# tmtlakmal/acme

Measured on AMD Instinct MI355X. Metric: learner transitions/sec (sample+step) at batch 512, 1/2/4/8 MI355X, higher is better.
Workload: dtype f32 (2xf16 split planes, 3 MFMA terms); 1 GPU; dqn_nature_cnn_prioritized_replay (BASELINE configs[1]); global_batch=512, batch_per_gpu=512, replay_slots=1000000, replay_slots_per_gpu=1000000, obs=uint8[84,84,4], num_actions=18, sampler=prioritized(alpha=0.6), IS beta=0.2, prefetch_size=4, parallelism=dp1

## Files before the change

### acme_amd/_lib.py

```python

from __future__ import annotations

import ctypes
import os
import threading

import torch

_HERE = os.path.dirname(os.path.abspath(__file__))
LIB_PATH = os.environ.get("ACME_LIB_PATH") or os.path.join(_HERE, "libacme_hip.so")

ACME_OK = 0
ACME_ERR_INVALID = -1
ACME_ERR_HIP = -2
ACME_ERR_EMPTY = -3
ACME_ERR_OOM = -4

SEMANTICS_TF = 0
SEMANTICS_JAX = 1

MATMUL_F32 = 0
MATMUL_X6 = 1

MAX_FIELDS = 16
# ... 68 lines not shown
MPO_MAX_ROWS = 131072
MPO_STATS = ("dual_alpha_mean", "dual_alpha_stddev", "dual_temperature", "loss_policy",
             "loss_alpha", "loss_temperature", "kl_q_rel", "penalty_kl_q_rel", "q_min", "q_max",
             "pi_stddev_min", "pi_stddev_max", "pi_stddev_cond")


class MPOConfig(ctypes.Structure):
    _fields_ = [("obs_dim", c_i32), ("act_dim", c_i32), ("max_batch", c_i32),
                ("num_policy_layers", c_i32), ("policy_sizes", c_i32 * D4PG_MAX_LAYERS),
                ("num_critic_layers", c_i32), ("critic_sizes", c_i32 * D4PG_MAX_LAYERS),
                ("action_min", c_f32 * D4PG_MAX_ACT), ("action_max", c_f32 * D4PG_MAX_ACT),
                ("discount", c_f32),
                ("policy_learning_rate", c_f32), ("critic_learning_rate", c_f32),
                ("adam_beta1", c_f32), ("adam_beta2", c_f32), ("adam_epsilon", c_f32),
                ("clipping", c_i32), ("layer_norm_epsilon", c_f32),
                ("num_samples", c_i32), ("target_policy_update_period", c_i32),
                ("target_critic_update_period", c_i32), ("dual_learning_rate", c_f32),
                ("epsilon", c_f32), ("epsilon_mean", c_f32), ("epsilon_stddev", c_f32),
                ("epsilon_penalty", c_f32), ("init_log_temperature", c_f32),
                ("init_log_alpha_mean", c_f32), ("init_log_alpha_stddev", c_f32),
                ("per_dim_constraining", c_i32), ("action_penalization", c_i32),
                ("init_scale", c_f32), ("min_scale", c_f32), ("seed", ctypes.c_uint64)]


class DMPOConfig(ctypes.Structure):
    _anonymous_ = ("mpo",)
    _fields_ = [("mpo", MPOConfig), ("num_atoms", c_i32), ("vmin", c_f32), ("vmax", c_f32)]


class MPOBatch(ctypes.Structure):
    _fields_ = [("o_tm1", c_vp), ("a_tm1", c_vp), ("r_t", c_vp), ("d_t", c_vp), ("o_t", c_vp),
                ("batch", c_i64), ("noise", c_vp)]


class MPOOutputs(ctypes.Structure):
    _fields_ = [("critic_loss", c_vp), ("policy_loss", c_vp), ("stats", c_vp),
                ("kl_mean_rel", c_vp), ("kl_stddev_rel", c_vp)]


IMPALA_TORSO_ATARI = 0
IMPALA_TORSO_FLAT = 1


class IMPALAConfig(ctypes.Structure):
    _fields_ = [("torso", c_i32), ("obs_dim", c_i32), ("num_actions", c_i32),
                ("max_batch", c_i32), ("max_sequence_length", c_i32), ("lstm_size", c_i32),
                ("head_size", c_i32), ("discount", c_f32), ("entropy_cost", c_f32),
                ("baseline_cost", c_f32), ("max_abs_reward", c_f32),
                ("max_gradient_norm", c_f32), ("learning_rate", c_f32), ("adam_beta1", c_f32),
                ("adam_beta2", c_f32), ("adam_epsilon", c_f32), ("semantics", c_i32)]


class R2D2Config(ctypes.Structure):
    _fields_ = [("torso", c_i32), ("obs_dim", c_i32), ("num_actions", c_i32),
                ("max_batch", c_i32), ("max_sequence_length", c_i32), ("burn_in_length", c_i32),
                ("lstm_size", c_i32), ("head_size", c_i32), ("n_step", c_i32),
                ("store_lstm_state", c_i32), ("target_update_period", c_i32),
                ("reserved", c_i32), ("max_replay_size", c_i64),
                ("max_priority_weight", ctypes.c_double),
                ("importance_sampling_exponent", ctypes.c_double), ("discount", c_f32),
                ("learning_rate", c_f32), ("adam_beta1", c_f32), ("adam_beta2", c_f32),
                ("adam_epsilon", c_f32)]


class R2D2Outputs(ctypes.Structure):
    _fields_ = [("loss", c_vp), ("errors", c_vp), ("priorities", c_vp)]


class SequenceBatch(ctypes.Structure):
    _fields_ = [("observation", c_vp), ("prev_action", c_vp), ("prev_reward", c_vp),
                ("action", c_vp), ("reward", c_vp), ("discount", c_vp),
                ("behaviour_logits", c_vp), ("h0", c_vp), ("c0", c_vp),
                ("state_stride", c_i64), ("batch", c_i64), ("sequence_length", c_i64)]


_SIGS = {
    "acme_last_error": (ctypes.c_char_p, []),
    "acme_tune_set": (ctypes.c_int, [ctypes.c_char_p, ctypes.c_int32]),
    "acme_version": (ctypes.c_char_p, []),
    "acme_target_arch": (ctypes.c_char_p, []),
    "acme_set_matmul_engine": (c_i32, [c_i32]),
    "acme_matmul_engine": (c_i32, []),
    "acme_dense_forward": (c_i32, [c_vp, c_i64, c_i64, c_vp, c_vp, c_i64, c_i32, c_vp, c_vp]),
    "acme_dense_forward_staged": (c_i32, [c_vp, c_i64, c_i64, c_vp, c_vp, c_i64, c_i32, c_vp,
                                          c_i32, c_i32, c_i32, c_vp]),
    "acme_replay_create": (c_i32, [ctypes.POINTER(ReplayConfig), ctypes.POINTER(c_vp)]),
    "acme_replay_destroy": (c_i32, [c_vp]),
    "acme_replay_insert": (c_i32, [c_vp, ctypes.POINTER(c_vp), c_i64, c_vp, c_i32, c_vp, c_vp]),
    "acme_replay_stage_capacity": (c_i64, [c_vp]),
    "acme_replay_stage": (c_i32, [c_vp, c_i64, ctypes.POINTER(c_vp)]),
    "acme_replay_commit": (c_i32, [c_vp, c_i64, c_vp, c_vp, c_vp]),
    "acme_replay_sync_inserts": (c_i32, [c_vp]),
    "acme_host_register": (c_i32, [c_vp, c_i64]),
    "acme_event_create": (c_i32, [ctypes.POINTER(c_vp)]),
    "acme_event_destroy": (c_i32, [c_vp]),
    "acme_event_record": (c_i32, [c_vp, c_vp]),
    "acme_stream_wait_event": (c_i32, [c_vp, c_vp]),
    "acme_event_query": (c_i32, [c_vp]),
    "acme_event_synchronize": (c_i32, [c_vp]),
    "acme_host_unregister": (c_i32, [c_vp]),
    "acme_nstep_writer_create": (c_i32, [c_vp, c_i32, c_f32, c_i64, c_i64, c_i64, c_vp]),
    "acme_nstep_writer_destroy": (c_i32, [c_vp]),
    "acme_nstep_writer_start": (c_i32, [c_vp, c_vp]),
    "acme_nstep_writer_add": (c_i32, [c_vp, c_vp, c_f32, c_f32, c_vp, c_i32, c_f64]),
    "acme_nstep_writer_flush": (c_i32, [c_vp]),
    "acme_nstep_writer_reset": (c_i32, [c_vp]),
    "acme_nstep_writer_pending": (c_i64, [c_vp]),
    "acme_replay_fill_synthetic": (c_i32, [c_vp, c_i64, c_i32, c_i32, c_u64, c_vp]),
    "acme_replay_sample": (c_i32, [c_vp, c_i64, c_u64, c_vp, c_vp, c_vp, c_vp, c_vp, c_vp]),
    "acme_replay_gather": (c_i32, [c_vp, c_vp, c_i64, ctypes.POINTER(c_vp), c_vp]),
    "acme_replay_total": (c_i32, [c_vp, c_vp, c_vp]),
    "acme_replay_sample_share": (c_i32, [c_vp, c_i64, c_u64, c_f64, c_vp, c_vp, c_vp, c_vp, c_vp,
                                         ctypes.POINTER(c_vp), c_vp]),
    "acme_replay_sample_share_frames": (c_i32, [c_vp, c_i64, c_u64, c_f64, c_vp, c_vp, c_vp, c_vp,
                                                c_vp, ctypes.POINTER(c_vp), c_vp, c_vp]),
    "acme_replay_sample_gather": (c_i32, [c_vp, c_i64, c_u64, c_vp, c_vp, c_vp, c_vp, c_vp,
                                          ctypes.POINTER(c_vp), c_vp]),
    "acme_replay_sample_gather_frames": (c_i32, [c_vp, c_i64, c_u64, c_vp, c_vp, c_vp, c_vp,
                                                 c_vp, ctypes.POINTER(c_vp), c_vp, c_vp]),
    "acme_replay_pipe_open": (c_i32, [c_vp, ctypes.POINTER(c_i32)]),
    "acme_replay_pipe_close": (c_i32, [c_vp, c_i32]),
    "acme_replay_pipe_flush": (c_i32, [c_vp, c_i32]),
    "acme_replay_sample_gather_pipe": (c_i32, [c_vp, c_i32, c_i64, c_u64, c_vp, c_vp, c_vp, c_vp,
                                               c_vp, ctypes.POINTER(c_vp), c_vp]),
    "acme_r2d2_priorities": (c_i32, [c_vp, c_i32, c_i32, ctypes.c_double, c_vp, c_vp]),
    "acme_r2d2_importance_weights": (c_i32, [c_vp, c_i32, c_i64, ctypes.c_double, c_vp, c_vp]),
    "acme_frames_expand": (c_i32, [c_vp, c_i64, c_i64, c_i32, c_vp, c_i64, c_vp, c_vp]),
    "acme_replay_update_priorities": (c_i32, [c_vp, c_vp, c_vp, c_i64, c_vp]),
    "acme_replay_update_priorities_gated": (c_i32, [c_vp, c_vp, c_vp, c_i64, c_vp, c_vp]),
    "acme_replay_size": (c_i64, [c_vp]),
    "acme_replay_capacity": (c_i64, [c_vp]),
    "acme_replay_debug_leaves": (c_i32, [c_vp, ctypes.POINTER(c_vp), ctypes.POINTER(c_vp),
                                         ctypes.POINTER(c_vp)]),
    "acme_replay_debug_level": (c_i32, [c_vp, c_i32, ctypes.POINTER(c_vp),
                                        ctypes.POINTER(c_i64), ctypes.POINTER(c_i32)]),
    "acme_replay_storage": (c_i32, [c_vp, c_i32, ctypes.POINTER(c_vp)]),
    "acme_replay_inserted": (c_i64, [c_vp]),
    "acme_replay_restore": (c_i32, [c_vp, c_i64, c_vp]),
    "acme_dqn_create": (c_i32, [ctypes.POINTER(DQNConfig), ctypes.POINTER(c_vp)]),
    "acme_dqn_destroy": (c_i32, [c_vp]),
    "acme_dqn_num_params": (c_i64, [c_vp]),
    "acme_dqn_flat_size": (c_i64, [c_vp]),
    "acme_dqn_num_tensors": (c_i32, [c_vp]),
    "acme_dqn_tensor_info": (c_i32, [c_vp, c_i32, ctypes.POINTER(c_i64), ctypes.POINTER(c_i64),
                                     ctypes.POINTER(c_i32), ctypes.POINTER(c_i64),
                                     ctypes.POINTER(ctypes.c_char_p)]),
    "acme_dqn_bind": (c_i32, [c_vp, c_vp, c_vp, c_vp, c_vp, c_vp]),
    "acme_dqn_params_changed": (c_i32, [c_vp]),
    "acme_dqn_plane_overflow": (c_i32, [c_vp, ctypes.POINTER(c_i32), c_i32]),
    "acme_dqn_skipped_steps": (c_i64, [c_vp]),
    "acme_dqn_guard_state": (c_i32, [c_vp, ctypes.POINTER(c_i64)]),
    "acme_dqn_verdict_timeouts": (c_i32, [c_vp, ctypes.POINTER(c_i64)]),
    "acme_dqn_update_rider_launches": (c_i64, [c_vp]),
    "acme_dqn_set_applied_steps": (c_i32, [c_vp, c_i64]),
    "acme_dqn_skip_word": (c_i32, [c_vp, ctypes.POINTER(c_vp)]),
    "acme_dqn_set_reissue": (c_i32, [c_vp, c_i32]),
    "acme_dqn_verdicts_issued": (c_i64, [c_vp]),
    "acme_dqn_step_verdict": (c_i32, [c_vp, c_i64, ctypes.POINTER(c_i32)]),
    "acme_dqn_set_data_parallel_gate": (c_i32, [c_vp, c_i32]),
    "acme_dqn_dense_grads_ready": (c_i32, [c_vp, c_vp]),
    "acme_dqn_dp_init": (c_i32, [c_vp, c_vp, c_i32]),
    "acme_dqn_dp_step": (c_i32, [c_vp, ctypes.POINTER(TransitionBatch), ctypes.POINTER(DQNOutputs),
                                 c_vp]),
    "acme_nccl_get_unique_id": (c_i32, [c_vp]),
    "acme_nccl_comm_init": (c_i32, [c_vp, c_i32, c_i32, ctypes.POINTER(c_vp)]),
    "acme_nccl_comm_destroy": (c_i32, [c_vp]),
    "acme_dqn_scale_state": (c_i32, [c_vp, c_vp, c_i32, ctypes.POINTER(c_i32)]),
    "acme_dqn_set_scale_state": (c_i32, [c_vp, c_vp, c_i32]),
    "acme_dqn_forward_backward": (c_i32, [c_vp, ctypes.POINTER(TransitionBatch),
                                          ctypes.POINTER(DQNOutputs), c_vp]),
    "acme_dqn_apply": (c_i32, [c_vp, c_vp]),
    "acme_dqn_forward_backward_stage": (c_i32, [c_vp, ctypes.POINTER(TransitionBatch),
                                                ctypes.POINTER(DQNOutputs), c_i32, c_vp]),
    "acme_dqn_grad_split": (c_i32, [c_vp, ctypes.POINTER(c_i64)]),
    "acme_dqn_step": (c_i32, [c_vp, ctypes.POINTER(TransitionBatch), ctypes.POINTER(DQNOutputs),
                              c_vp]),
    "acme_dqn_step_update": (c_i32, [c_vp, ctypes.POINTER(TransitionBatch),
                                     ctypes.POINTER(DQNOutputs), c_vp, c_vp, c_vp, c_vp]),
    "acme_dqn_q_values": (c_i32, [c_vp, c_vp, c_i64, c_i32, c_vp, c_vp]),
    "acme_dqn_num_steps": (c_i64, [c_vp]),
    "acme_dqn_debug_buffer": (c_i32, [c_vp, ctypes.c_char_p, ctypes.POINTER(c_vp),
                                      ctypes.POINTER(c_i64)]),
    "acme_dqn_set_num_steps": (c_i32, [c_vp, c_i64]),
    "acme_min_f64": (c_i32, [c_vp, c_i64, c_vp, c_vp]),
    "acme_r2d2_create": (c_i32, [ctypes.POINTER(R2D2Config), ctypes.POINTER(c_vp)]),
    "acme_r2d2_destroy": (c_i32, [c_vp]),
    "acme_r2d2_flat_size": (c_i64, [c_vp]),
    "acme_r2d2_num_tensors": (c_i32, [c_vp]),
    "acme_r2d2_tensor_info": (c_i32, [c_vp, c_i32, ctypes.POINTER(c_i64), ctypes.POINTER(c_i64),
                                      ctypes.POINTER(c_i32), ctypes.POINTER(c_i64),
                                      ctypes.POINTER(ctypes.c_char_p)]),
    "acme_r2d2_bind": (c_i32, [c_vp, c_vp, c_vp, c_vp, c_vp, c_vp]),
    "acme_r2d2_step": (c_i32, [c_vp, ctypes.POINTER(SequenceBatch), c_vp,
                               ctypes.POINTER(R2D2Outputs), c_vp]),
    "acme_r2d2_params_changed": (c_i32, [c_vp]),
    "acme_r2d2_scale_state": (c_i32, [c_vp, c_vp, c_i32, ctypes.POINTER(c_i32)]),
    "acme_r2d2_set_scale_state": (c_i32, [c_vp, c_vp, c_i32]),
    "acme_r2d2_skipped_steps": (c_i64, [c_vp]),
    "acme_r2d2_guard_state": (c_i32, [c_vp, ctypes.POINTER(c_i64)]),
    "acme_r2d2_skip_word": (c_vp, [c_vp]),
    "acme_r2d2_set_applied_steps": (c_i32, [c_vp, c_i64]),
    "acme_r2d2_num_steps": (c_i64, [c_vp]),
    "acme_r2d2_set_num_steps": (c_i32, [c_vp, c_i64]),
    "acme_r2d2_set_lstm_unroll": (c_i32, [c_vp, c_i32]),
    "acme_r2d2_debug_buffer": (c_i32, [c_vp, ctypes.c_char_p, ctypes.POINTER(c_vp),
                                       ctypes.POINTER(c_i64)]),
    "acme_impala_create": (c_i32, [ctypes.POINTER(IMPALAConfig), ctypes.POINTER(c_vp)]),
    "acme_impala_destroy": (c_i32, [c_vp]),
    "acme_impala_flat_size": (c_i64, [c_vp]),
    "acme_impala_num_tensors": (c_i32, [c_vp]),
    "acme_impala_tensor_info": (c_i32, [c_vp, c_i32, ctypes.POINTER(c_i64), ctypes.POINTER(c_i64),
                                        ctypes.POINTER(c_i32), ctypes.POINTER(c_i64),
                                        ctypes.POINTER(ctypes.c_char_p)]),
    "acme_impala_bind": (c_i32, [c_vp, c_vp, c_vp, c_vp, c_vp]),
    "acme_impala_params_changed": (c_i32, [c_vp]),
    "acme_impala_step": (c_i32, [c_vp, ctypes.POINTER(SequenceBatch), c_vp, c_vp]),
    "acme_impala_set_lstm_unroll": (c_i32, [c_vp, c_i32]),
    "acme_impala_plane_overflow": (c_i32, [c_vp, ctypes.POINTER(c_i32), c_i32]),
    "acme_impala_skipped_steps": (c_i64, [c_vp]),
    "acme_impala_guard_state": (c_i32, [c_vp, ctypes.POINTER(c_i64)]),
    "acme_impala_set_applied_steps": (c_i32, [c_vp, c_i64]),
    "acme_impala_scale_state": (c_i32, [c_vp, c_vp, c_i32, ctypes.POINTER(c_i32)]),
    "acme_impala_set_scale_state": (c_i32, [c_vp, c_vp, c_i32]),
    "acme_impala_policy_step": (c_i32, [c_vp, c_vp, c_vp, c_vp, c_vp, c_vp, c_i64, c_vp, c_vp,
                                        c_vp, c_vp, c_vp]),
    "acme_impala_set_policy_planes": (c_i32, [c_vp, c_i32]),
    "acme_impala_num_steps": (c_i64, [c_vp]),
    "acme_impala_set_num_steps": (c_i32, [c_vp, c_i64]),
    "acme_impala_debug_buffer": (c_i32, [c_vp, ctypes.c_char_p, ctypes.POINTER(c_vp),
                                         ctypes.POINTER(c_i64)]),
    "acme_d4pg_create": (c_i32, [ctypes.POINTER(D4PGConfig), ctypes.POINTER(c_vp)]),
    "acme_d4pg_destroy": (c_i32, [c_vp]),
    "acme_d4pg_flat_size": (c_i64, [c_vp]),
    "acme_d4pg_policy_size": (c_i64, [c_vp]),
    "acme_d4pg_num_tensors": (c_i32, [c_vp]),
    "acme_d4pg_tensor_info": (c_i32, [c_vp, c_i32, ctypes.POINTER(c_i64), ctypes.POINTER(c_i64),
                                      ctypes.POINTER(c_i32), ctypes.POINTER(c_i64),
                                      ctypes.POINTER(ctypes.c_char_p)]),
    "acme_d4pg_bind": (c_i32, [c_vp, c_vp, c_vp, c_vp, c_vp, c_vp]),
    "acme_d4pg_step": (c_i32, [c_vp, ctypes.POINTER(D4PGBatch), ctypes.POINTER(D4PGOutputs),
                               c_vp]),
    "acme_d4pg_policy": (c_i32, [c_vp, c_vp, c_i64, c_i32, c_vp, c_vp]),
    "acme_d4pg_num_steps": (c_i64, [c_vp]),
    "acme_d4pg_set_num_steps": (c_i32, [c_vp, c_i64]),
    "acme_d4pg_debug_buffer": (c_i32, [c_vp, ctypes.c_char_p, ctypes.POINTER(c_vp),
                                       ctypes.POINTER(c_i64)]),
    "acme_ddpg_create": (c_i32, [ctypes.POINTER(DDPGConfig), ctypes.POINTER(c_vp)]),
    "acme_ddpg_destroy": (c_i32, [c_vp]),
    "acme_ddpg_flat_size": (c_i64, [c_vp]),
    "acme_ddpg_policy_size": (c_i64, [c_vp]),
    "acme_ddpg_num_tensors": (c_i32, [c_vp]),
    "acme_ddpg_tensor_info": (c_i32, [c_vp, c_i32, ctypes.POINTER(c_i64), ctypes.POINTER(c_i64),
                                      ctypes.POINTER(c_i32), ctypes.POINTER(c_i64),
                                      ctypes.POINTER(ctypes.c_char_p)]),
    "acme_ddpg_bind": (c_i32, [c_vp, c_vp, c_vp, c_vp, c_vp, c_vp]),
    "acme_ddpg_step": (c_i32, [c_vp, ctypes.POINTER(D4PGBatch), ctypes.POINTER(D4PGOutputs),
                               c_vp]),
    "acme_ddpg_policy": (c_i32, [c_vp, c_vp, c_i64, c_i32, c_vp, c_vp]),
    "acme_ddpg_num_steps": (c_i64, [c_vp]),
    "acme_ddpg_set_num_steps": (c_i32, [c_vp, c_i64]),
    "acme_ddpg_debug_buffer": (c_i32, [c_vp, ctypes.c_char_p, ctypes.POINTER(c_vp),
                                       ctypes.POINTER(c_i64)]),
    "acme_mpo_create": (c_i32, [ctypes.POINTER(MPOConfig), ctypes.POINTER(c_vp)]),
    "acme_mpo_destroy": (c_i32, [c_vp]),
    "acme_mpo_flat_size": (c_i64, [c_vp]),
    "acme_mpo_policy_size": (c_i64, [c_vp]),
    "acme_mpo_dual_offset": (c_i64, [c_vp]),
    "acme_mpo_num_tensors": (c_i32, [c_vp]),
    "acme_mpo_tensor_info": (c_i32, [c_vp, c_i32, ctypes.POINTER(c_i64), ctypes.POINTER(c_i64),
                                     ctypes.POINTER(c_i32), ctypes.POINTER(c_i64),
                                     ctypes.POINTER(ctypes.c_char_p)]),
    "acme_mpo_bind": (c_i32, [c_vp, c_vp, c_vp, c_vp, c_vp, c_vp]),
    "acme_mpo_init_duals": (c_i32, [c_vp]),
    "acme_mpo_step": (c_i32, [c_vp, ctypes.POINTER(MPOBatch), ctypes.POINTER(MPOOutputs), c_vp]),
    "acme_mpo_policy": (c_i32, [c_vp, c_vp, c_i64, c_i32, c_vp, c_vp, c_vp]),
    "acme_mpo_num_steps": (c_i64, [c_vp]),
    "acme_mpo_set_num_steps": (c_i32, [c_vp, c_i64]),
    "acme_mpo_debug_buffer": (c_i32, [c_vp, ctypes.c_char_p, ctypes.POINTER(c_vp),
                                      ctypes.POINTER(c_i64)]),
    "acme_dmpo_create": (c_i32, [ctypes.POINTER(DMPOConfig), ctypes.POINTER(c_vp)]),
    "acme_dmpo_destroy": (c_i32, [c_vp]),
    "acme_dmpo_flat_size": (c_i64, [c_vp]),
    "acme_dmpo_policy_size": (c_i64, [c_vp]),
    "acme_dmpo_dual_offset": (c_i64, [c_vp]),
    "acme_dmpo_num_tensors": (c_i32, [c_vp]),
    "acme_dmpo_tensor_info": (c_i32, [c_vp, c_i32, ctypes.POINTER(c_i64), ctypes.POINTER(c_i64),
                                      ctypes.POINTER(c_i32), ctypes.POINTER(c_i64),
                                      ctypes.POINTER(ctypes.c_char_p)]),
    "acme_dmpo_bind": (c_i32, [c_vp, c_vp, c_vp, c_vp, c_vp, c_vp]),
    "acme_dmpo_init_duals": (c_i32, [c_vp]),
    "acme_dmpo_step": (c_i32, [c_vp, ctypes.POINTER(MPOBatch), ctypes.POINTER(MPOOutputs), c_vp]),
    "acme_dmpo_policy": (c_i32, [c_vp, c_vp, c_i64, c_i32, c_vp, c_vp, c_vp]),
    "acme_dmpo_num_steps": (c_i64, [c_vp]),
    "acme_dmpo_set_num_steps": (c_i32, [c_vp, c_i64]),
    "acme_dmpo_debug_buffer": (c_i32, [c_vp, ctypes.c_char_p, ctypes.POINTER(c_vp),
                                       ctypes.POINTER(c_i64)]),
    "acme_profile_enable": (c_i32, [c_i32]),
    "acme_profile_reset": (c_i32, []),
    "acme_profile_num_sections": (c_i32, []),
    "acme_profile_query_peak": (c_i32, [c_i32, ctypes.POINTER(c_f64)]),
    "acme_profile_query": (c_i32, [c_i32, ctypes.POINTER(ctypes.c_char_p), ctypes.POINTER(c_f64),
                                   ctypes.POINTER(c_i64), ctypes.POINTER(c_f64),
                                   ctypes.POINTER(c_f64)]),
    "acme_adam_update": (c_i32, [c_vp, c_vp, c_vp, c_vp, c_i64, c_f32, c_f32, c_f32, c_f32, c_i64,
                                 c_vp]),
}
# ... 106 lines not shown
```

### acme_amd/csrc/dqn.hip

```cpp
#include <hip/hip_runtime.h>

#include <algorithm>
#include <cmath>
#include <cstring>
#include <string>
#include <vector>

#include "common.h"
#include "conv.h"
#include "rescale.h"
#include "conv_p3.h"
#include "gemm.h"
#include "gemm_p3.h"
#include "gemm_x6.h"
#include "kernels.h"
#include "launch.h"
#include "learner_common.h"
#include "plane_guard.h"
#include "prio_update.h"
#include "profiler.h"
#include "rccl_dyn.h"
#include "torso.h"

using namespace acme;
using namespace acme::conv;
using acme::gemm::launch_gemm;

namespace {

using torso::G1;
constexpr int kFlat = torso::kFlat;
constexpr int kHidden = 512;
constexpr int kObsBytes = 84 * 84 * 4;

struct Layer {
  int in = 0, out = 0;
  int w = -1, b = -1;
  bool relu = true;
};

struct StepPlan {
  bool calibrating = false;
  bool fused = false;
  bool join_dense = false;
  acme_replay* replay = nullptr;
  const uint64_t* keys = nullptr;
  hipEvent_t after = nullptr;
};

struct StepState {
  int64_t fwd_batch = 0;
  bool last_p3 = false;
  torso::Frames cur_frames{nullptr};
  LossArgs pending_la{};
  bool loss_pending = false;
  bool head_deferred = false;
  int head_splits = 0;
  int64_t loss_nparts = 0;
  hipEvent_t dense_ev = nullptr;
  bool slabs_pending = false;
  torso::WgradSlab wslabs[3];
  bool rescaled = false;
  const double* upd_prio = nullptr;
  int upd_n = 0;
  bool update_issued = false;
};

}

struct acme_dqn : PlaneGuard {
  acme_dqn_config cfg;
  std::vector<Tensor> tensors;
  int64_t flat = 0, logical = 0;
  float *params = nullptr, *target = nullptr, *grads = nullptr, *m = nullptr, *v = nullptr;
  int64_t num_steps = 0;
  int t_c1w = -1, t_c1b, t_c2w, t_c2b, t_c3w, t_c3b, t_fcw, t_fcb, t_vw, t_vb, t_aw, t_ab;
  std::vector<Layer> layers;
  std::vector<void*> allocs;
  float *x1 = nullptr, *x2 = nullptr, *x3 = nullptr, *hid = nullptr;
  float *t1 = nullptr, *t2 = nullptr, *t3 = nullptr, *thid = nullptr;
  std::vector<float*> mlp_act, mlp_tact, mlp_dz;
  float *q_on = nullptr, *q_tg = nullptr;
  float *dzh = nullptr, *dz3 = nullptr, *dz2 = nullptr, *dz1 = nullptr;
  float* slab = nullptr;
  int64_t slab_floats = 0;
  bool stamps_on = false;
  uint64_t* stamps = nullptr;
  float* g = nullptr;
  int32_t* a_cache = nullptr;
  float* loss_tmp = nullptr;
  float* td_tmp = nullptr;
  double* prio_tmp = nullptr;
  bool p3_capable = false;
  bool planes_stale = true;
  uint16_t *wpl = nullptr, *tpl = nullptr;
  uint16_t* frames = nullptr;
  StepState step;
  hipStream_t side = nullptr;
  hipEvent_t ev[4] = {nullptr, nullptr, nullptr, nullptr};
  float* slab2 = nullptr;
  float* side_slab = nullptr;
  float* tslab = nullptr;
  bool target_dirty = true;
  torso::Plane x1p{}, x2p{}, x3p{}, t1p{}, t2p{}, t3p{}, dzhp{}, dz3p{}, dz2p{}, dz1p{};
  hipEvent_t ev_dense = nullptr;
  void* dp_comm = nullptr;
  int dp_world = 0;
  hipStream_t dp_stream = nullptr;
  hipEvent_t dp_ev[4] = {nullptr, nullptr, nullptr, nullptr};
  double* dp_gmin = nullptr;
  double* loss_part = nullptr;
  bool single_stream = false;
  bool single_role = false;
  bool bk32 = false;
  bool update_rider = true;
  int64_t rider_launches = 0;
  bool frames_u8 = true;
  int64_t seq = 0;
  uint32_t* host_verdicts = nullptr;
  uint32_t verdict_seq = 0;
  bool sticky = false;
  bool dp_gate = false;
  int64_t dp_gate_index = -1;
};

namespace {

enum {
  kScX1, kScX2, kScX3, kScT1, kScT2, kScT3, kScDzh, kScDz3, kScDz2, kScDz1,
  kScTransient,
  kScParams = kScTransient, kScTarget,
  kScCount
};
constexpr int64_t kParamAmaxPeriod = 8;
constexpr int kVerdictRing = 64;

int add_tensor(acme_dqn* l, const std::string& name, std::initializer_list<int64_t> shape) {
  const int t = acme::add_tensor<acme_dqn>(l, name, shape);
  l->logical += l->tensors[t].numel;
  return t;
}

inline torso::Plane WP(const acme_dqn* l, uint16_t* base, int t) {
  return torso::Plane{base + l->tensors[t].offset, l->flat,
                      l->scales + (base == l->tpl ? kScTarget : kScParams)};
}
int convert_frames(acme_dqn* l, const void* obs_a, const void* obs_b, int split, int rows,
                   hipStream_t st) {
  ACME_PROF("frames_f16", st, 0.0, 3.0 * (double)rows * kObsBytes);
  return launch_frames_f16(static_cast<const uint8_t*>(obs_a), static_cast<const uint8_t*>(obs_b),
                           split, rows, kObsBytes, l->frames, st);
}
bool use_p3(const acme_dqn* l) { return l->p3_capable && gemm::use_x6(); }
Gate step_gate(const acme_dqn* l) {
  Gate q;
  q.g = l->guard;
  q.par = (int)(l->seq & 1);
  if (l->dp_gate) q.dp = l->grads + l->dp_gate_index;
  return q;
}
hipStream_t side_stream(const acme_dqn* l) { return prof::enabled() ? nullptr : l->side; }

constexpr int kFcFwdSplits = 8;
constexpr int kHeadFwdSplits = 16;
constexpr int kHeadBwdSplits = 8;

int64_t slab_floats_needed(int B, int A) {
  return std::max<int64_t>({torso::wgrad_slab_floats(), (int64_t)kFcFwdSplits * 2 * B * 2 * kHidden,
                            (int64_t)kHeadFwdSplits * 2 * B * (A + 1),
                            (int64_t)kHeadBwdSplits * (2 * kHidden + 1) * (A + 1)});
}

int slab_reduce(const float* slab, int splits, int64_t count, float* out0, int64_t split_at,
                float* out1, const float* bias, int ncols, int relu, const char* name,
                hipStream_t st) {
  ACME_PROF(name, st, 0.0, 4.0 * (double)(splits + 1) * (double)count);
  return launch_slab_reduce(slab, splits, count, out0, split_at, out1, bias, ncols, relu, st);
}

int adam_range(acme_dqn* l, int64_t off, int64_t n, const Gate& gate, const AdamTail& tail,
               hipStream_t st) {
  const bool jax = l->cfg.semantics == ACME_SEMANTICS_JAX;
  const bool p3 = l->p3_capable;
  return launch_adam(l->params + off, l->grads + off, l->m + off, l->v + off, n,
                     l->cfg.learning_rate, l->cfg.adam_beta1, l->cfg.adam_beta2,
                     l->cfg.adam_epsilon, 0, p3 ? l->wpl + off : nullptr, l->flat, st, jax ? 1 : 0,
                     &l->guard->applied, p3 ? l->scales + kScParams : nullptr, gate, !p3, tail);
}

torso::Weights torso_weights(const acme_dqn* l, const float* prm) {
  return torso::Weights{P(l, prm, l->t_c1w), P(l, prm, l->t_c1b), P(l, prm, l->t_c2w),
                        P(l, prm, l->t_c2b), P(l, prm, l->t_c3w), P(l, prm, l->t_c3b)};
}
torso::Grads torso_grads(const acme_dqn* l) {
  float* gr = l->grads;
  return torso::Grads{Pm(l, gr, l->t_c1w), Pm(l, gr, l->t_c1b), Pm(l, gr, l->t_c2w),
                      Pm(l, gr, l->t_c2b), Pm(l, gr, l->t_c3w), Pm(l, gr, l->t_c3b)};
}
torso::PWeights torso_pweights(const acme_dqn* l, const float* prm, uint16_t* wpl) {
  return torso::PWeights{WP(l, wpl, l->t_c1w), WP(l, wpl, l->t_c2w), WP(l, wpl, l->t_c3w),
                         P(l, prm, l->t_c1b), P(l, prm, l->t_c2b), P(l, prm, l->t_c3b)};
}

int head_forward(acme_dqn* l, const float* prm, int rows, const float* hid, float* q,
                 hipStream_t st) {
  const int A = l->cfg.num_actions;
  DuelHeadFwd p;
  p.M = rows; p.N = A + 1; p.K = 2 * kHidden; p.k_chunk = chunk_for(p.K, kHeadFwdSplits);
  p.H = kHidden; p.A = A; p.h = hid; p.wv = P(l, prm, l->t_vw); p.wa = P(l, prm, l->t_aw);
  p.slab = l->slab;
  ACME_GEMM("head_fwd", 64, 32, 2, 1, 16, 1, p, kHeadFwdSplits);
  ACME_PROF("head_fwd_finish", st, 0.0, 0.0);
  return launch_duel_head_finish(l->slab, kHeadFwdSplits, rows, A, P(l, prm, l->t_vb),
                                 P(l, prm, l->t_ab), q, st);
}

int nature_forward(acme_dqn* l, const float* prm, const void* obs_a, const void* obs_b,
                   int split, int rows, float* x1, float* x2, float* x3, float* hid,
                   float* q, hipStream_t st) {
  const bool u8 = l->cfg.obs_dtype == ACME_OBS_U8_SCALED;
  int rc0 = torso::forward(torso_weights(l, prm), u8, obs_a, obs_b, split, rows,
                           torso::Acts{x1, x2, x3}, st);
  if (rc0 != ACME_OK) return rc0;
  {
    DenseFwd<true> p;
    const int splits = kFcFwdSplits;
    p.M = rows; p.N = 2 * kHidden; p.K = kFlat; p.k_chunk = chunk_for(kFlat, splits);
    p.x = x3; p.x2 = x3; p.split_b = rows; p.ldx = kFlat;
    p.w = P(l, prm, l->t_fcw); p.bias = P(l, prm, l->t_fcb); p.y = hid; p.act = ACT_RELU;
    p.slab = l->slab;
    ACME_GEMM("fc_fwd", 128, 128, 2, 2, 32, 1, p, splits);
    const int64_t cnt = (int64_t)rows * 2 * kHidden;
    int rc = slab_reduce(l->slab, splits, cnt, hid, cnt, nullptr, P(l, prm, l->t_fcb),
                         2 * kHidden, 1, "fc_fwd_reduce", st);
    if (rc != ACME_OK) return rc;
  }
  return head_forward(l, prm, rows, hid, q, st);
}

template <int BM>
int fc_fwd_gemm(const acme_dqn* l, const char* name, P3DenseFwd p, int splits,
                hipStream_t st) {
  if (l->single_role) ACME_P3_GEMM(name, BM, 128, 2, 2, 32, p, splits);
  else ACME_P3WS_GEMM(name, BM, 128, 2, 2, 32, p, splits);
  return ACME_OK;
}

int nature_forward_p3(acme_dqn* l, const float* prm, uint16_t* wpl, const torso::Frames& frames,
                      int rows, const torso::Plane& x1, const torso::Plane& x2,
                      const torso::Plane& x3, float* hid, float* q, hipStream_t st,
                      float* slab = nullptr, int keep_x1 = -1, bool defer_head = false) {
  if (!slab) slab = l->slab;
  int rc = torso::forward_p3(torso_pweights(l, prm, wpl), frames, rows, torso::PActs{x1, x2, x3}, st, keep_x1, l->bk32);
  if (rc != ACME_OK) return rc;
  {
    P3DenseFwd p;
    const bool tall = rows > 512;
    const bool ttall = rows == 512 && !defer_head;
    const int splits = kFcFwdSplits;
    p.M = rows; p.N = 2 * kHidden; p.K = kFlat; p.k_chunk = chunk_for(kFlat, splits);
    p.a_src = SRC(x3, (int64_t)rows * kFlat); p.ldx = kFlat;
    p.b_src = SRC(WP(l, wpl, l->t_fcw), (int64_t)kFlat * 2 * kHidden); p.slab = slab;
    if (tall) p.stamps = l->stamps;
    rc = tall || ttall ? fc_fwd_gemm<256>(l, ttall ? "fc_fwd_target" : "fc_fwd", p, splits, st)
                       : fc_fwd_gemm<128>(l, "fc_fwd", p, splits, st);
    if (rc != ACME_OK) return rc;
    if (defer_head &&
        dqn_head_loss_dz_fusable(kHidden, l->cfg.num_actions, splits, P(l, prm, l->t_vw),
                                 P(l, prm, l->t_aw), P(l, prm, l->t_fcb))) {
      l->step.head_deferred = true;
      l->step.head_splits = splits;
      return ACME_OK;
    }
    ACME_PROF("fc_head_fwd", st, 0.0, 4.0 * (double)rows * 2 * kHidden * (splits + 1));
    return launch_fc_head_forward(slab, splits, rows, kHidden, P(l, prm, l->t_fcb),
                                  P(l, prm, l->t_vw), P(l, prm, l->t_vb), P(l, prm, l->t_aw),
                                  P(l, prm, l->t_ab), l->cfg.num_actions, hid, q, st);
  }
}

template <class In>
int mlp_layer(acme_dqn* l, const float* prm, const Layer& L, const void* a, const void* b,
              int split, int rows, float* y, hipStream_t st) {
  const bool vec = L.in % 4 == 0 && L.out % 4 == 0;
  if (vec) {
    DenseFwd<true, In> p;
    p.M = rows; p.N = L.out; p.K = L.in; p.k_chunk = L.in;
    p.x = static_cast<const typename In::T*>(a); p.x2 = static_cast<const typename In::T*>(b);
    p.split_b = split; p.ldx = L.in; p.w = P(l, prm, L.w); p.bias = P(l, prm, L.b); p.y = y;
    p.act = L.relu ? ACT_RELU : ACT_NONE;
    ACME_GEMM("mlp_fwd", 64, 64, 2, 2, 16, 1, p, 1);
  } else {
    DenseFwd<false, In> p;
    p.M = rows; p.N = L.out; p.K = L.in; p.k_chunk = L.in;
    p.x = static_cast<const typename In::T*>(a); p.x2 = static_cast<const typename In::T*>(b);
    p.split_b = split; p.ldx = L.in; p.w = P(l, prm, L.w); p.bias = P(l, prm, L.b); p.y = y;
    p.act = L.relu ? ACT_RELU : ACT_NONE;
    ACME_GEMM("mlp_fwd", 64, 64, 2, 2, 16, 1, p, 1);
  }
  return ACME_OK;
}

int mlp_forward(acme_dqn* l, const float* prm, const void* obs_a, const void* obs_b, int split,
                int rows, std::vector<float*>& act, float* q, hipStream_t st) {
  const int nl = (int)l->layers.size();
  for (int i = 0; i < nl; ++i) {
    const Layer& L = l->layers[i];
    float* y = i == nl - 1 ? q : act[i];
    int rc;
    if (i == 0) {
      rc = l->cfg.obs_dtype == ACME_OBS_U8_SCALED
               ? mlp_layer<InU8>(l, prm, L, obs_a, obs_b, split, rows, y, st)
               : mlp_layer<InF32>(l, prm, L, obs_a, obs_b, split, rows, y, st);
    } else {
      rc = mlp_layer<InF32>(l, prm, L, act[i - 1], act[i - 1], rows, rows, y, st);
    }
    if (rc != ACME_OK) return rc;
  }
  return ACME_OK;
}

RescaleJob take_step_rescale(acme_dqn* l, bool defer_r) {
  RescaleJob j;
  j.s = l->scales;
  j.nt = j.n = kScTransient;
  j.overflow = l->overflow;
  j.skip_lo = kScT1;
  j.skip_hi = kScT3 + 1;
  j.defer_r = defer_r ? 1 : 0;
  j.rg.g = l->guard;
  j.rg.mode = kRgStep;
  j.rg.gate = step_gate(l);
  j.rg.host_skipped = l->host_skipped;
  j.rg.host_verdicts = l->host_verdicts;
  j.rg.seq = l->verdict_seq++;
  j.rg.sticky = l->sticky ? 1 : 0;
  l->step.rescaled = true;
  return j;
}

int torso_backward_p3(acme_dqn* l, const StepPlan& plan, int B, hipStream_t st) {
  const torso::Grads g = torso_grads(l);
  StepState& s = l->step;
  torso::Side sd;
  sd.bk32 = l->bk32;
  sd.conv1_single = true;
  if (side_stream(l)) {
    sd.side = l->side;
    sd.slab = l->side_slab;
    for (int i = 0; i < 3; ++i) sd.e[i] = l->ev[i];
  }
  if (plan.fused && !plan.calibrating && l->slab2) {
    sd.slab = l->side_slab;
    sd.slab2 = l->slab2;
    sd.defer = s.wslabs;
    s.slabs_pending = true;
  }
  int rc = torso::backward_p3_convs(torso_pweights(l, l->params, l->wpl), g, B,
                                    torso::PActs{l->x1p, l->x2p, l->x3p}, l->dz3p, l->dz2p,
                                    l->dz1p, l->slab, st, sd);
  if (rc != ACME_OK) return rc;
  const bool write_back = plan.replay && s.upd_prio;
  FusedUpdateArgs upd;
  const bool rider = write_back && l->update_rider && plan.fused && !l->dp_gate &&
                     s.upd_n >= 1 && s.upd_n <= kUpdateRiderMax;
  if (rider) {
    if (plan.after) ACME_HIP_TRY(hipStreamWaitEvent(st, plan.after, 0));
    const RescaleJob job = take_step_rescale(l, true);
    if ((rc = replay_update_prepare(plan.replay, plan.keys, s.upd_prio, s.upd_n, step_gate(l), st,
                                    &job, kUpdateRiderBlocks, &upd)) != ACME_OK)
      return rc;
    l->rider_launches += 1;
    s.update_issued = true;
  }
  rc = torso::backward_p3_conv1(g, s.cur_frames, B, l->dz1p, l->slab, st, sd,
                                rider ? &upd : nullptr);
  if (rider) replay_update_release(plan.replay);
  if (rc != ACME_OK) return rc;
  if (write_back && !rider) {
    s.update_issued = true;
    if (plan.after) ACME_HIP_TRY(hipStreamWaitEvent(st, plan.after, 0));
    const RescaleJob job = take_step_rescale(l, true);
    if ((rc = replay_update_priorities_gated(plan.replay, plan.keys, s.upd_prio, s.upd_n,
                                             step_gate(l), st, &job)) != ACME_OK)
      return rc;
  }
  return torso::backward_p3_join(st, sd);
}

int nature_backward(acme_dqn* l, const StepPlan& plan, const void* o_tm1, int B,
                    hipStream_t st_main, bool join_dense) {
  StepState& s = l->step;
  hipStream_t st = st_main;
  const float* prm = l->params;
  float* gr = l->grads;
  const int A = l->cfg.num_actions;
  const bool p3 = use_p3(l);
  int rc;
  bool loss_sum = false;
  const LossArgs la = s.pending_la;
  if (p3 && s.loss_pending && s.head_deferred) {
    s.loss_pending = s.head_deferred = false;
    loss_sum = true;
    s.loss_nparts = B;
    ACME_PROF("head_loss_dz", st, 0.0, 4.0 * (double)2 * B * 2 * kHidden * (s.head_splits + 1));
    rc = launch_dqn_head_loss_dz(la, l->slab, s.head_splits, kHidden, P(l, prm, l->t_fcb),
// ... 29 lines not shown
    s.upd_n = B;
  }
  const bool sum_in_scatter = loss_sum;
  {
    DuelHeadWgrad p;
    p.M = 2 * kHidden; p.N = A + 1; p.K = B; p.k_chunk = chunk_for(B, kHeadBwdSplits);
    p.A = A; p.h = l->hid; p.g = l->g; p.act = l->a_cache; p.slab = hslab;
    ACME_GEMM("head_wgrad", 64, 32, 2, 1, 16, 1, p, kHeadBwdSplits);
    ACME_PROF("head_wgrad_scatter", st, 0.0, 0.0);
    rc = launch_duel_head_grad_scatter(
        hslab, kHeadBwdSplits, kHidden, A, Pm(l, gr, l->t_vw), Pm(l, gr, l->t_vb),
        Pm(l, gr, l->t_aw), Pm(l, gr, l->t_ab), st, sum_in_scatter ? la.loss_part : nullptr,
        s.loss_nparts, la.mean_over, la.loss);
    if (rc != ACME_OK) return rc;
  }
  if (p3) {
    {
      P3DenseWgrad p;
      p.M = kFlat; p.N = 2 * kHidden; p.K = B; p.k_chunk = B;
      p.a_src = SRC(l->x3p, (int64_t)B * kFlat); p.ldx = kFlat;
      p.b_src = SRC(l->dzhp, (int64_t)B * 2 * kHidden); p.out = Pm(l, gr, l->t_fcw);
      p.bias_out = Pm(l, gr, l->t_fcb);
      ACME_P3_GEMM("fc_wgrad", 128, 128, 2, 2, 16, p, 1);
    }
    if (fork) {
      ACME_HIP_TRY(hipEventRecord(l->ev[3], l->side));
      st = st_main;
    }
    {
      P3DenseDgrad p;
      p.M = B; p.N = kFlat; p.K = 2 * kHidden; p.k_chunk = p.K;
      p.a_src = SRC(l->dzhp, (int64_t)B * 2 * kHidden);
      p.b_src = SRC(WP(l, l->wpl, l->t_fcw), (int64_t)kFlat * 2 * kHidden); p.xprev = CP(l->x3p);
      p.ldx = kFlat; p.dx = PP(l->dz3p);
      if (l->single_role) ACME_P3G_GEMM("fc_dgrad", 128, 128, 2, 2, 32, 3, p, 1);
      else ACME_P3WS_GEMM("fc_dgrad", 128, 128, 2, 2, 32, p, 1);
    }
    if (fork && join_dense) ACME_HIP_TRY(hipStreamWaitEvent(st_main, l->ev[3], 0));
    if (fork) s.dense_ev = l->ev[3];
    return ACME_OK;
  }
  {
    DenseWgrad<true> p;
    p.M = kFlat; p.N = 2 * kHidden; p.K = B; p.k_chunk = B;
    p.x = l->x3; p.ldx = kFlat; p.dz = l->dzh; p.out = Pm(l, gr, l->t_fcw);
    p.bias_out = Pm(l, gr, l->t_fcb);
    ACME_GEMM("fc_wgrad", 128, 128, 2, 2, 16, 1, p, 1);
  }
  {
    DenseDgrad<true> p;
    p.M = B; p.N = kFlat; p.K = 2 * kHidden; p.k_chunk = p.K;
    p.dz = l->dzh; p.w = P(l, prm, l->t_fcw); p.xprev = l->x3; p.ldx = kFlat; p.dx = l->dz3;
    ACME_GEMM("fc_dgrad", 64, 128, 2, 2, 16, 1, p, 1);
  }
  return ACME_OK;
}

template <class In>
int mlp_wgrad(acme_dqn* l, const Layer& L, const void* x, const float* dz, int B, float* dw,
              float* db, hipStream_t st) {
  if (L.in % 4 == 0 && L.out % 4 == 0) {
    DenseWgrad<true, In> p;
    p.M = L.in; p.N = L.out; p.K = B; p.k_chunk = B;
    p.x = static_cast<const typename In::T*>(x); p.ldx = L.in; p.dz = dz; p.out = dw;
    p.bias_out = db;
    ACME_GEMM("mlp_wgrad", 64, 64, 2, 2, 16, 1, p, 1);
  } else {
    DenseWgrad<false, In> p;
    p.M = L.in; p.N = L.out; p.K = B; p.k_chunk = B;
    p.x = static_cast<const typename In::T*>(x); p.ldx = L.in; p.dz = dz; p.out = dw;
    p.bias_out = db;
    ACME_GEMM("mlp_wgrad", 64, 64, 2, 2, 16, 1, p, 1);
  }
  return ACME_OK;
}

int mlp_backward(acme_dqn* l, const void* o_tm1, int B, hipStream_t st) {
  const int nl = (int)l->layers.size();
  const float* prm = l->params;
  float* gr = l->grads;
  int rc = launch_onehot_dq(l->g, l->a_cache, B, l->cfg.num_actions, l->mlp_dz[nl - 1], st);
  if (rc != ACME_OK) return rc;
  for (int i = nl - 1; i >= 0; --i) {
    const Layer& L = l->layers[i];
    const float* dz = l->mlp_dz[i];
    if (i == 0) {
      rc = l->cfg.obs_dtype == ACME_OBS_U8_SCALED
               ? mlp_wgrad<InU8>(l, L, o_tm1, dz, B, Pm(l, gr, L.w), Pm(l, gr, L.b), st)
               : mlp_wgrad<InF32>(l, L, o_tm1, dz, B, Pm(l, gr, L.w), Pm(l, gr, L.b), st);
    } else {
      rc = mlp_wgrad<InF32>(l, L, l->mlp_act[i - 1], dz, B, Pm(l, gr, L.w), Pm(l, gr, L.b), st);
    }
    if (rc != ACME_OK) return rc;
    if (i > 0) {
      if (L.in % 4 == 0 && L.out % 4 == 0) {
        DenseDgrad<true> p;
        p.M = B; p.N = L.in; p.K = L.out; p.k_chunk = L.out;
        p.dz = dz; p.w = P(l, prm, L.w); p.xprev = l->mlp_act[i - 1]; p.ldx = L.in;
        p.dx = l->mlp_dz[i - 1];
        ACME_GEMM("mlp_dgrad", 64, 64, 2, 2, 16, 1, p, 1);
      } else {
        DenseDgrad<false> p;
        p.M = B; p.N = L.in; p.K = L.out; p.k_chunk = L.out;
        p.dz = dz; p.w = P(l, prm, L.w); p.xprev = l->mlp_act[i - 1]; p.ldx = L.in;
        p.dx = l->mlp_dz[i - 1];
        ACME_GEMM("mlp_dgrad", 64, 64, 2, 2, 16, 1, p, 1);
      }
    }
  }
  return ACME_OK;
}

int sync_planes(acme_dqn* l, hipStream_t st) {
  if (!l->p3_capable || !l->planes_stale) return ACME_OK;
  int rc = launch_split_planes(l->params, l->flat, l->wpl, l->flat, l->scales + kScParams, st,
                               l->overflow, 1);
  if (rc == ACME_OK)
    rc = launch_split_planes(l->target, l->flat, l->tpl, l->flat, l->scales + kScTarget, st,
                             l->overflow, 1);
  if (rc == ACME_OK) l->planes_stale = false;
  return rc;
}

int reset_scales(acme_dqn* l) {
  return scales_init(l, kScCount, [l](int i) {
    return i >= kScT1 && i <= kScT3 ? &l->guard->tt
           : i >= kScTransient     ? &l->guard->prm
                                   : &l->guard->on;
  });
}

}

extern "C" {

int acme_dqn_create(const acme_dqn_config* cfg, acme_dqn** out) {
  ACME_CHECK_ARG(cfg && out, "null argument");
  ACME_CHECK_ARG(cfg->num_actions >= 1 && cfg->num_actions <= 63, "num_actions must be in [1, 63]");
  ACME_CHECK_ARG(cfg->max_batch >= 1 && cfg->max_batch <= 65536, "max_batch must be in [1, 65536]");
  ACME_CHECK_ARG(cfg->network == ACME_NET_NATURE_DQN || cfg->network == ACME_NET_MLP,
                 "unknown network kind %d", cfg->network);
  ACME_CHECK_ARG(cfg->obs_dtype == ACME_OBS_U8_SCALED || cfg->obs_dtype == ACME_OBS_F32,
                 "unknown observation dtype %d", cfg->obs_dtype);
  ACME_CHECK_ARG(cfg->huber_loss_parameter >= 0.f, "quadratic_linear_boundary must be >= 0.");
  ACME_CHECK_ARG(cfg->target_update_period >= 1, "target_update_period must be >= 1");
  ACME_CHECK_ARG(cfg->semantics == ACME_SEMANTICS_TF || cfg->semantics == ACME_SEMANTICS_JAX,
                 "unknown learner semantics %d", cfg->semantics);
  acme_dqn* l = new acme_dqn();
  l->cfg = *cfg;
  l->single_stream = tune_variant("SIDE") == 1;
  l->single_role = tune_variant("WSN") == 1;
  l->bk32 = tune_variant("BK32") == 1;
  l->update_rider = tune_variant("UPDATE_RIDER", kUpdateRiderDefault) != 0;
  l->stamps_on = tune_variant("STAMPS") == 1;
  const int A = cfg->num_actions;
  const int B = cfg->max_batch;
  int rc = ACME_OK;
  auto fail = [&](int code) {
    acme_dqn_destroy(l);
    return code;
  };
  if ((rc = guard_create(l)) != ACME_OK) return fail(rc);
  if (hipHostMalloc(reinterpret_cast<void**>(&l->host_verdicts), kVerdictRing * sizeof(uint32_t),
                    hipHostMallocCoherent | hipHostMallocMapped) != hipSuccess)
    return fail((set_error("step guard allocation failed"), ACME_ERR_HIP));
  for (int i = 0; i < kVerdictRing; ++i) l->host_verdicts[i] = 0xFFFFFFFFu;
  if (cfg->network == ACME_NET_NATURE_DQN) {
    l->t_c1w = add_tensor(l, "atari_torso/conv2_d/w", {8, 8, 4, 32});
    l->t_c1b = add_tensor(l, "atari_torso/conv2_d/b", {32});
    l->t_c2w = add_tensor(l, "atari_torso/conv2_d_1/w", {4, 4, 32, 64});
    l->t_c2b = add_tensor(l, "atari_torso/conv2_d_1/b", {64});
    l->t_c3w = add_tensor(l, "atari_torso/conv2_d_2/w", {3, 3, 64, 64});
    l->t_c3b = add_tensor(l, "atari_torso/conv2_d_2/b", {64});
    l->t_fcw = add_tensor(l, "duelling_q_network/hidden/w", {kFlat, 2 * kHidden});
    l->t_fcb = add_tensor(l, "duelling_q_network/hidden/b", {2 * kHidden});
    l->t_vw = add_tensor(l, "duelling_q_network/mlp/linear_1/w", {kHidden, 1});
    l->t_vb = add_tensor(l, "duelling_q_network/mlp/linear_1/b", {1});
    l->t_aw = add_tensor(l, "duelling_q_network/mlp_1/linear_1/w", {kHidden, A});
    l->t_ab = add_tensor(l, "duelling_q_network/mlp_1/linear_1/b", {A});
    const int R2 = 2 * B;
    if ((rc = dev_alloc(l, &l->x1, (int64_t)R2 * G1::OPIX * G1::CO)) ||
        (rc = dev_alloc(l, &l->x2, (int64_t)R2 * kFlat)) ||
        (rc = dev_alloc(l, &l->x3, (int64_t)R2 * kFlat)) ||
        (rc = dev_alloc(l, &l->hid, (int64_t)R2 * 2 * kHidden)) ||
        (rc = dev_alloc(l, &l->t1, (int64_t)B * G1::OPIX * G1::CO)) ||
        (rc = dev_alloc(l, &l->t2, (int64_t)B * kFlat)) ||
        (rc = dev_alloc(l, &l->t3, (int64_t)B * kFlat)) ||
        (rc = dev_alloc(l, &l->thid, (int64_t)B * 2 * kHidden)) ||
        (rc = dev_alloc(l, &l->dzh, (int64_t)B * 2 * kHidden)) ||
        (rc = dev_alloc(l, &l->dz3, (int64_t)B * kFlat)) ||
        (rc = dev_alloc(l, &l->dz2, (int64_t)B * kFlat)) ||
        (rc = dev_alloc(l, &l->dz1, (int64_t)B * G1::OPIX * G1::CO)))
      return fail(rc);
    l->slab_floats = slab_floats_needed(B, A);
    if (cfg->obs_dtype == ACME_OBS_U8_SCALED && (int64_t)R2 * kObsBytes * 2 < (int64_t)INT32_MAX) {
      l->p3_capable = true;
      const int64_t fl = l->flat;
      if ((rc = reset_scales(l)) ||
          (rc = dev_alloc(l, &l->wpl, gemm::kPlanes * fl)) ||
          (rc = dev_alloc(l, &l->tpl, gemm::kPlanes * fl)) ||
          (rc = dev_alloc(l, &l->frames, (int64_t)R2 * kObsBytes)) ||
          (rc = plane_alloc(l, &l->x1p, (int64_t)R2 * torso::kX1, kScX1)) ||
          (rc = plane_alloc(l, &l->x2p, (int64_t)R2 * kFlat, kScX2)) ||
          (rc = plane_alloc(l, &l->x3p, (int64_t)R2 * kFlat, kScX3)) ||
          (rc = plane_alloc(l, &l->t1p, (int64_t)B * torso::kX1, kScT1)) ||
          (rc = plane_alloc(l, &l->t2p, (int64_t)B * kFlat, kScT2)) ||
          (rc = plane_alloc(l, &l->t3p, (int64_t)B * kFlat, kScT3)) ||
          (rc = plane_alloc(l, &l->dzhp, (int64_t)B * 2 * kHidden, kScDzh)) ||
          (rc = dev_alloc(l, &l->loss_part,
                          std::max<int64_t>(B, dqn_loss_head_dz_blocks(B, kHidden)))) ||
          (rc = plane_alloc(l, &l->dz3p, (int64_t)B * kFlat, kScDz3)) ||
          (rc = plane_alloc(l, &l->dz2p, (int64_t)B * kFlat, kScDz2)) ||
          (rc = plane_alloc(l, &l->dz1p, (int64_t)B * torso::kX1, kScDz1)))
        return fail(rc);
      l->slab_floats = std::max(l->slab_floats, torso::wgrad_slab_floats_p3());
      if (!l->single_stream) {
        hipError_t e = hipStreamCreateWithFlags(&l->side, hipStreamNonBlocking);
        for (auto& ev : l->ev)
          if (e == hipSuccess) e = make_order_event(&ev);
        if (e != hipSuccess)
          return fail((set_error("side stream: %s", hipGetErrorString(e)), ACME_ERR_HIP));
      }
      if ((rc = dev_alloc(l, &l->side_slab, l->slab_floats)) ||
          (rc = dev_alloc(l, &l->tslab, l->slab_floats)) ||
          (rc = dev_alloc(l, &l->slab2, torso::wgrad_slab_floats_p3())))
        return fail(rc);
    }
  } else {
    ACME_CHECK_ARG(cfg->obs_dim >= 1, "obs_dim must be >= 1");
    ACME_CHECK_ARG(cfg->num_hidden >= 0 && cfg->num_hidden <= ACME_MAX_MLP_LAYERS,
                   "num_hidden must be in [0, %d]", ACME_MAX_MLP_LAYERS);
    int in = cfg->obs_dim;
    char name[64];
    for (int i = 0; i <= cfg->num_hidden; ++i) {
      Layer L;
      L.in = in;
      L.out = i < cfg->num_hidden ? cfg->hidden[i] : A;
      L.relu = i < cfg->num_hidden;
      if (L.out < 1) return fail((set_error("hidden sizes must be >= 1"), ACME_ERR_INVALID));
      snprintf(name, sizeof(name), "mlp/linear_%d/w", i);
      L.w = add_tensor(l, name, {L.in, L.out});
      snprintf(name, sizeof(name), "mlp/linear_%d/b", i);
      L.b = add_tensor(l, name, {L.out});
      l->layers.push_back(L);
      in = L.out;
    }
    for (size_t i = 0; i < l->layers.size(); ++i) {
      float *a = nullptr, *ta = nullptr, *dz = nullptr;
      const int w = l->layers[i].out;
      if ((rc = dev_alloc(l, &a, (int64_t)2 * B * w)) || (rc = dev_alloc(l, &ta, (int64_t)B * w)) ||
          (rc = dev_alloc(l, &dz, (int64_t)B * w)))
        return fail(rc);
      l->mlp_act.push_back(a);
      l->mlp_tact.push_back(ta);
      l->mlp_dz.push_back(dz);
    }
    l->slab_floats = 1;
  }
  if (make_order_event(&l->ev_dense) != hipSuccess)
    return fail((set_error("event creation failed"), ACME_ERR_HIP));
  if ((rc = dev_alloc(l, &l->q_on, (int64_t)2 * B * A)) ||
      (rc = dev_alloc(l, &l->q_tg, (int64_t)B * A)) ||
      (rc = dev_alloc(l, &l->slab, l->slab_floats)) ||
      (rc = dev_alloc(l, &l->g, (int64_t)B)) || (rc = dev_alloc(l, &l->a_cache, (int64_t)B)) ||
      (rc = dev_alloc(l, &l->loss_tmp, 4)) || (rc = dev_alloc(l, &l->td_tmp, (int64_t)B)) ||
      (rc = dev_alloc(l, &l->prio_tmp, (int64_t)B)) ||
      (l->stamps_on && (rc = dev_alloc(l, &l->stamps, (int64_t)5 * 4096 * 8))))
    return fail(rc);
  if (l->stamps_on) {
    for (int i = 0; i < 3; ++i) torso::g_stamps_conv[i] = l->stamps + (int64_t)(i + 1) * 4096 * 8;
    g_update_stamps = l->stamps + (int64_t)4 * 4096 * 8;
  }
  if (hipDeviceSynchronize() != hipSuccess)
    return fail((set_error("learner init failed"), ACME_ERR_HIP));
  *out = l;
  return ACME_OK;
}

int acme_dqn_destroy(acme_dqn* l) {
  if (!l) return ACME_OK;
  (void)hipDeviceSynchronize();
  if (l->stamps_on) {
    for (auto& p : torso::g_stamps_conv) p = nullptr;
    g_update_stamps = nullptr;
  }
  for (void* p : l->allocs) (void)hipFree(p);
  for (auto& e : l->ev)
    if (e) (void)hipEventDestroy(e);
  if (l->side) (void)hipStreamDestroy(l->side);
  if (l->ev_dense) (void)hipEventDestroy(l->ev_dense);
  for (auto& e : l->dp_ev)
    if (e) (void)hipEventDestroy(e);
  if (l->dp_stream) (void)hipStreamDestroy(l->dp_stream);
  guard_destroy(l);
  if (l->host_verdicts) (void)hipHostFree(l->host_verdicts);
  delete l;
  return ACME_OK;
}

int64_t acme_dqn_num_params(const acme_dqn* l) { return l ? l->logical : 0; }
int64_t acme_dqn_flat_size(const acme_dqn* l) { return l ? l->flat : 0; }
int32_t acme_dqn_num_tensors(const acme_dqn* l) { return l ? (int32_t)l->tensors.size() : 0; }

int acme_dqn_tensor_info(const acme_dqn* l, int32_t i, int64_t* offset, int64_t* numel,
                         int32_t* ndim, int64_t* shape4, const char** name) {
  return tensor_info(l, i, offset, numel, ndim, shape4, name);
}

int acme_dqn_bind(acme_dqn* l, float* params, float* target, float* grads, float* adam_m,
                  float* adam_v) {
  ACME_CHECK_ARG(l && params && target && grads && adam_m && adam_v, "null buffer");
  for (const float* p : {params, target, grads, adam_m, adam_v})
    ACME_CHECK_ARG(reinterpret_cast<uintptr_t>(p) % 16 == 0, "buffers must be 16-byte aligned");
  l->params = params;
  l->target = target;
  l->grads = grads;
  l->m = adam_m;
  l->v = adam_v;
  l->planes_stale = true;
  l->scales_ok = false;
  return ACME_OK;
}

int acme_dqn_params_changed(acme_dqn* l) {
  ACME_CHECK_ARG(l, "null learner");
  l->planes_stale = true;
  l->scales_ok = false;
  l->target_dirty = true;
  return ACME_OK;
}

int acme_dqn_scale_state(const acme_dqn* l, float* out, int32_t capacity, int32_t* count) {
  return scale_state(l, out, capacity, count);
}

int acme_dqn_set_scale_state(acme_dqn* l, const float* in, int32_t count) {
  const int rc = set_scale_state(l, in, count);
  if (rc == ACME_OK) l->target_dirty = true;
  return rc;
}

int acme_dqn_plane_overflow(acme_dqn* l, int32_t* overflow, int32_t reset) {
  return plane_overflow(l, overflow, reset);
}

int64_t acme_dqn_skipped_steps(const acme_dqn* l) { return skipped_steps(l); }

int acme_dqn_guard_state(acme_dqn* l, int64_t* out4) {
  ACME_CHECK_ARG(l && out4 && l->guard, "null argument");
  StepGuard g;
  if (int rc = read_guard(l, &g)) return rc;
  out4[0] = g.applied;
  out4[1] = g.skipped;
  out4[2] = g.last;
  out4[3] = g.qv;
  return ACME_OK;
}

int acme_dqn_verdict_timeouts(acme_dqn* l, int64_t* out) {
  ACME_CHECK_ARG(l && out, "null argument");
  *out = 0;
  if (!l->guard) return ACME_OK;
  StepGuard g;
  if (int rc = read_guard(l, &g)) return rc;
  *out = g.vtimeout;
  return ACME_OK;
}

int64_t acme_dqn_update_rider_launches(const acme_dqn* l) { return l ? l->rider_launches : 0; }

int acme_dqn_set_reissue(acme_dqn* l, int32_t enable) {
  ACME_CHECK_ARG(l, "null learner");
  l->sticky = enable != 0 && l->p3_capable;
  return ACME_OK;
}

int64_t acme_dqn_verdicts_issued(const acme_dqn* l) { return l ? (int64_t)l->verdict_seq : 0; }

int acme_dqn_step_verdict(const acme_dqn* l, int64_t seq, int32_t* state) {
  ACME_CHECK_ARG(l && state && seq >= 0, "bad argument");
  *state = -1;
  if (!l->host_verdicts || seq >= (int64_t)l->verdict_seq) return ACME_OK;
  ACME_CHECK_ARG(seq + kVerdictRing >= (int64_t)l->verdict_seq,
                 "verdict %lld is older than the ring's %d", (long long)seq, kVerdictRing);
  const uint32_t v =
      __atomic_load_n(l->host_verdicts + (seq & (kVerdictRing - 1)), __ATOMIC_ACQUIRE);
  if ((v >> 1) == ((uint32_t)seq & 0x7fffffffu)) *state = (int32_t)(v & 1u);
  return ACME_OK;
}

int acme_dqn_set_applied_steps(acme_dqn* l, int64_t n) {
  ACME_CHECK_ARG(l && l->guard && n >= 0, "bad argument");
  return set_applied(l, n);
}

int acme_dqn_skip_word(const acme_dqn* l, const uint32_t** out) {
  ACME_CHECK_ARG(l && out, "null argument");
  *out = l->p3_capable ? &l->guard->last : nullptr;
  return ACME_OK;
}

int acme_dqn_set_data_parallel_gate(acme_dqn* l, int32_t enable) {
  ACME_CHECK_ARG(l, "null learner");
  if (enable && l->cfg.network == ACME_NET_NATURE_DQN && l->p3_capable) {
    const Tensor& t = l->tensors[l->t_c1b];
    ACME_CHECK_ARG(align64(t.offset + t.numel) > t.offset + t.numel, "no padding word for the gate");
    l->dp_gate_index = t.offset + t.numel;
    l->dp_gate = true;
  } else {
    l->dp_gate = false;
  }
  return ACME_OK;
}

int64_t acme_dqn_num_steps(const acme_dqn* l) { return l ? l->num_steps : 0; }
int acme_dqn_set_num_steps(acme_dqn* l, int64_t n) {
  ACME_CHECK_ARG(l && n >= 0, "bad argument");
  l->num_steps = n;
  return ACME_OK;
}

int acme_dqn_debug_buffer(const acme_dqn* l, const char* name, const float** out,
                          int64_t* count) {
  ACME_CHECK_ARG(l && name && out && count, "null argument");
  const int64_t B = l->cfg.max_batch;
  struct {
    const char* n;
    const float* p;
    int64_t c;
  } tab[] = {{"gemm_stamps", reinterpret_cast<const float*>(l->stamps), 2 * 5 * 4096 * 8},
             {"x1", l->x1, 2 * B * 441 * 32}, {"x2", l->x2, 2 * B * kFlat},
             {"x3", l->x3, 2 * B * kFlat},    {"hid", l->hid, 2 * B * 2 * kHidden},
             {"dzh", l->dzh, B * 2 * kHidden}, {"dz3", l->dz3, B * kFlat},
             {"dz2", l->dz2, B * kFlat},       {"dz1", l->dz1, B * 441 * 32},
             {"q_on", l->q_on, 2 * B * l->cfg.num_actions},
             {"q_tg", l->q_tg, B * l->cfg.num_actions}, {"g", l->g, B}};
  for (auto& e : tab)
    if (e.p && std::strcmp(e.n, name) == 0) {
      if (l->step.last_p3) {
        struct {
          const char* n;
          torso::Plane pl;
        } ptab[] = {{"x1", l->x1p},   {"x2", l->x2p},   {"x3", l->x3p},  {"dzh", l->dzhp},
                    {"dz3", l->dz3p}, {"dz2", l->dz2p}, {"dz1", l->dz1p}};
        for (auto& q : ptab)
          if (std::strcmp(q.n, name) == 0) {
            int rc = launch_join_planes(q.pl.p, q.pl.stride, e.c, const_cast<float*>(e.p),
                                        q.pl.sc, 0);
            if (rc != ACME_OK) return rc;
            ACME_HIP_TRY(hipDeviceSynchronize());
          }
      }
      *out = e.p;
      *count = e.c;
      return ACME_OK;
    }
  for (size_t i = 0; i < l->mlp_act.size(); ++i) {
    char nm[16];
    snprintf(nm, sizeof(nm), "act%zu", i);
    if (std::strcmp(nm, name) == 0) {
      *out = l->mlp_act[i];
      *count = 2 * B * l->layers[i].out;
      return ACME_OK;
    }
  }
  set_error("unknown debug buffer '%s'", name);
  return ACME_ERR_INVALID;
}

int acme_dqn_q_values(acme_dqn* l, const void* obs, int64_t batch, int32_t use_target,
                      float* q_out, void* stream) {
  ACME_CHECK_ARG(l && obs && q_out && l->params, "null argument or unbound learner");
  ACME_CHECK_ARG(batch >= 1 && batch <= l->cfg.max_batch, "batch must be in [1, max_batch]");
  hipStream_t st = as_stream(stream);
  const float* prm = use_target ? l->target : l->params;
  const int B = (int)batch;
  if (l->cfg.network == ACME_NET_NATURE_DQN && use_p3(l)) {
    l->target_dirty = true;
    int rc = sync_planes(l, st);
    if (rc == ACME_OK) rc = convert_frames(l, obs, obs, B, B, st);
    for (int pass = l->scales_ok ? 1 : 0; pass < 2 && rc == ACME_OK; ++pass) {
      rc = nature_forward_p3(l, prm, use_target ? l->tpl : l->wpl, torso::Frames{l->frames}, B,
                             l->t1p, l->t2p, l->t3p, l->thid, q_out, st);
      RescaleGuard rg;
      rg.g = l->guard;
      rg.mode = kRgQValues;
      if (rc == ACME_OK)
        rc = launch_plane_rescale(l->scales + kScT1, 3, 3, -1, -1, l->overflow, st, -1, -1, rg);
    }
    return rc;
  }
  if (l->cfg.network == ACME_NET_NATURE_DQN)
    return nature_forward(l, prm, obs, obs, B, B, l->t1, l->t2, l->t3, l->thid, q_out, st);
  return mlp_forward(l, prm, obs, obs, B, B, l->mlp_tact, q_out, st);
}

static int forward_backward_stage(acme_dqn* l, const StepPlan& plan,
                                  const acme_transition_batch* batch,
                                  const acme_dqn_outputs* out, int32_t stage, void* stream);

int acme_dqn_forward_backward_stage(acme_dqn* l, const acme_transition_batch* batch,
                                    const acme_dqn_outputs* out, int32_t stage, void* stream) {
  StepPlan plan;
  plan.join_dense = true;
  return forward_backward_stage(l, plan, batch, out, stage, stream);
}

static int loss_and_dense_backward(acme_dqn* l, const StepPlan& plan,
                                   const acme_transition_batch* batch,
                                   const acme_dqn_outputs* out, hipStream_t st, bool join_dense) {
  const int B = (int)batch->batch, A = l->cfg.num_actions;
  const bool nature = l->cfg.network == ACME_NET_NATURE_DQN;
  int rc;
  float* loss = out && out->loss ? out->loss : l->loss_tmp;
  float* td = out && out->td_error ? out->td_error : l->td_tmp;
  double* prio = out && out->priorities ? out->priorities : l->prio_tmp;
  LossArgs la;
  la.q_on = l->q_on;
  la.q_tg = l->q_tg;
  la.a = batch->a_tm1;
  la.r = batch->r_t;
  la.d = batch->d_t;
  la.probs = batch->probabilities;
  la.global_min_prob = batch->global_min_probability;
  la.B = B;
  la.A = A;
  la.mean_over = batch->mean_over > 0 ? (int)batch->mean_over : B;
  la.discount = l->cfg.discount;
  la.beta = l->cfg.importance_sampling_exponent;
  la.delta = l->cfg.huber_loss_parameter;
  la.max_abs_reward = l->cfg.max_abs_reward;
  la.jax = l->cfg.semantics == ACME_SEMANTICS_JAX;
  la.loss = loss;
  la.td = td;
  la.prio = prio;
  la.g = l->g;
  la.a_cache = l->a_cache;
  if (l->step.last_p3) {
    la.loss_part = l->loss_part;
    l->step.pending_la = la;
    l->step.loss_pending = true;
  } else {
    ACME_PROF("loss", st, 0.0, 0.0);
    if ((rc = launch_dqn_loss(la, st)) != ACME_OK) return rc;
  }
  rc = nature ? nature_backward(l, plan, batch->o_tm1, B, st, join_dense)
              : mlp_backward(l, batch->o_tm1, B, st);
  if (rc != ACME_OK) return rc;
  if (out && out->q_tm1)
    ACME_HIP_TRY(hipMemcpyAsync(out->q_tm1, l->q_on, (size_t)B * A * sizeof(float),
                                hipMemcpyDeviceToDevice, st));
  if (!l->step.dense_ev) {
    ACME_HIP_TRY(hipEventRecord(l->ev_dense, st));
    l->step.dense_ev = l->ev_dense;
  }
  return ACME_OK;
}

constexpr int kCalibrationPasses = 4;
static int calibrate_scales(acme_dqn* l, const acme_transition_batch* batch, hipStream_t st) {
  acme_transition_batch cb = *batch;
  cb.global_min_probability = nullptr;
  StepPlan plan;
  plan.calibrating = true;
  const StepState outer = l->step;
  int rc = ACME_OK;
  for (int pass = 0; pass < kCalibrationPasses && rc == ACME_OK; ++pass) {
    rc = forward_backward_stage(l, plan, &cb, nullptr, 2, st);
    if (rc == ACME_OK) rc = forward_backward_stage(l, plan, &cb, nullptr, 3, st);
    if (rc == ACME_OK) rc = forward_backward_stage(l, plan, &cb, nullptr, 1, st);
    if (rc == ACME_OK)
      rc = launch_plane_rescale(l->scales, kScTransient, kScTransient, -1, -1, l->overflow, st);
  }
  l->step = outer;
  if (rc != ACME_OK) return rc;
  return calibration_done(l, st);
}

static int forward_backward_stage(acme_dqn* l, const StepPlan& plan,
                                  const acme_transition_batch* batch,
                                  const acme_dqn_outputs* out, int32_t stage, void* stream) {
  ACME_CHECK_ARG(l && batch && l->params, "null argument or unbound learner");
  ACME_CHECK_ARG(stage >= 0 && stage <= 4, "stage must be 0, 1, 2, 3 or 4");
  ACME_CHECK_ARG(batch->o_tm1 && batch->a_tm1 && batch->r_t && batch->d_t && batch->o_t &&
                     batch->probabilities,
                 "transition batch has null fields");
  ACME_CHECK_ARG(batch->batch >= 1 && batch->batch <= l->cfg.max_batch,
                 "batch %lld outside [1, max_batch=%d]", (long long)batch->batch, l->cfg.max_batch);
  hipStream_t st = as_stream(stream);
  const int B = (int)batch->batch;
  const bool nature = l->cfg.network == ACME_NET_NATURE_DQN;
  if (stage == 1) {
    if (!nature) return ACME_OK;
    if (use_p3(l)) {
      int rc = torso_backward_p3(l, plan, B, st);
      if (rc == ACME_OK && l->dp_gate && !plan.calibrating) {
        Gate local = step_gate(l);
        local.dp = nullptr;
        rc = launch_gate_publish(local, l->grads + l->dp_gate_index, st, l->scales,
                                 kScTransient, kScT1, kScT3 + 1);
      }
      return rc;
    }
    return torso::backward(torso_weights(l, l->params), torso_grads(l),
                           l->cfg.obs_dtype == ACME_OBS_U8_SCALED, batch->o_tm1, B,
                           torso::Acts{l->x1, l->x2, l->x3}, l->dz3, l->dz2, l->dz1, l->slab, st);
  }
  int rc;
  if (stage == 3 || stage == 4) {
    ACME_CHECK_ARG(l->step.fwd_batch == (int64_t)B,
                   "stage %d needs the stage-2 forward of this batch", stage);
    l->step.fwd_batch = 0;
    return loss_and_dense_backward(l, plan, batch, out, st, plan.join_dense && stage == 3);
  }
  l->step = StepState{};
  l->step.last_p3 = nature && use_p3(l);
  if (l->step.last_p3) {
    const bool u8 = !batch->obs_f16 && l->frames_u8 &&
                    ((reinterpret_cast<uintptr_t>(batch->o_tm1) |
                      reinterpret_cast<uintptr_t>(batch->o_t)) & 15) == 0;
    const bool quiet =
        !l->planes_stale && l->scales_ok && (batch->obs_f16 || u8) && !plan.calibrating;
    if ((rc = sync_planes(l, st)) != ACME_OK) return rc;
    if (!l->scales_ok && !plan.calibrating && (rc = calibrate_scales(l, batch, st)) != ACME_OK)
      return rc;
    hipStream_t tst = st;
    hipStream_t side = side_stream(l);
    if (!batch->obs_f16 && !u8 &&
        (rc = convert_frames(l, batch->o_tm1, batch->o_t, B, 2 * B, st)) != ACME_OK)
      return rc;
    const torso::Frames fwd_frames =
        u8 ? torso::Frames{batch->o_tm1, true, batch->o_t, B}
           : torso::Frames{batch->obs_f16 ? static_cast<const void*>(batch->obs_f16)
                                          : static_cast<const void*>(l->frames)};
    l->step.cur_frames = fwd_frames;
    if (side) {
      if (quiet && batch->inputs_event && !l->target_dirty) {
        ACME_HIP_TRY(hipStreamWaitEvent(side, static_cast<hipEvent_t>(batch->inputs_event), 0));
      } else {
        ACME_HIP_TRY(hipEventRecord(l->ev[0], st));
        ACME_HIP_TRY(hipStreamWaitEvent(side, l->ev[0], 0));
      }
      l->target_dirty = plan.calibrating;
      tst = side;
    } else {
      l->target_dirty = true;
    }
    const bool online_first = side != nullptr;
    if (online_first &&
        (rc = nature_forward_p3(l, l->params, l->wpl, fwd_frames, 2 * B, l->x1p, l->x2p, l->x3p,
                                l->hid, l->q_on, st, nullptr, B, true)) != ACME_OK)
      return rc;
    if ((rc = nature_forward_p3(l, l->target, l->tpl, fwd_frames.rows_from(B), B,
                                l->t1p, l->t2p, l->t3p, l->thid, l->q_tg, tst,
                                side ? l->tslab : l->slab, 0)) != ACME_OK)
      return rc;
    {
      RescaleGuard rg;
      rg.g = l->guard;
      rg.mode = kRgTarget;
      rg.gate = step_gate(l);
      if ((rc = launch_plane_rescale(l->scales + kScT1, 3, 3, -1, -1, l->overflow, tst, -1, -1,
                                     rg)))
        return rc;
    }
    if (side) ACME_HIP_TRY(hipEventRecord(l->ev[1], side));
    if (!online_first &&
        (rc = nature_forward_p3(l, l->params, l->wpl, fwd_frames, 2 * B, l->x1p, l->x2p, l->x3p,
                                l->hid, l->q_on, st, nullptr, B, true)) != ACME_OK)
      return rc;
    if (side) ACME_HIP_TRY(hipStreamWaitEvent(st, l->ev[1], 0));
  } else if (nature) {
    if ((rc = nature_forward(l, l->params, batch->o_tm1, batch->o_t, B, 2 * B, l->x1, l->x2, l->x3,
                             l->hid, l->q_on, st)) != ACME_OK)
      return rc;
    if ((rc = nature_forward(l, l->target, batch->o_t, batch->o_t, B, B, l->t1, l->t2, l->t3,
                             l->thid, l->q_tg, st)) != ACME_OK)
      return rc;
  } else {
    if ((rc = mlp_forward(l, l->params, batch->o_tm1, batch->o_t, B, 2 * B, l->mlp_act, l->q_on,
                          st)) != ACME_OK)
      return rc;
    if ((rc = mlp_forward(l, l->target, batch->o_t, batch->o_t, B, B, l->mlp_tact, l->q_tg, st)) !=
        ACME_OK)
      return rc;
  }
  if (stage == 2) {
    l->step.fwd_batch = B;
    return ACME_OK;
  }
  return loss_and_dense_backward(l, plan, batch, out, st, plan.join_dense);
}

int acme_dqn_forward_backward(acme_dqn* l, const acme_transition_batch* batch,
                              const acme_dqn_outputs* out, void* stream) {
  const StepPlan plan;
  int rc = forward_backward_stage(l, plan, batch, out, 0, stream);
  if (rc != ACME_OK) return rc;
  return forward_backward_stage(l, plan, batch, out, 1, stream);
}

int acme_dqn_grad_split(const acme_dqn* l, int64_t* split) {
  ACME_CHECK_ARG(l && split, "null argument");
  *split = l->cfg.network == ACME_NET_NATURE_DQN ? l->tensors[l->t_fcw].offset : 0;
  return ACME_OK;
}

static bool copies_target(const acme_dqn* l) {
  const int64_t at = l->cfg.semantics == ACME_SEMANTICS_JAX ? l->num_steps + 1 : l->num_steps;
  return at % l->cfg.target_update_period == 0;
}

static int apply_impl(acme_dqn* l, hipStream_t st) {
  const bool copy = copies_target(l);
  int rc = ACME_OK;
  Gate gate;
  AdamTail tail;
  if (l->p3_capable) {
    if (!l->step.rescaled) {
      ACME_PROF("plane_rescale", st, 0.0, 0.0);
      if ((rc = launch_rescale_job(take_step_rescale(l, false), st)) != ACME_OK) return rc;
    } else {
      tail.commit = l->scales;
      tail.ncommit = kScTransient;
      tail.skip_lo = kScT1;
      tail.skip_hi = kScT3 + 1;
    }
    l->step.rescaled = false;
    gate.g = l->guard;
    gate.use_last = 1;
    tail.clear = l->guard;
    tail.params = l->scales + kScParams;
    if (copy) tail.target = l->scales + kScTarget;
  }
  const double adam_bytes = 28.0 * (double)l->logical + (l->p3_capable ? 4.0 * (double)l->flat : 0.0);
  if (l->step.slabs_pending) {
    l->step.slabs_pending = false;
    double slab_bytes = 0.0;
    for (int k = 0; k < 3; ++k) {
      const double count4 = (double)((l->step.wslabs[k].wcount + l->step.wslabs[k].bcount) / 4);
      slab_bytes += 16.0 * count4 * (double)(l->step.wslabs[k].splits + 1);
    }
    ACME_PROF("adam", st, 0.0, adam_bytes + slab_bytes);
    const int ten[3][2] = {{l->t_c1w, l->t_c1b}, {l->t_c2w, l->t_c2b}, {l->t_c3w, l->t_c3b}};
    AdamSlabs a;
    for (int k = 0; k < 3; ++k) {
      const torso::WgradSlab& w = l->step.wslabs[k];
      const int64_t count4 = (w.wcount + w.bcount) / 4;
      for (int j = 0; j < 2; ++j) {
        const Tensor& t = l->tensors[ten[k][j]];
        a.seg[a.nseg++] = AdamSlabs::Seg{t.offset / 4, t.numel / 4, w.slab, w.splits, count4,
                                         j ? w.wcount / 4 : 0};
      }
    }
    a.dense_off4 = l->tensors[l->t_fcw].offset / 4;
    a.dense_n4 = (l->flat - l->tensors[l->t_fcw].offset) / 4;
    rc = launch_adam_slabs(l->params, l->grads, l->m, l->v, a, l->cfg.learning_rate,
                           l->cfg.adam_beta1, l->cfg.adam_beta2, l->cfg.adam_epsilon,
                           &l->guard->applied, l->wpl, l->flat, l->scales + kScParams,
                           l->cfg.semantics == ACME_SEMANTICS_JAX ? 1 : 0, gate, tail, st);
    if (rc != ACME_OK) return rc;
  } else {
    ACME_PROF("adam", st, 0.0, adam_bytes);
    if ((rc = adam_range(l, 0, l->flat, gate, tail, st)) != ACME_OK) return rc;
  }
  if (copy) {
    l->target_dirty = true;
    ACME_PROF("target_copy", st, 0.0, 8.0 * (double)l->logical);
    if (l->p3_capable) {
      if ((rc = launch_copy_gated(l->target, l->params, l->flat * sizeof(float), l->tpl, l->wpl,
                                  gemm::kPlanes * l->flat * sizeof(uint16_t), gate, st)))
        return rc;
    } else {
      ACME_HIP_TRY(hipMemcpyAsync(l->target, l->params, l->flat * sizeof(float),
                                  hipMemcpyDeviceToDevice, st));
    }
  }
  if (l->p3_capable && l->num_steps % kParamAmaxPeriod == 0) {
    {
      ACME_PROF("param_amax", st, 0.0, 4.0 * (double)l->flat);
      if ((rc = launch_param_amax(l->params, l->flat, l->scales + kScParams, st)) != ACME_OK)
        return rc;
    }
    ACME_PROF("param_rescale", st, 0.0, 0.0);
    if ((rc = launch_plane_rescale(l->scales + kScParams, 0, 1, -1, -1, l->overflow, st)))
      return rc;
  }
  l->num_steps += 1;
  l->seq += 1;
  return ACME_OK;
}

int acme_dqn_apply(acme_dqn* l, void* stream) {
  ACME_CHECK_ARG(l && l->params, "unbound learner");
  return apply_impl(l, as_stream(stream));
}

static int step_impl(acme_dqn* l, const StepPlan& plan, const acme_transition_batch* batch,
                     const acme_dqn_outputs* out, hipStream_t st) {
  int rc = forward_backward_stage(l, plan, batch, out, 0, st);
  if (rc == ACME_OK) rc = forward_backward_stage(l, plan, batch, out, 1, st);
  if (rc == ACME_OK) rc = apply_impl(l, st);
  return rc;
}

int acme_dqn_dense_grads_ready(acme_dqn* l, void* stream) {
  ACME_CHECK_ARG(l && l->step.dense_ev, "no stage 3 / 4 has run");
  ACME_HIP_TRY(hipStreamWaitEvent(as_stream(stream), l->step.dense_ev, 0));
  return ACME_OK;
}

int acme_dqn_dp_init(acme_dqn* l, void* nccl_comm, int32_t world_size) {
  ACME_CHECK_ARG(l && nccl_comm && world_size >= 1, "bad data-parallel arguments");
  if (!acme::rccl::api()) return ACME_ERR_HIP;
  if (!l->dp_stream) {
    ACME_HIP_TRY(hipStreamCreateWithFlags(&l->dp_stream, hipStreamNonBlocking));
    for (auto& e : l->dp_ev) ACME_HIP_TRY(make_order_event(&e));
    int rc = dev_alloc(l, &l->dp_gmin, 1);
    if (rc != ACME_OK) return rc;
  }
  l->dp_comm = nccl_comm;
  l->dp_world = world_size;
// ... 86 lines not shown
```

### acme_amd/csrc/gemm_p3c12.h

```cpp
#pragma once

#include "conv_p3.h"
#include "gemm_p3i.h"

namespace acme {
namespace gemm {

template <class G1, class G2, bool U8 = false>
struct P3C1ToLds {
  using Base = conv::P3ConvFwd<G1, 1, U8>;
  using I2 = ImgGeom<G2, false>;
  static constexpr int A_MODE = Base::A_MODE, B_MODE = Base::B_MODE;
  static constexpr int A_PLANES = 1, B_PLANES = kPlanes;
  static constexpr bool kStore8 = true;
  static constexpr bool kAmax = true;
  int M, N, K, k_chunk;
  Base base;
  uint8_t* x1;
  int plane;
  int m0;
  bool hbm;
  __device__ PScale* amax_sc() const { return base.y.sc; }
  __device__ float store8(int m, int n, const conv::V8& acc, int) const {
    conv::V8 v;
    base.act8(n, acc, v);
    uint32_t h[4], l[4];
    const float mx = conv::split8(v, base.y.w(), h, l);
    const int pp = m - m0, oh = pp / G1::OW, ow = pp - oh * G1::OW;
    const int a = I2::at(0, oh, ow, n / 8);
    *reinterpret_cast<u32x4*>(x1 + a) = u32x4{h[0], h[1], h[2], h[3]};
    *reinterpret_cast<u32x4*>(x1 + plane + a) = u32x4{l[0], l[1], l[2], l[3]};
    if (hbm) {
      const int64_t e = (int64_t)m * G1::CO + n;
      *reinterpret_cast<uint4*>(base.y.p + e) = uint4{h[0], h[1], h[2], h[3]};
      *reinterpret_cast<uint4*>(base.y.p + base.y.stride + e) = uint4{l[0], l[1], l[2], l[3]};
    }
    return mx;
  }
};

template <class G1, class G2, bool U8 = false, int BK1_ = 32, int BK2_ = 32>
struct P3C12Cfg {
  using I1 = ImgGeomPairs<G1>;
  using I2 = ImgGeom<G2, false>;
  using P1 = conv::P3ConvFwd<G1, 1, U8>;
  using P2 = conv::P3ConvFwd<G2, kPlanes>;
  static constexpr int NP = kPlanes;
  using P1L = P3C1ToLds<G1, G2, U8>;
  static constexpr int NT = 512, GK = 32, KS = 2;
  static constexpr int BK1 = BK1_, BK2 = BK2_, NG1 = BK1 / GK, NG2 = BK2 / GK;
  using C1 = P3Core<512, 32, 8, 1, GK, P1L>;
  using C2 = P3Core<128, 64, 4, 2, GK, P2>;
  using PB1 = PlanP3<32, NT, RCONTIG, NP, GK>;
  using PB2 = PlanP3<64, NT, RCONTIG, NP, GK>;
  static_assert(BK1 % GK == 0 && BK2 % GK == 0, "a stage is whole 32-k groups");
  static_assert(NG1 * PB1::UNITS <= NT && NG2 * PB2::UNITS <= NT,
                "one weight unit per thread per plane and stage");
  static constexpr int ZERO1 = img_zero_base(I1::IMG);
  static constexpr int FRAME = ZERO1 + kImgZeroBytes;
  static constexpr int X1 = FRAME;
  static constexpr int RING1 = X1;
  static constexpr int ZERO2 = img_zero_base(I2::IMG);
  static constexpr int PLANE2 = ZERO2 + kImgZeroBytes;
  static constexpr int LDS = X1 + NP * PLANE2;
  static_assert(2 * NG1 * PB1::BYTES <= I2::IMG, "conv1's ring fits the first x1 plane's image");
  static_assert(2 * NG2 * PB2::BYTES <= I1::IMG && C1::EPI_BYTES <= I1::IMG &&
                    C2::EPI_BYTES <= I1::IMG,
                "conv2's ring and the epilogue staging reuse the frame image region");
  static_assert(G1::OPIX <= 512 && I2::OPIX <= 128 && P2::A_PLANES == NP, "geometry");
};

template <class G1, class G2, bool U8, int BK1_, int BK2_>
__global__ void __launch_bounds__(512) gemm_p3c12_kernel(const conv::P3ConvFwd<G1, 1, U8> p1,
                                                         const conv::P3ConvFwd<G2, kPlanes> p2,
                                                         int frames, int hbm_frames) {
  using Cfg = P3C12Cfg<G1, G2, U8, BK1_, BK2_>;
  using I1 = typename Cfg::I1;
  using I2 = typename Cfg::I2;
  using PB1 = typename Cfg::PB1;
  using PB2 = typename Cfg::PB2;
  using P1 = typename Cfg::P1;
  using P2 = typename Cfg::P2;
  constexpr int NT = Cfg::NT, GK = Cfg::GK, KS = Cfg::KS, NP = Cfg::NP;
  constexpr int BK1 = Cfg::BK1, BK2 = Cfg::BK2, NG1 = Cfg::NG1, NG2 = Cfg::NG2;
  extern __shared__ __attribute__((aligned(16))) uint8_t smem[];
  const int tid = threadIdx.x, lane = tid & 63, wave = tid >> 6;
  const int f = blockIdx.x;
  uint8_t* x1 = smem + Cfg::X1;
  using S0 = std::integral_constant<int, 0>;
  using S1 = std::integral_constant<int, 1>;

  const bool own1 = tid < NG1 * PB1::UNITS, own2 = tid < NG2 * PB2::UNITS;
  const int g1 = tid / PB1::UNITS, u1 = tid % PB1::UNITS;
  const int g2 = tid / PB2::UNITS, u2 = tid % PB2::UNITS;
  const typename P1::BRow br1 = p1.b_row(own1 ? PB1::row_of(u1) : 0);
  const typename P2::BRow br2 = p2.b_row(own2 ? PB2::row_of(u2) : 0);
  __amdgpu_buffer_rsrc_t sb1[NP], sb2[NP];
#pragma unroll
  for (int pl = 0; pl < NP; ++pl) {
    sb1[pl] = plane_rsrc(p1.b_src, pl);
    sb2[pl] = plane_rsrc(p2.b_src, pl);
  }
  u32x4 r1[2][NP], r2[2][NP];
  auto fetch1 = [&](auto S, int k0) {
    constexpr int set = decltype(S)::value;
    const uint32_t off =
        own1 && k0 + g1 * GK < p1.K ? p1.b_off(br1, k0 + g1 * GK, PB1::kk_of(u1)) : kOOB;
#pragma unroll
    for (int pl = 0; pl < NP; ++pl)
      r1[set][pl] = __builtin_bit_cast(u32x4, __builtin_amdgcn_raw_buffer_load_b128(sb1[pl], off, 0, 0));
  };
  auto fetch2 = [&](auto S, int k0) {
    constexpr int set = decltype(S)::value;
    const uint32_t off =
        own2 && k0 + g2 * GK < p2.K ? p2.b_off(br2, k0 + g2 * GK, PB2::kk_of(u2)) : kOOB;
#pragma unroll
    for (int pl = 0; pl < NP; ++pl)
      r2[set][pl] = __builtin_bit_cast(u32x4, __builtin_amdgcn_raw_buffer_load_b128(sb2[pl], off, 0, 0));
  };
  auto stash1 = [&](auto S, int buf) {
    constexpr int set = decltype(S)::value;
    if (!own1) return;
    uint8_t* s = smem + Cfg::RING1 + (buf * NG1 + g1) * PB1::BYTES;
#pragma unroll
    for (int pl = 0; pl < NP; ++pl) *reinterpret_cast<u32x4*>(s + pl * PB1::PLANE + PB1::offset(u1)) = r1[set][pl];
  };
  auto stash2 = [&](auto S, int buf) {
    constexpr int set = decltype(S)::value;
    if (!own2) return;
    uint8_t* s = smem + (buf * NG2 + g2) * PB2::BYTES;
#pragma unroll
    for (int pl = 0; pl < NP; ++pl) *reinterpret_cast<u32x4*>(s + pl * PB2::PLANE + PB2::offset(u2)) = r2[set][pl];
  };
  fetch1(S0{}, 0);
  fetch1(S1{}, BK1);
  fetch2(S0{}, 0);
  fetch2(S1{}, BK2);

  if constexpr (AU8<P1>::value) {
    constexpr int U8U = I1::UNITS / 2;
    constexpr int PER = (U8U + NT - 1) / NT;
    const __amdgpu_buffer_rsrc_t sa = plane_rsrc(p1.a_src, 0);
    u32x4 v[PER];
#pragma unroll
    for (int j = 0; j < PER; ++j) {
      const int u = tid + j * NT;
      const uint32_t off = u < U8U ? (uint32_t)(((int64_t)f * U8U + u) * 16) : kOOB;
      v[j] = __builtin_bit_cast(u32x4, __builtin_amdgcn_raw_buffer_load_b128(sa, off, 0, 0));
    }
#pragma unroll
    for (int j = 0; j < PER; ++j) {
      const int u = tid + j * NT;
      if (u < U8U) {
        *reinterpret_cast<u32x4*>(smem + I1::fill(0, 2 * u)) = f16x8_of_bytes(v[j][0], v[j][1]);
        *reinterpret_cast<u32x4*>(smem + I1::fill(0, 2 * u + 1)) = f16x8_of_bytes(v[j][2], v[j][3]);
      }
    }
    if (tid < 16) *reinterpret_cast<u32x4*>(smem + Cfg::ZERO1 + 16 * tid) = zero_u4();
    else if (tid < 16 + 16 * NP)
      *reinterpret_cast<u32x4*>(x1 + ((tid >> 4) - 1) * Cfg::PLANE2 + Cfg::ZERO2 + 16 * (tid & 15)) = zero_u4();
  } else {
    constexpr int PER = (I1::UNITS + NT - 1) / NT;
    const __amdgpu_buffer_rsrc_t sa = plane_rsrc(p1.a_src, 0);
    u32x4 v[PER];
#pragma unroll
    for (int j = 0; j < PER; ++j) {
      const int u = tid + j * NT;
      const uint32_t off = u < I1::UNITS ? (uint32_t)(((int64_t)f * I1::UNITS + u) * 16) : kOOB;
      v[j] = __builtin_bit_cast(u32x4, __builtin_amdgcn_raw_buffer_load_b128(sa, off, 0, 0));
    }
#pragma unroll
    for (int j = 0; j < PER; ++j) {
      const int u = tid + j * NT;
      if (u < I1::UNITS) *reinterpret_cast<u32x4*>(smem + I1::fill(0, u)) = v[j];
    }
    if (tid < 16) *reinterpret_cast<u32x4*>(smem + Cfg::ZERO1 + 16 * tid) = zero_u4();
    else if (tid < 16 + 16 * NP)
      *reinterpret_cast<u32x4*>(x1 + ((tid >> 4) - 1) * Cfg::PLANE2 + Cfg::ZERO2 + 16 * (tid & 15)) = zero_u4();
  }
  stash1(S0{}, 0);
  __syncthreads();

  {
    typename I1::Lane ln[2];
#pragma unroll
    for (int i = 0; i < 2; ++i) {
      const int lr = wave * 64 + i * 32 + (lane & 31);
      ln[i] = I1::lane(0, lr, lr < G1::OPIX);
    }
    typename Cfg::C1::Acc acc;
    acc.zero();
    auto group = [&](int k0, const uint8_t* sb) {
      typename I1::Stage sg[2];
#pragma unroll
      for (int i = 0; i < 2; ++i) sg[i] = I1::stage(ln[i], k0, Cfg::ZERO1);
#pragma unroll
      for (int s = 0; s < KS; ++s) {
        f16x8 fb[NP];
#pragma unroll
        for (int pl = 0; pl < NP; ++pl) fb[pl] = PB1::frag(sb, pl, 0, s, lane);
#pragma unroll
        for (int i = 0; i < 2; ++i) {
          const int u = I1::unit(sg[i], ln[i], k0, s, lane >> 5);
          const f16x8 fa[1] = {*reinterpret_cast<const f16x8*>(smem + u)};
          acc.terms(i, 0, fa, fb);
        }
      }
    };
    auto compute = [&](int k0, int buf) {
#pragma unroll
      for (int g = 0; g < NG1; ++g)
        group(k0 + g * GK, smem + Cfg::RING1 + (buf * NG1 + g) * PB1::BYTES);
    };
    auto iter = [&](auto S, int kt) {
      constexpr int set = decltype(S)::value;
      using Other = std::integral_constant<int, set ^ 1>;
      stash1(Other{}, set ^ 1);
      fetch1(S, (kt + 2) * BK1);
      compute(kt * BK1, set);
      __syncthreads();
    };
    const int nk = p1.K / BK1;
    for (int kt = 0; kt < nk; kt += 2) {
      iter(S0{}, kt);
      iter(S1{}, kt + 1);
    }
    typename Cfg::P1L q;
    q.M = (f + 1) * G1::OPIX < p1.M ? (f + 1) * G1::OPIX : p1.M;
    q.N = p1.N; q.K = p1.K; q.k_chunk = p1.k_chunk;
    q.base = p1; q.x1 = x1; q.plane = Cfg::PLANE2; q.m0 = f * G1::OPIX; q.hbm = f < hbm_frames;
    Cfg::C1::epilogue(q, smem, q.m0, 0, wave, wave, 0, lane, 0, acc, false);
  }

  stash2(S0{}, 0);
  __syncthreads();
  {
    const int wm = wave >> 1, wn = wave & 1;
    const int lr = wm * 32 + (lane & 31);
    const typename I2::Lane ln = I2::lane(0, lr, lr < I2::OPIX);
    typename Cfg::C2::Acc acc;
    acc.zero();
    auto group = [&](int k0, const uint8_t* sb) {
      const typename I2::Stage sg = I2::stage(ln, k0, Cfg::ZERO2);
#pragma unroll
      for (int s = 0; s < KS; ++s) {
        f16x8 fb[NP];
#pragma unroll
        for (int pl = 0; pl < NP; ++pl) fb[pl] = PB2::frag(sb, pl, wn * 32, s, lane);
        const int u = I2::unit(sg, ln, k0, s, lane >> 5);
        const uint8_t* a = x1 + u;
        f16x8 fa[NP];
#pragma unroll
        for (int pl = 0; pl < NP; ++pl) fa[pl] = *reinterpret_cast<const f16x8*>(a + pl * Cfg::PLANE2);
        acc.terms(0, 0, fa, fb);
      }
    };
    auto compute = [&](int k0, int buf) {
#pragma unroll
      for (int g = 0; g < NG2; ++g) group(k0 + g * GK, smem + (buf * NG2 + g) * PB2::BYTES);
    };
    auto iter = [&](auto S, int kt) {
      constexpr int set = decltype(S)::value;
      using Other = std::integral_constant<int, set ^ 1>;
      stash2(Other{}, set ^ 1);
      fetch2(S, (kt + 2) * BK2);
      compute(kt * BK2, set);
      __syncthreads();
    };
    const int nk = p2.K / BK2;
    for (int kt = 0; kt < nk; kt += 2) {
      iter(S0{}, kt);
      iter(S1{}, kt + 1);
    }
    P2 q = p2;
    q.M = (f + 1) * I2::OPIX < p2.M ? (f + 1) * I2::OPIX : p2.M;
    Cfg::C2::epilogue(q, smem, f * I2::OPIX, 0, wave, wm, wn, lane, 0, acc, false);
  }
}

template <int BK1_, int BK2_, class G1, class G2, bool U8>
inline hipError_t launch_gemm_p3c12(const conv::P3ConvFwd<G1, 1, U8>& p1,
                                    const conv::P3ConvFwd<G2, kPlanes>& p2, int frames, int hbm_frames,
                                    hipStream_t st) {
  using Cfg = P3C12Cfg<G1, G2, U8, BK1_, BK2_>;
  static_assert(Cfg::LDS <= 160 * 1024, "LDS");
  static hipError_t attr = p3_set_lds(&gemm_p3c12_kernel<G1, G2, U8, BK1_, BK2_>, Cfg::LDS);
  if (attr != hipSuccess) return attr;
  if (frames < 1 || p1.M != frames * G1::OPIX || p2.M != frames * G2::OPIX || p1.N > 32 ||
      p2.N > 64 || p1.K % (2 * Cfg::BK1) != 0 || p2.K % (2 * Cfg::BK2) != 0)
    return hipErrorInvalidValue;
  hipLaunchKernelGGL((gemm_p3c12_kernel<G1, G2, U8, BK1_, BK2_>), dim3(frames), dim3(Cfg::NT), Cfg::LDS, st, p1, p2,
                     frames, hbm_frames);
  return hipGetLastError();
}

}
}
```

### acme_amd/csrc/gemm_p3i_geom.h

```cpp
#pragma once

#include "conv_geom.h"

#if defined(__HIPCC__)
#define ACME_GEOM_FN __host__ __device__ static __forceinline__
#else
#define ACME_GEOM_FN static inline
#endif

namespace acme {
namespace gemm {

constexpr int kImgZeroBytes = 256;

constexpr int img_zero_base(int bytes) { return (bytes + 255) & ~255; }

constexpr int img_pitch(int n, int opix) { return n + (((opix - n) % 16) + 16) % 16; }

template <class G, bool DGRAD>
struct ImgGeom {
  static constexpr int H = DGRAD ? G::OH : G::IH, W = DGRAD ? G::OW : G::IW;
  static constexpr int C = DGRAD ? G::CO : G::CI;
  static constexpr int OH = DGRAD ? G::IH : G::OH, OW = DGRAD ? G::IW : G::OW;
  static constexpr int S = DGRAD ? 1 : G::S;
// ... 1 lines not shown
  static constexpr int OPIX = OH * OW, IPIX = H * W;
  static constexpr int CPX = C / 8;
  static constexpr int SWZ = CPX == 8 ? 1 : 2;
  static constexpr int CH = (H + S - 1) / S, CW = (W + S - 1) / S;
  static constexpr int FPITCH = img_pitch(S * S * CH * CW, OPIX);
  static constexpr int UNITS = IPIX * CPX, IMG = FPITCH * 2 * C;
  static_assert(!DGRAD || G::S == 1, "strided input gradients are not image-resident");
  static_assert(C == 32 || C == 64, "a 32-k group must stay within one tap");
  static_assert(S == 1 || S == 2, "stride 1 or 2");
  static_assert(CW == OW, "class pitch = output pitch: a tap's positions are row + constant");
  ACME_GEOM_FN int dh(int kh) { return DGRAD ? G::PT - kh : kh - G::PT; }
  ACME_GEOM_FN int dw(int kw) { return DGRAD ? G::PL - kw : kw - G::PL; }
  ACME_GEOM_FN int pix(int fr, int ih, int iw) {
    if constexpr (S == 1) return fr * FPITCH + ih * CW + iw;
    else return fr * FPITCH + ((ih & 1) * 2 + (iw & 1)) * (CH * CW) + (ih >> 1) * CW + (iw >> 1);
  }
  ACME_GEOM_FN int swz(int q) { return (q >> SWZ) & (CPX - 1); }
  ACME_GEOM_FN int at(int fr, int ih, int iw, int c) {
    const int q = pix(fr, ih, iw);
    return q * (2 * C) + 16 * (c ^ swz(q));
  }
  ACME_GEOM_FN int fill(int f, int u) {
    const int px = u / CPX, c = u - px * CPX;
    const int ih = px / W, iw = px - ih * W;
    return at(f, ih, iw, c);
  }
  struct Lane {
    int f, ih, iw;
    bool ok;
  };
  ACME_GEOM_FN Lane lane(int f, int pp, bool ok) {
    const int oh = pp / OW, ow = pp - oh * OW;
    return Lane{f, oh * S, ow * S, ok};
  }
  struct Stage {
    int base, x;
  };
  ACME_GEOM_FN Stage stage(const Lane& l, int k0, int zero) {
    const int tap = k0 / C;
    const int kh = tap / KW, kw = tap - kh * KW;
    const int ih = l.ih + dh(kh), iw = l.iw + dw(kw);
    const bool in = l.ok && (unsigned)ih < (unsigned)H && (unsigned)iw < (unsigned)W;
    const int q = pix(l.f, ih, iw);
    const int b = q * (2 * C);
    return Stage{in ? b : zero + (b & 255), swz(q)};
  }
  ACME_GEOM_FN int unit(const Stage& st, const Lane&, int k0, int s, int h) {
    const int c = ((k0 % C) >> 3) + 2 * s + h;
    return st.base + 16 * (c ^ st.x);
  }
};

template <class G>
struct ImgGeomPairs {
  static constexpr int UNIT = 16;
  static constexpr int H = G::IH, W = G::IW;
  static constexpr int OW = G::OW, OPIX = G::OPIX;
  static constexpr int PAIRS = W / 2;
  static constexpr int SR = G::S, SC = G::S / 2;
  static constexpr int CH = (H + SR - 1) / SR, CW = (PAIRS + SC - 1) / SC;
  static constexpr int FPITCH = img_pitch(SR * SC * CH * CW, OPIX);
  static constexpr int UNITS = H * PAIRS, IMG = FPITCH * UNIT;
  static_assert(G::CI == 4 && G::KW * G::CI == 32, "4 channels, one kernel row per group");
  static_assert(W % 2 == 0 && G::S % 2 == 0 && G::PL % 2 == 0, "pairs never straddle the border");
  static_assert((SR & (SR - 1)) == 0 && (SC & (SC - 1)) == 0, "power-of-two classes");
  static_assert(CW == OW, "class pitch = output pitch: a tap's positions are row + constant");
  ACME_GEOM_FN int row_pos(int fr, int ih) {
    const int cr = ih & (SR - 1);
    return fr * FPITCH + cr * SC * (CH * CW) + (ih - cr) / SR * CW;
  }
  ACME_GEOM_FN int pos(int rp, int pw) {
    const int cc = pw & (SC - 1);
    return rp + cc * (CH * CW) + (pw - cc) / SC;
  }
  ACME_GEOM_FN int fill(int f, int u) {
    const int ih = u / PAIRS, pw = u - ih * PAIRS;
    return pos(row_pos(f, ih), pw) * UNIT;
  }
  struct Lane {
    int f, ih, iw;
    bool ok;
  };
  ACME_GEOM_FN Lane lane(int f, int pp, bool ok) {
    const int oh = pp / OW, ow = pp - oh * OW;
    return Lane{f, oh * G::S - G::PT, ow * G::S - G::PL, ok};
  }
  struct Stage {
    int rp;
    bool in;
    int zero;
  };
  ACME_GEOM_FN Stage stage(const Lane& l, int k0, int zero) {
    const int ih = l.ih + k0 / 32;
    return Stage{row_pos(l.f, ih), l.ok && (unsigned)ih < (unsigned)H, zero};
  }
  ACME_GEOM_FN int unit(const Stage& st, const Lane& l, int, int s, int h) {
    const int iw = l.iw + 4 * s + 2 * h;
    const int q = pos(st.rp, (iw - (iw & 1)) / 2);
    const int a = q * UNIT;
    return st.in && (unsigned)iw < (unsigned)W ? a : st.zero + (a & 255);
  }
};

template <class G>
struct ImgGeomSub {
  static constexpr int S = G::S, CLASSES = S * S;
  static constexpr int H = G::OH, W = G::OW, C = G::CO;
  static constexpr int JW = G::KW / S, KR = (G::KH / S) * JW * C;
  static constexpr int CPX = C / 8;
  static constexpr int SWZ = CPX == 8 ? 1 : 2;
  static constexpr int UNITS = H * W * CPX, IMG = H * W * 2 * C;
  static_assert(C == 32 || C == 64, "a 32-k group must stay within one tap");
  struct Cls {
    int ph, pw, rh, rw, nh, nw;
  };
  ACME_GEOM_FN Cls cls(int z) {
    const int ph = z / S, pw = z % S;
    const int rh = ((ph - G::PT) % S + S) % S, rw = ((pw - G::PL) % S + S) % S;
    return Cls{ph, pw, rh, rw, (G::IH - rh + S - 1) / S, (G::IW - rw + S - 1) / S};
  }
  ACME_GEOM_FN int swz(int q) { return (q >> SWZ) & (CPX - 1); }
  ACME_GEOM_FN int fill(int f, int u) {
    const int q = u / CPX, c = u - q * CPX;
    return f * IMG + q * (2 * C) + 16 * (c ^ swz(q));
  }
  struct Lane {
    int f, oh0, ow0;
    bool ok;
  };
  ACME_GEOM_FN Lane lane(int f, int z, int lr, bool ok) {
    const Cls k = cls(z);
    const bool in = ok && lr < k.nh * k.nw;
    const int i = in ? lr / k.nw : 0, j = in ? lr - i * k.nw : 0;
    return Lane{f, (k.rh + S * i + G::PT - k.ph) / S, (k.rw + S * j + G::PL - k.pw) / S, in};
  }
  struct Stage {
    int base, x;
  };
  ACME_GEOM_FN Stage stage(const Lane& l, int k0, int zero) {
    constexpr int T = JW * C;
    const int jh = k0 / T, jw = (k0 - jh * T) / C;
    const int oh = l.oh0 - jh, ow = l.ow0 - jw;
    const bool in = l.ok && (unsigned)oh < (unsigned)H && (unsigned)ow < (unsigned)W;
    const int q = oh * W + ow;
    const int b = l.f * IMG + q * (2 * C);
    return in ? Stage{b, swz(q)} : Stage{zero, 0};
  }
  ACME_GEOM_FN int unit(const Stage& st, const Lane&, int k0, int s, int h) {
    const int c = ((k0 % C) >> 3) + 2 * s + h;
    return st.base + 16 * (c ^ st.x);
  }
};

}
}
```

### acme_amd/csrc/torso.h

```cpp
#pragma once

#include <hip/hip_runtime.h>

#include <cstdint>

#include "conv.h"

namespace acme {
struct FusedUpdateArgs;
namespace gemm {
struct PScale;
}
namespace torso {

using G1 = conv::Geom<84, 84, 4, 21, 21, 32, 8, 8, 4, 2, 2>;
using G2 = conv::Geom<21, 21, 32, 11, 11, 64, 4, 4, 2, 1, 1>;
using G3 = conv::Geom<11, 11, 64, 11, 11, 64, 3, 3, 1, 1, 1>;
constexpr int kFlat = 11 * 11 * 64;
constexpr int kObsBytes = 84 * 84 * 4;
constexpr int kX1 = G1::OPIX * G1::CO;

struct Weights {
  const float *w1, *b1, *w2, *b2, *w3, *b3;
};
struct Grads {
  float *w1, *b1, *w2, *b2, *w3, *b3;
};
struct Acts {
  float *x1, *x2, *x3;
};

int64_t wgrad_slab_floats();

int forward(const Weights& w, bool u8, const void* obs_a, const void* obs_b, int split, int rows,
            const Acts& a, hipStream_t st);

int backward(const Weights& w, const Grads& g, bool u8, const void* obs, int rows, const Acts& a,
             const float* dz3, float* dz2, float* dz1, float* slab, hipStream_t st);

struct Plane {
  uint16_t* p;
  int64_t stride;
  gemm::PScale* sc;
};
struct PWeights {
  Plane w1, w2, w3;
  const float *b1, *b2, *b3;
};
extern uint64_t* g_stamps_conv[3];

struct PActs {
  Plane x1, x2, x3;
};
int64_t wgrad_slab_floats_p3();
struct Frames {
  const void* p;
  bool u8 = false;
  const void* p2 = nullptr;
  int split = 1 << 30;
  Frames rows_from(int r) const {
    if (!u8) return Frames{static_cast<const uint8_t*>(p) + (size_t)r * kObsBytes * 2};
    if (r >= split)
      return Frames{static_cast<const uint8_t*>(p2) + (size_t)(r - split) * kObsBytes, true};
    return Frames{static_cast<const uint8_t*>(p) + (size_t)r * kObsBytes, true, p2, split - r};
  }
};
int forward_p3(const PWeights& w, const Frames& frames, int rows, const PActs& a,
               hipStream_t st, int keep_x1 = -1, bool bk32 = false);
struct WgradSlab {
  const float* slab = nullptr;
  int splits = 0;
  int64_t wcount = 0, bcount = 0;
};
struct Side {
  hipStream_t side = nullptr;
  float* slab = nullptr;
  hipEvent_t e[3] = {nullptr, nullptr, nullptr};
  float* slab2 = nullptr;
  WgradSlab* defer = nullptr;
  bool conv1_single = false;
  bool bk32 = false;
};
int backward_p3(const PWeights& w, const Grads& g, const Frames& frames, int rows,
                const PActs& a, const Plane& dz3, const Plane& dz2, const Plane& dz1, float* slab,
                hipStream_t st, const Side& side = Side());
int backward_p3_convs(const PWeights& w, const Grads& g, int rows, const PActs& a,
                      const Plane& dz3, const Plane& dz2, const Plane& dz1, float* slab,
                      hipStream_t st, const Side& side);
int backward_p3_conv1(const Grads& g, const Frames& frames, int rows, const Plane& dz1,
                      float* slab, hipStream_t st, const Side& side,
                      const FusedUpdateArgs* rider = nullptr);
int backward_p3_join(hipStream_t st, const Side& side);

}
}
```

### acme_amd/csrc/torso.hip

```cpp
#include "torso.h"

#include <algorithm>

#include "common.h"
#include "conv_p3.h"
#include "gemm.h"
#include "gemm_p3.h"
#include "gemm_p3i.h"
#include "gemm_p3s.h"
#include "gemm_p3c12.h"
#include "gemm_x6.h"
#include "kernels.h"
#include "launch.h"
#include "plane_guard.h"
#include "prio_update.h"
#include "profiler.h"

namespace acme {
namespace torso {

using namespace acme::conv;
using acme::gemm::launch_gemm;

namespace {

constexpr int kConv1WgradSplits = 256, kConv2WgradSplits = 64, kConv3WgradSplits = 64;

template <class G, class In, int BM, int BN, int WM, int WN>
int conv_wgrad(const typename In::T* x, const float* dz, int rows, int splits, float* slab,
               float* dw, float* db, const char* name, const char* rname, hipStream_t st) {
  ConvWgrad<G, In> p;
  p.M = G::K; p.N = G::CO; p.K = rows * G::OPIX; p.k_chunk = chunk_for(p.K, splits);
  p.x = x; p.dz = dz; p.slab = slab;
  ACME_GEMM(name, BM, BN, WM, WN, 16, 1, p, splits);
  const int64_t count = (int64_t)(p.M + 1) * p.N;
  ACME_PROF(rname, st, 0.0, 4.0 * (double)(splits + 1) * (double)count);
  return launch_slab_reduce(slab, splits, count, dw, (int64_t)p.M * p.N, db, nullptr, 0, 0, st);
}

}

int64_t wgrad_slab_floats() {
  return std::max<int64_t>({(int64_t)kConv1WgradSplits * (G1::K + 1) * G1::CO,
                            (int64_t)kConv2WgradSplits * (G2::K + 1) * G2::CO,
                            (int64_t)kConv3WgradSplits * (G3::K + 1) * G3::CO});
}

int forward(const Weights& w, bool u8, const void* obs_a, const void* obs_b, int split, int rows,
            const Acts& a, hipStream_t st) {
  if (u8) {
    ConvFwd<G1, InU8> p;
    p.M = rows * G1::OPIX; p.N = G1::CO; p.K = G1::K; p.k_chunk = G1::K;
    p.x = static_cast<const uint8_t*>(obs_a); p.x2 = static_cast<const uint8_t*>(obs_b);
    p.split_b = split; p.w = w.w1; p.bias = w.b1; p.y = a.x1;
    ACME_GEMM("conv1_fwd", 128, 32, 4, 1, 16, 1, p, 1);
  } else {
    ConvFwd<G1, InF32> p;
    p.M = rows * G1::OPIX; p.N = G1::CO; p.K = G1::K; p.k_chunk = G1::K;
    p.x = static_cast<const float*>(obs_a); p.x2 = static_cast<const float*>(obs_b);
    p.split_b = split; p.w = w.w1; p.bias = w.b1; p.y = a.x1;
    ACME_GEMM("conv1_fwd", 128, 32, 4, 1, 16, 1, p, 1);
  }
  {
    ConvFwd<G2, InF32> p;
    p.M = rows * G2::OPIX; p.N = G2::CO; p.K = G2::K; p.k_chunk = G2::K;
    p.x = a.x1; p.x2 = a.x1; p.split_b = rows; p.w = w.w2; p.bias = w.b2; p.y = a.x2;
    ACME_GEMM("conv2_fwd", 128, 64, 2, 2, 16, 1, p, 1);
  }
  {
    ConvFwd<G3, InF32> p;
    p.M = rows * G3::OPIX; p.N = G3::CO; p.K = G3::K; p.k_chunk = G3::K;
    p.x = a.x2; p.x2 = a.x2; p.split_b = rows; p.w = w.w3; p.bias = w.b3; p.y = a.x3;
    ACME_GEMM("conv3_fwd", 128, 64, 2, 2, 16, 1, p, 1);
  }
  return ACME_OK;
}

int backward(const Weights& w, const Grads& g, bool u8, const void* obs, int rows, const Acts& a,
             const float* dz3, float* dz2, float* dz1, float* slab, hipStream_t st) {
  int rc;
  if ((rc = conv_wgrad<G3, InF32, 64, 64, 2, 2>(a.x2, dz3, rows, kConv3WgradSplits, slab, g.w3,
                                                g.b3, "conv3_wgrad", "conv3_wgrad_reduce", st)))
    return rc;
  {
    ConvDgrad<G3> p;
    p.M = rows * G3::IPIX; p.N = G3::CI; p.K = G3::KH * G3::KW * G3::CO; p.k_chunk = p.K;
    p.dz = dz3; p.w = w.w3; p.xprev = a.x2; p.dx = dz2;
    ACME_GEMM("conv3_dgrad", 128, 64, 2, 2, 16, 1, p, 1);
  }
  if ((rc = conv_wgrad<G2, InF32, 64, 64, 2, 2>(a.x1, dz2, rows, kConv2WgradSplits, slab, g.w2,
                                                g.b2, "conv2_wgrad", "conv2_wgrad_reduce", st)))
    return rc;
  {
    ConvDgradSubZ<G2> p;
    p.M = ConvDgradSubZ<G2>::max_rows(rows); p.N = G2::CI; p.K = ConvDgradSubZ<G2>::KR;
    p.k_chunk = p.K; p.batch = rows;
    p.dz = dz2; p.w = w.w2; p.xprev = a.x1; p.dx = dz1;
    ACME_GEMM_F("conv2_dgrad", 2.0 * rows * G2::IPIX * G2::CI * (double)p.K, 256, 32, 4, 1, 16,
                1, p, G2::S * G2::S);
  }
  if (u8)
    return conv_wgrad<G1, InU8, 128, 32, 4, 1>(static_cast<const uint8_t*>(obs), dz1, rows,
                                               kConv1WgradSplits, slab, g.w1, g.b1,
                                               "conv1_wgrad", "conv1_wgrad_reduce", st);
  return conv_wgrad<G1, InF32, 128, 32, 4, 1>(static_cast<const float*>(obs), dz1, rows,
                                              kConv1WgradSplits, slab, g.w1, g.b1, "conv1_wgrad",
                                              "conv1_wgrad_reduce", st);
}

namespace {

constexpr int kP3Conv1WgradSplits = 512, kP3Conv2WgradSplits = 128, kP3Conv3WgradSplits = 128;
constexpr int kP3MaxWgradSplits = 512;

using I1F = gemm::ImgGeomPairs<G1>;
using I2F = gemm::ImgGeom<G2, false>;
using I3F = gemm::ImgGeom<G3, false>;
using I3D = gemm::ImgGeom<G3, true>;
#define P3I_GEMM(name, GI, FPB, BN, WM, WN, MT, BK, prob, frames)                             \
  ACME_LAUNCH_GEMM(name, ACME_MNK_FLOPS(prob), gemm::p3_peak_tflops<decltype(prob)>(),        \
                   (gemm::launch_gemm_p3i<GI, FPB, BN, WM, WN, MT, BK>(prob, frames, st)))
#define P3I_GEMM_BK(name, GI, FPB, BN, WM, WN, MT, BK, bk32, prob, frames) \
  do {                                                                     \
    if (bk32) P3I_GEMM(name, GI, FPB, BN, WM, WN, MT, 32, prob, frames);   \
    else P3I_GEMM(name, GI, FPB, BN, WM, WN, MT, BK, prob, frames);        \
  } while (0)

constexpr int kBkConv1 = 64, kBkConv2 = 64, kBkConv3 = 32;
constexpr int kBkConv3Dgrad = 128, kBkConv2Dgrad = 32;
constexpr int kBkFused1 = 32, kBkFused2 = 64;

inline PlaneSrc frames_src(const Frames& f, int rows) {
  return PlaneSrc{static_cast<const uint16_t*>(f.p), 0,
                  (int32_t)((f.u8 ? 1 : 2) * (int64_t)rows * G1::IPIX * G1::CI)};
}

template <bool U8>
int conv1_fwd_p3(const PWeights& w, const Frames& frames, int rows, const Planes& y,
                 hipStream_t st, bool bk32, uint64_t* stamps = nullptr) {
  P3ConvFwd<G1, 1, U8> p;
  p.stamps = stamps;
  p.M = rows * G1::OPIX; p.N = G1::CO; p.K = G1::K; p.k_chunk = G1::K;
  const int n1 = U8 ? std::min(rows, frames.split) : rows;
  p.a_src = frames_src(frames, n1); p.b_src = SRC(w.w1, G1::K * G1::CO);
  if (U8 && n1 < rows) {
    p.a_src2 = frames_src(frames.rows_from(n1), rows - n1);
    p.a_split = n1;
  }
  p.bias = w.b1; p.y = y;
  P3I_GEMM_BK("conv1_fwd", I1F, 1, 32, 7, 1, 2, kBkConv1, bk32, p, rows);
  return ACME_OK;
}

template <bool U8>
int conv12_fwd_p3(const PWeights& w, const Frames& frames, int rows, int nsep, const PActs& a,
                  hipStream_t st, bool bk32) {
  const int nf = rows - nsep;
  const Frames fr = frames.rows_from(nsep);
  if (U8 && fr.split < nf)
    return (set_error("the fused conv1 -> conv2 forward reads its frames from one buffer"),
            ACME_ERR_INVALID);
  P3ConvFwd<G1, 1, U8> p1;
  p1.M = nf * G1::OPIX; p1.N = G1::CO; p1.K = G1::K; p1.k_chunk = G1::K;
  p1.a_src = frames_src(fr, nf); p1.b_src = SRC(w.w1, G1::K * G1::CO);
  p1.bias = w.b1;
  p1.y = Planes{a.x1.p + (int64_t)nsep * kX1, a.x1.stride, a.x1.sc};
  P3ConvFwd<G2, gemm::kPlanes> p2;
  p2.M = nf * G2::OPIX; p2.N = G2::CO; p2.K = G2::K; p2.k_chunk = G2::K;
  p2.a_src = SRC(a.x1, (int64_t)rows * kX1); p2.b_src = SRC(w.w2, G2::K * G2::CO);
  p2.bias = w.b2;
  p2.y = Planes{a.x2.p + (int64_t)nsep * kFlat, a.x2.stride, a.x2.sc};
  const double fl = 2.0 * p1.M * p1.N * (double)p1.K + 2.0 * p2.M * p2.N * (double)p2.K;
  ACME_PROF_PEAK("conv12_fwd", st, fl, 0.0, gemm::p3_peak_tflops<decltype(p2)>());
  hipError_t e = bk32 ? gemm::launch_gemm_p3c12<32, 32>(p1, p2, nf, 0, st)
                      : gemm::launch_gemm_p3c12<kBkFused1, kBkFused2>(p1, p2, nf, 0, st);
  if (e != hipSuccess) return (set_error("gemm launch failed: %s", hipGetErrorString(e)), ACME_ERR_HIP);
  return ACME_OK;
}

template <class P>
int p3_wgrad_reduce(const P& p, int splits, float* slab, float* dw, float* db, const char* rname,
                    hipStream_t st) {
  const int64_t count = (int64_t)(p.M + 1) * p.N;
  ACME_PROF(rname, st, 0.0, 4.0 * (double)(splits + 1) * (double)count);
  return launch_slab_reduce(slab, splits, count, dw, (int64_t)p.M * p.N, db, nullptr, 0, 0, st);
}

template <bool U8>
int conv1_wgrad_p3(const Grads& g, const Frames& frames, int rows, const Plane& dz1, float* slab,
                   hipStream_t st, const Side& sd, const FusedUpdateArgs* rider) {
  if (U8 && frames.split < rows)
    return (set_error("conv1's weight gradient reads its frames from one buffer"),
            ACME_ERR_INVALID);
  const int splits = kP3Conv1WgradSplits;
  P3ConvWgrad<G1, 1, U8> p;
  p.M = G1::K; p.N = G1::CO; p.K = rows * G1::OPIX;
  p.k_chunk = chunk_for(p.K, splits);
  p.a_src = frames_src(frames, rows); p.b_src = SRC(dz1, (int64_t)rows * kX1);
  p.slab = slab;
  if (rider && !sd.conv1_single)
    return (set_error("the update rider needs conv1's single-role kernel"), ACME_ERR_INVALID);
  if (rider)
    ACME_LAUNCH_GEMM("conv1_wgrad", ACME_MNK_FLOPS(p), gemm::p3_peak_tflops<decltype(p)>(),
                     (gemm::launch_gemm_p3_rider<256, 32, 4, 1, 32, UpdateRider>(p, splits, *rider,
                                                                                 st)));
  else if (sd.conv1_single) ACME_P3_GEMM("conv1_wgrad", 256, 32, 4, 1, 32, p, splits);
  else ACME_P3WS_GEMM("conv1_wgrad", 256, 32, 4, 1, 32, p, splits);
  if (sd.defer) {
    sd.defer[0] = WgradSlab{slab, splits, (int64_t)p.M * p.N, p.N};
    return ACME_OK;
  }
  return p3_wgrad_reduce(p, splits, slab, g.w1, g.b1, "conv1_wgrad_reduce", st);
}

}

uint64_t* g_stamps_conv[3] = {nullptr, nullptr, nullptr};

int64_t wgrad_slab_floats_p3() {
  return std::max<int64_t>({(int64_t)kP3MaxWgradSplits * (G1::K + 1) * G1::CO,
                            (int64_t)kP3MaxWgradSplits * (G2::K + 1) * G2::CO,
                            (int64_t)kP3MaxWgradSplits * (G3::K + 1) * G3::CO});
}

int forward_p3(const PWeights& w, const Frames& frames, int rows, const PActs& a,
               hipStream_t st, int keep_x1, bool bk32) {
  const int nsep = keep_x1 == 0 ? 0 : rows;
  int rc;
  if (nsep < rows &&
      (rc = frames.u8 ? conv12_fwd_p3<true>(w, frames, rows, nsep, a, st, bk32)
                      : conv12_fwd_p3<false>(w, frames, rows, nsep, a, st, bk32)) != ACME_OK)
    return rc;
  if (nsep > 0 && (rc = frames.u8 ? conv1_fwd_p3<true>(w, frames, nsep, PP(a.x1), st, bk32, g_stamps_conv[0])
                                  : conv1_fwd_p3<false>(w, frames, nsep, PP(a.x1), st, bk32, g_stamps_conv[0])) != ACME_OK)
    return rc;
  if (nsep > 0) {
    P3ConvFwd<G2, gemm::kPlanes> p;
    p.M = nsep * G2::OPIX; p.N = G2::CO; p.K = G2::K; p.k_chunk = G2::K;
    p.a_src = SRC(a.x1, (int64_t)nsep * kX1); p.b_src = SRC(w.w2, G2::K * G2::CO);
    p.bias = w.b2; p.y = PP(a.x2);
    p.stamps = g_stamps_conv[1];
    P3I_GEMM_BK("conv2_fwd", I2F, 2, 64, 8, 2, 1, kBkConv2, bk32, p, nsep);
  }
  {
    P3ConvFwd<G3, gemm::kPlanes> p;
    p.M = rows * G3::OPIX; p.N = G3::CO; p.K = G3::K; p.k_chunk = G3::K;
    p.a_src = SRC(a.x2, (int64_t)rows * kFlat); p.b_src = SRC(w.w3, G3::K * G3::CO);
    p.bias = w.b3; p.y = PP(a.x3);
    if (keep_x1 != 0) p.stamps = g_stamps_conv[2];
    P3I_GEMM_BK("conv3_fwd", I3F, 1, 64, 4, 2, 1, kBkConv3, bk32, p, rows);
  }
  return ACME_OK;
}

int backward_p3_convs(const PWeights& w, const Grads& g, int rows, const PActs& a,
                      const Plane& dz3, const Plane& dz2, const Plane& dz1, float* slab,
                      hipStream_t st_main, const Side& sd) {
  int rc;
  const bool fork = sd.side != nullptr;
  const bool defer = sd.defer != nullptr;
  if (defer && !(sd.slab && sd.slab2))
    return (set_error("deferred weight gradients need two side slabs"), ACME_ERR_INVALID);
  hipStream_t st = fork ? sd.side : st_main;
  float* wslab = fork || defer ? sd.slab : slab;
  {
    if (fork) {
      ACME_HIP_TRY(hipEventRecord(sd.e[0], st_main));
      ACME_HIP_TRY(hipStreamWaitEvent(sd.side, sd.e[0], 0));
    }
    P3ConvWgrad<G3, gemm::kPlanes> p;
    p.M = G3::K; p.N = G3::CO; p.K = rows * G3::OPIX;
    const int splits = kP3Conv3WgradSplits;
    p.k_chunk = chunk_for(p.K, splits);
    p.a_src = SRC(a.x2, (int64_t)rows * kFlat); p.b_src = SRC(dz3, (int64_t)rows * kFlat);
    p.slab = wslab;
    ACME_P3_GEMM("conv3_wgrad", 128, 64, 2, 2, 32, p, splits);
    if (defer) sd.defer[2] = WgradSlab{wslab, splits, (int64_t)p.M * p.N, p.N};
    else if ((rc = p3_wgrad_reduce(p, splits, wslab, g.w3, g.b3, "conv3_wgrad_reduce", st)))
      return rc;
  }
  st = st_main;
  {
    P3ConvDgrad<G3> p;
    p.M = rows * G3::IPIX; p.N = G3::CI; p.K = G3::KH * G3::KW * G3::CO; p.k_chunk = p.K;
    p.a_src = SRC(dz3, (int64_t)rows * kFlat); p.b_src = SRC(w.w3, G3::K * G3::CO);
    p.xprev = CP(a.x2); p.dx = PP(dz2);
    P3I_GEMM_BK("conv3_dgrad", I3D, 2, 64, 8, 2, 1, kBkConv3Dgrad, sd.bk32, p, rows);
  }
  if (fork) {
    ACME_HIP_TRY(hipEventRecord(sd.e[1], st_main));
    ACME_HIP_TRY(hipStreamWaitEvent(sd.side, sd.e[1], 0));
    st = sd.side;
  }
  {
    P3ConvWgrad<G2, gemm::kPlanes> p;
    p.M = G2::K; p.N = G2::CO; p.K = rows * G2::OPIX;
    const int splits = kP3Conv2WgradSplits;
    p.k_chunk = chunk_for(p.K, splits);
    p.a_src = SRC(a.x1, (int64_t)rows * kX1); p.b_src = SRC(dz2, (int64_t)rows * kFlat);
    float* slab2 = defer ? sd.slab2 : wslab;
    p.slab = slab2;
    ACME_P3_GEMM("conv2_wgrad", 128, 64, 2, 2, 32, p, splits);
    if (defer) sd.defer[1] = WgradSlab{slab2, splits, (int64_t)p.M * p.N, p.N};
    else if ((rc = p3_wgrad_reduce(p, splits, slab2, g.w2, g.b2, "conv2_wgrad_reduce", st)))
      return rc;
    if (fork) ACME_HIP_TRY(hipEventRecord(sd.e[2], sd.side));
  }
  st = st_main;
  {
    P3ConvDgradSubZ<G2> p;
    p.M = P3ConvDgradSubZ<G2>::max_rows(rows); p.N = G2::CI; p.K = P3ConvDgradSubZ<G2>::KR;
    p.k_chunk = p.K; p.batch = rows;
    p.a_src = SRC(dz2, (int64_t)rows * kFlat); p.b_src = SRC(w.w2, G2::K * G2::CO);
    p.xprev = CP(a.x1); p.dx = PP(dz1);
    const double fl = 2.0 * rows * G2::IPIX * G2::CI * (double)p.K;
    ACME_PROF_PEAK("conv2_dgrad", st, fl, 0.0, gemm::p3_peak_tflops<decltype(p)>());
    hipError_t e = sd.bk32 ? gemm::launch_gemm_p3s<G2, 2, 32>(p, rows, st)
                           : gemm::launch_gemm_p3s<G2, 2, kBkConv2Dgrad>(p, rows, st);
    if (e != hipSuccess) return (set_error("gemm launch failed: %s", hipGetErrorString(e)), ACME_ERR_HIP);
  }
  return ACME_OK;
}

int backward_p3_conv1(const Grads& g, const Frames& frames, int rows, const Plane& dz1,
                      float* slab, hipStream_t st, const Side& sd, const FusedUpdateArgs* rider) {
  return frames.u8 ? conv1_wgrad_p3<true>(g, frames, rows, dz1, slab, st, sd, rider)
                   : conv1_wgrad_p3<false>(g, frames, rows, dz1, slab, st, sd, rider);
}

int backward_p3_join(hipStream_t st_main, const Side& sd) {
  if (sd.side) ACME_HIP_TRY(hipStreamWaitEvent(st_main, sd.e[2], 0));
  return ACME_OK;
}

int backward_p3(const PWeights& w, const Grads& g, const Frames& frames, int rows,
                const PActs& a, const Plane& dz3, const Plane& dz2, const Plane& dz1, float* slab,
                hipStream_t st, const Side& sd) {
  int rc = backward_p3_convs(w, g, rows, a, dz3, dz2, dz1, slab, st, sd);
  if (rc == ACME_OK) rc = backward_p3_conv1(g, frames, rows, dz1, slab, st, sd);
  if (rc == ACME_OK) rc = backward_p3_join(st, sd);
  return rc;
}

}
}
```

### acme_amd/native.py

```python

from __future__ import annotations

import ctypes
from typing import Dict, List, Optional, Sequence, Tuple

import numpy as np
import torch

from acme_amd import _lib
from acme_amd._lib import check, lib, ptr, stream_ptr

SAMPLER_UNIFORM = 0
SAMPLER_PRIORITIZED = 1


class NativeReplay:

    def __init__(self, capacity: int, field_bytes: Sequence[int], prioritized: bool,
                 priority_exponent: float = 0.6, seed: int = 1234, device=None):
        _lib.require_gpu()
        if len(field_bytes) > _lib.MAX_FIELDS:
            raise ValueError(f"at most {_lib.MAX_FIELDS} flattened fields per item")
        cfg = _lib.ReplayConfig()
        cfg.capacity = int(capacity)
# ... 351 lines not shown

    def _copy_in(self, flat: torch.Tensor, src: Dict[str, np.ndarray]) -> None:
        for name, t in self.views(flat).items():
            t.copy_(torch.as_tensor(np.asarray(src[name], np.float32)).view(t.shape))

    def set_params(self, params: Dict[str, np.ndarray], target: Optional[Dict] = None) -> None:
        self._copy_in(self.params, params)
        if self._has_target:
            self._copy_in(self.target, target if target is not None else params)
        self.params_changed()

    def get_params(self, which: str = "params") -> Dict[str, np.ndarray]:
        flat = getattr(self, which)
        return {k: v.detach().cpu().numpy().copy() for k, v in self.views(flat).items()}

    @property
    def num_steps(self) -> int:
        return int(self._fn("num_steps")(self._h))

    @num_steps.setter
    def num_steps(self, n: int) -> None:
        check(self._fn("set_num_steps")(self._h, int(n)))

    def debug_buffer(self, name: str) -> np.ndarray:
        return _debug_buffer(self._fn("debug_buffer"), self._h, name, self.device)

    def params_changed(self) -> None:
        """The params / target buffers were written from outside (nothing to do for a learner
        whose step reads the f32 buffers directly)."""

    def _sequence_batch(self, observation, prev_action, prev_reward, action, reward, discount,
                        h0, c0, behaviour_logits=None, core_state=True):
        B, T = int(action.shape[0]), int(action.shape[1])
        want = torch.uint8 if self.torso == "atari" else torch.float32
        checks = [("observation", observation, want), ("prev_action", prev_action, torch.int32),
                  ("prev_reward", prev_reward, torch.float32), ("action", action, torch.int32),
                  ("reward", reward, torch.float32), ("discount", discount, torch.float32)]
        if behaviour_logits is not None:
            checks.append(("behaviour_logits", behaviour_logits, torch.float32))
        for name, t, dt in checks:
            if not (isinstance(t, torch.Tensor) and t.is_cuda and t.is_contiguous()
                    and t.dtype == dt):
                raise ValueError(f"{name} must be a contiguous {dt} device tensor")
            if tuple(t.shape[:2]) != (B, T):
                raise ValueError(f"{name} has shape {tuple(t.shape)}, expected [{B}, {T}, ...]")
        b = _lib.SequenceBatch()
        b.observation, b.prev_action, b.prev_reward = ptr(observation), ptr(prev_action), ptr(prev_reward)
        b.action, b.reward, b.discount = ptr(action), ptr(reward), ptr(discount)
        b.behaviour_logits = ptr(behaviour_logits) if behaviour_logits is not None else None
        if core_state:
            for name, t in (("h0", h0), ("c0", c0)):
                if (t is None or t.dtype != torch.float32 or t.shape != (B, self.lstm_size)
                        or t.stride(1) != 1):
                    raise ValueError(f"{name} must be float32 [{B}, {self.lstm_size}] with unit "
                                     "inner stride")
            if h0.stride(0) != c0.stride(0):
                raise ValueError("h0 and c0 must share a row stride")
            b.h0, b.c0, b.state_stride = ptr(h0), ptr(c0), int(h0.stride(0))
        else:
            b.h0 = b.c0 = None
            b.state_stride = self.lstm_size
        b.batch, b.sequence_length = B, T
        return b


class _PlaneState:

    def params_changed(self) -> None:
        check(self._fn("params_changed")(self._h), f"{self._tag} params_changed")

    def scale_state(self) -> np.ndarray:
        n = ctypes.c_int32(0)
        fn, what = self._fn("scale_state"), f"{self._tag} scale_state"
        check(fn(self._h, None, 0, ctypes.byref(n)), what)
        out = np.zeros(n.value, np.float32)
        if n.value:
            check(fn(self._h, out.ctypes.data, n.value, ctypes.byref(n)), what)
        return out

    def set_scale_state(self, state) -> None:
        a = np.ascontiguousarray(np.asarray(state, np.float32))
        if a.size:
            check(self._fn("set_scale_state")(self._h, a.ctypes.data, a.size),
                  f"{self._tag} set_scale_state")

    @property
    def skipped_steps(self) -> int:
        return int(self._fn("skipped_steps")(self._h))


def _plane_overflow(self, reset: bool = False) -> bool:
    v = ctypes.c_int32(0)
    check(self._fn("plane_overflow")(self._h, ctypes.byref(v), int(reset)),
          f"{self._tag} plane_overflow")
    return bool(v.value)


class NativeDQN(_PlaneState, _NativeLearner):

    _prefix, _tag = "acme_dqn", "dqn"
    plane_overflow = _plane_overflow

    def __init__(self, *, network: str, num_actions: int, max_batch: int, obs_dtype: str,
                 obs_dim: int = 0, hidden: Sequence[int] = (), discount: float = 0.99,
                 importance_sampling_exponent: float = 0.2, learning_rate: float = 1e-3,
                 huber_loss_parameter: float = 1.0, target_update_period: int = 100,
                 max_abs_reward: float = 1.0, adam_beta1: float = 0.9, adam_beta2: float = 0.999,
                 adam_epsilon: float = 1e-8, semantics: str = "tf", device=None):
        _lib.require_gpu()
        if semantics not in ("tf", "jax"):
            raise ValueError(f"semantics must be 'tf' or 'jax', got {semantics!r}")
        if huber_loss_parameter < 0:
            raise ValueError("quadratic_linear_boundary must be >= 0.")
        cfg = _lib.DQNConfig()
        cfg.network = NET_NATURE if network == "nature" else NET_MLP
        cfg.obs_dtype = OBS_U8 if obs_dtype == "uint8" else OBS_F32
        cfg.num_actions = int(num_actions)
        cfg.max_batch = int(max_batch)
        cfg.obs_dim = int(obs_dim)
        if len(hidden) > _lib.MAX_MLP_LAYERS:
            raise ValueError(f"at most {_lib.MAX_MLP_LAYERS} hidden layers")
        cfg.num_hidden = len(hidden)
        for i, h in enumerate(hidden):
            cfg.hidden[i] = int(h)
        cfg.discount = discount
        cfg.importance_sampling_exponent = importance_sampling_exponent
        cfg.learning_rate = learning_rate
        cfg.huber_loss_parameter = huber_loss_parameter
        cfg.adam_beta1, cfg.adam_beta2, cfg.adam_epsilon = adam_beta1, adam_beta2, adam_epsilon
        cfg.target_update_period = int(target_update_period)
        cfg.max_abs_reward = max_abs_reward
        cfg.semantics = _lib.SEMANTICS_JAX if semantics == "jax" else _lib.SEMANTICS_TF
        self.semantics = semantics
        self.network = network
        self.num_actions = int(num_actions)
        self.max_batch = int(max_batch)
        self._create(cfg, device)
        self.num_params = int(lib().acme_dqn_num_params(self._h))
        d = self.device
        self.loss = torch.zeros(1, dtype=torch.float32, device=d)
        self.td_error = torch.zeros(max_batch, dtype=torch.float32, device=d)
        self.priorities = torch.zeros(max_batch, dtype=torch.float64, device=d)

    def guard_state(self) -> Dict[str, int]:
        a = (ctypes.c_int64 * 4)()
        check(lib().acme_dqn_guard_state(self._h, a), "dqn guard_state")
        t = ctypes.c_int64()
        check(lib().acme_dqn_verdict_timeouts(self._h, ctypes.byref(t)), "dqn verdict_timeouts")
        return dict(applied=int(a[0]), skipped=int(a[1]), last_skipped=int(a[2]),
                    q_values_overflowed=int(a[3]), verdict_timeouts=int(t.value))

    def update_rider_launches(self) -> int:
        return int(lib().acme_dqn_update_rider_launches(self._h))

    @property
    def applied_steps(self) -> int:
        return self.guard_state()["applied"]

    @applied_steps.setter
    def applied_steps(self, n: int) -> None:
        check(lib().acme_dqn_set_applied_steps(self._h, int(n)), "dqn set_applied_steps")

    @property
    def skip_word(self) -> Optional[int]:
        p = ctypes.c_void_p()
        check(lib().acme_dqn_skip_word(self._h, ctypes.byref(p)), "dqn skip_word")
        return p.value

    def set_reissue(self, enable: bool) -> None:
        check(lib().acme_dqn_set_reissue(self._h, 1 if enable else 0), "dqn set_reissue")

    @property
    def verdicts_issued(self) -> int:
        return int(lib().acme_dqn_verdicts_issued(self._h))

    def step_verdict(self, seq: int) -> Optional[bool]:
        v = ctypes.c_int32(-1)
        check(lib().acme_dqn_step_verdict(self._h, int(seq), ctypes.byref(v)), "dqn step_verdict")
        return None if v.value < 0 else bool(v.value)

    def set_data_parallel_gate(self, enable: bool) -> None:
        check(lib().acme_dqn_set_data_parallel_gate(self._h, 1 if enable else 0), "dqn dp gate")

    def _batch(self, o_tm1, a_tm1, r_t, d_t, o_t, probabilities, global_min_probability=None,
               mean_over=None, obs_f16=None):
        B = int(a_tm1.shape[0])
        if B < 1 or B > self.max_batch:
            raise ValueError(f"batch of {B} rows: the learner takes 1..{self.max_batch}")
        for name, t in (("o_tm1", o_tm1), ("a_tm1", a_tm1), ("r_t", r_t), ("d_t", d_t),
                        ("o_t", o_t), ("probabilities", probabilities)):
            if not (isinstance(t, torch.Tensor) and t.is_cuda and t.is_contiguous()):
                raise ValueError(f"{name} must be a contiguous device tensor")
            if t.shape[0] != B:
                raise ValueError(f"{name} has leading dim {t.shape[0]}, expected {B}")
        if a_tm1.dtype != torch.int32 or r_t.dtype != torch.float32 or d_t.dtype != torch.float32:
            raise ValueError("a_tm1 must be int32, r_t and d_t float32")
        if probabilities.dtype != torch.float64:
            raise ValueError("probabilities must be float64")
        want = torch.uint8 if self.cfg.obs_dtype == OBS_U8 else torch.float32
        if o_tm1.dtype != want or o_t.dtype != want:
            raise ValueError(f"observations must be {want}")
        tb = _lib.TransitionBatch()
        tb.o_tm1, tb.a_tm1, tb.r_t, tb.d_t, tb.o_t = (ptr(o_tm1), ptr(a_tm1), ptr(r_t), ptr(d_t),
                                                      ptr(o_t))
        tb.probabilities = ptr(probabilities)
        tb.batch = B
        tb.global_min_probability = ptr(global_min_probability)
        tb.mean_over = int(mean_over or 0)
        if obs_f16 is not None:
            if not (isinstance(obs_f16, torch.Tensor) and obs_f16.is_cuda and
                    obs_f16.dtype in (torch.int16, torch.uint16, torch.float16) and
                    obs_f16.is_contiguous() and obs_f16.shape[0] >= 2 * B and
                    obs_f16[0].numel() == o_tm1[0].numel()):
                raise ValueError("obs_f16 must be a contiguous [2B, obs] 16-bit device tensor")
            tb.obs_f16 = ptr(obs_f16)
        return tb

    @staticmethod
    def _event_handle(ev) -> Optional[int]:
        if ev is None:
            return None
        return ev.handle if hasattr(ev, "handle") else int(ev.cuda_event)

    def _outputs(self, q_tm1=None):
        o = _lib.DQNOutputs()
        o.loss, o.td_error, o.priorities = ptr(self.loss), ptr(self.td_error), ptr(self.priorities)
        o.q_tm1 = ptr(q_tm1)
        return o

    def forward_backward(self, *batch, global_min_probability=None, q_tm1=None, stream=None):
        tb = self._batch(*batch, global_min_probability=global_min_probability)
        out = self._outputs(q_tm1)
        check(lib().acme_dqn_forward_backward(self._h, ctypes.byref(tb), ctypes.byref(out),
                                              stream_ptr(stream)), "dqn forward_backward")

    def forward_backward_stage(self, stage: int, *batch, global_min_probability=None,
                               q_tm1=None, stream=None, mean_over=None, obs_f16=None,
                               inputs_event=None):
        tb = self._batch(*batch, global_min_probability=global_min_probability,
                         mean_over=mean_over, obs_f16=obs_f16)
        tb.inputs_event = self._event_handle(inputs_event)
        out = self._outputs(q_tm1)
        check(lib().acme_dqn_forward_backward_stage(self._h, ctypes.byref(tb), ctypes.byref(out),
                                                    int(stage), stream_ptr(stream)),
              f"dqn forward_backward stage {stage}")

    def dense_grads_ready(self, stream=None) -> None:
        check(lib().acme_dqn_dense_grads_ready(self._h, stream_ptr(stream)), "dense grads ready")

    def dp_init(self, comm, world_size: int) -> None:
        check(lib().acme_dqn_dp_init(self._h, ctypes.c_void_p(comm), int(world_size)), "dp init")

    def dp_step(self, *batch, mean_over=None, q_tm1=None, stream=None, obs_f16=None):
        tb = self._batch(*batch, mean_over=mean_over, obs_f16=obs_f16)
        out = self._outputs(q_tm1)
        check(lib().acme_dqn_dp_step(self._h, ctypes.byref(tb), ctypes.byref(out),
                                     stream_ptr(stream)), "dqn dp step")

    @property
    def grad_split(self) -> int:
        s = ctypes.c_int64()
        check(lib().acme_dqn_grad_split(self._h, ctypes.byref(s)))
        return int(s.value)

    def batch_min_probability(self, probabilities: torch.Tensor, out: torch.Tensor, stream=None):
        check(lib().acme_min_f64(ptr(probabilities), int(probabilities.numel()), ptr(out),
                                 stream_ptr(stream)), "min_f64")

    def apply(self, stream=None):
        check(lib().acme_dqn_apply(self._h, stream_ptr(stream)), "dqn apply")

    def step(self, *batch, q_tm1=None, stream=None, obs_f16=None, priority_update=None,
             inputs_event=None):
        tb = self._batch(*batch, obs_f16=obs_f16)
        tb.inputs_event = self._event_handle(inputs_event)
        out = self._outputs(q_tm1)
        if priority_update is None:
            check(lib().acme_dqn_step(self._h, ctypes.byref(tb), ctypes.byref(out),
                                      stream_ptr(stream)), "dqn step")
            return
        handle, keys, after = (tuple(priority_update) + (None,))[:3]
        if keys.dtype not in (torch.uint64, torch.int64) or not keys.is_contiguous():
            raise ValueError("priority_update keys must be a contiguous 64-bit tensor")
        if keys.numel() != int(tb.batch) or not keys.is_cuda:
            raise ValueError("priority_update keys must hold one key per batch row, on the "
                             "learner's device")
        check(lib().acme_dqn_step_update(self._h, ctypes.byref(tb), ctypes.byref(out), handle,
                                         ptr(keys), after, stream_ptr(stream)), "dqn step")

    def q_values(self, obs: torch.Tensor, use_target: bool = False, stream=None) -> torch.Tensor:
        B = int(obs.shape[0])
        q = torch.empty(B, self.num_actions, dtype=torch.float32, device=self.device)
        check(lib().acme_dqn_q_values(self._h, ptr(obs.contiguous()), B, 1 if use_target else 0,
                                      ptr(q), stream_ptr(stream)), "dqn q_values")
        return q


def nccl_unique_id() -> bytes:
    buf = (ctypes.c_uint8 * 128)()
    check(lib().acme_nccl_get_unique_id(buf), "nccl unique id")
    return bytes(buf)


def nccl_comm_init(uid: bytes, world_size: int, rank: int) -> int:
    buf = (ctypes.c_uint8 * 128).from_buffer_copy(uid)
    comm = ctypes.c_void_p()
# ... 399 lines not shown
```

### include/acme_hip.h

```cpp
#ifndef ACME_HIP_H_
#define ACME_HIP_H_

#include <stdint.h>

#ifdef __cplusplus
extern "C" {
#endif

typedef enum acme_status {
  ACME_OK = 0,
  ACME_ERR_INVALID = -1,
  ACME_ERR_HIP = -2,
  ACME_ERR_EMPTY = -3,
  ACME_ERR_OOM = -4
} acme_status;

const char* acme_last_error(void);

int acme_tune_set(const char* key, int32_t value);
const char* acme_version(void);
const char* acme_target_arch(void);

int acme_event_create(void** ev);
int acme_event_destroy(void* ev);
// ... 20 lines not shown
  int64_t capacity;
  int32_t sampler;
  int32_t num_fields;
  double priority_exponent;
  uint64_t seed;
  int64_t field_bytes[ACME_MAX_FIELDS];
} acme_replay_config;

typedef struct acme_replay acme_replay;

int acme_replay_create(const acme_replay_config* cfg, acme_replay** out);
int acme_replay_destroy(acme_replay* r);

int acme_replay_insert(acme_replay* r, const void* const* fields, int64_t n,
                       const double* priorities, int32_t src_on_device,
                       uint64_t* out_keys, void* stream);

int64_t acme_replay_stage_capacity(acme_replay* r);
int acme_replay_stage(acme_replay* r, int64_t n, void** field_ptrs);
int acme_replay_commit(acme_replay* r, int64_t n, const double* priorities, uint64_t* out_keys,
                       void* stream);
int acme_replay_sync_inserts(acme_replay* r);
int acme_host_register(void* p, int64_t bytes);
int acme_host_unregister(void* p);

typedef struct acme_nstep_writer acme_nstep_writer;
int acme_nstep_writer_create(acme_replay* r, int32_t n_step, float discount, int64_t obs_bytes,
                             int64_t action_bytes, int64_t rows_per_chunk,
                             acme_nstep_writer** out);
int acme_nstep_writer_destroy(acme_nstep_writer* w);
int acme_nstep_writer_start(acme_nstep_writer* w, const void* observation);
int acme_nstep_writer_add(acme_nstep_writer* w, const void* action, float reward,
                          float discount, const void* next_observation, int32_t last,
                          double priority);
int acme_nstep_writer_flush(acme_nstep_writer* w);
int acme_nstep_writer_reset(acme_nstep_writer* w);
int64_t acme_nstep_writer_pending(acme_nstep_writer* w);

int acme_replay_fill_synthetic(acme_replay* r, int64_t n, int32_t layout,
                               int32_t num_actions, uint64_t seed, void* stream);

int acme_replay_sample(acme_replay* r, int64_t batch, uint64_t step_counter,
                       int64_t* slots, uint64_t* keys, double* probabilities,
                       int64_t* table_size, double* priorities, void* stream);

int acme_replay_gather(acme_replay* r, const int64_t* slots, int64_t batch,
                       void* const* out_fields, void* stream);

int acme_replay_sample_gather(acme_replay* r, int64_t batch, uint64_t step_counter,
                              int64_t* slots, uint64_t* keys, double* probabilities,
                              int64_t* table_size, double* priorities, void* const* out_fields,
                              void* stream);

int acme_replay_sample_gather_frames(acme_replay* r, int64_t batch, uint64_t step_counter,
                                     int64_t* slots, uint64_t* keys, double* probabilities,
                                     int64_t* table_size, double* priorities,
                                     void* const* out_fields, uint16_t* frames_f16,
                                     void* stream);

int acme_replay_pipe_open(acme_replay* r, int32_t* pipe);
int acme_replay_pipe_close(acme_replay* r, int32_t pipe);
int acme_replay_pipe_flush(acme_replay* r, int32_t pipe);
int acme_replay_sample_gather_pipe(acme_replay* r, int32_t pipe, int64_t batch,
                                   uint64_t step_counter, int64_t* slots, uint64_t* keys,
                                   double* probabilities, int64_t* table_size,
                                   double* priorities, void* const* out_fields, void* stream);

int acme_replay_total(acme_replay* r, double* out, void* stream);
int acme_replay_sample_share(acme_replay* r, int64_t batch, uint64_t step_counter,
                             double prob_scale, int64_t* slots, uint64_t* keys,
                             double* probabilities, int64_t* table_size, double* priorities,
                             void* const* out_fields, void* stream);
int acme_replay_sample_share_frames(acme_replay* r, int64_t batch, uint64_t step_counter,
                                    double prob_scale, int64_t* slots, uint64_t* keys,
                                    double* probabilities, int64_t* table_size,
                                    double* priorities, void* const* out_fields,
                                    uint16_t* frames_f16, void* stream);

int acme_frames_expand(const uint8_t* frames, int64_t num_frames, int64_t frame_bytes,
                       int32_t stack, const int32_t* idx, int64_t batch, uint8_t* out,
                       void* stream);

int acme_r2d2_priorities(const float* errors, int32_t T, int32_t B, double eta, double* out,
                         void* stream);
int acme_r2d2_importance_weights(const double* probabilities, int32_t B,
                                 int64_t max_replay_size, double beta, float* out,
                                 void* stream);

int acme_replay_update_priorities(acme_replay* r, const uint64_t* keys,
                                  const double* priorities, int64_t n, void* stream);
int acme_replay_update_priorities_gated(acme_replay* r, const uint64_t* keys,
                                        const double* priorities, int64_t n,
                                        const uint32_t* skip_word, void* stream);

int64_t acme_replay_size(const acme_replay* r);
int64_t acme_replay_capacity(const acme_replay* r);
int acme_replay_debug_leaves(const acme_replay* r, const double** leaf_values,
                             const double** raw_priorities, const uint64_t** keys);
int acme_replay_debug_level(const acme_replay* r, int32_t level, const double** values,
                            int64_t* count, int32_t* nlevels);

int acme_replay_storage(acme_replay* r, int32_t field, void** out);
int64_t acme_replay_inserted(const acme_replay* r);
int acme_replay_restore(acme_replay* r, int64_t inserted, void* stream);


enum { ACME_NET_NATURE_DQN = 0, ACME_NET_MLP = 1 };
enum { ACME_SEMANTICS_TF = 0, ACME_SEMANTICS_JAX = 1 };
enum { ACME_OBS_U8_SCALED = 0, ACME_OBS_F32 = 1 };

#define ACME_MAX_MLP_LAYERS 8

typedef struct acme_dqn_config {
  int32_t network;
  int32_t obs_dtype;
  int32_t num_actions;
  int32_t max_batch;
  int32_t obs_dim;
  int32_t num_hidden;
  int32_t hidden[ACME_MAX_MLP_LAYERS];
  float discount;
  float importance_sampling_exponent;
  float learning_rate;
  float huber_loss_parameter;
  float adam_beta1, adam_beta2, adam_epsilon;
  int32_t target_update_period;
  float max_abs_reward;
  int32_t semantics;
} acme_dqn_config;

typedef struct acme_dqn acme_dqn;

int acme_dqn_create(const acme_dqn_config* cfg, acme_dqn** out);
int acme_dqn_destroy(acme_dqn* l);
int64_t acme_dqn_num_params(const acme_dqn* l);
int64_t acme_dqn_flat_size(const acme_dqn* l);
int32_t acme_dqn_num_tensors(const acme_dqn* l);
int acme_dqn_tensor_info(const acme_dqn* l, int32_t i, int64_t* offset, int64_t* numel,
                         int32_t* ndim, int64_t* shape4, const char** name);

int acme_dqn_bind(acme_dqn* l, float* params, float* target, float* grads, float* adam_m,
                  float* adam_v);
int acme_dqn_params_changed(acme_dqn* l);
int acme_dqn_plane_overflow(acme_dqn* l, int32_t* overflow, int32_t reset);
int64_t acme_dqn_skipped_steps(const acme_dqn* l);
int acme_dqn_guard_state(acme_dqn* l, int64_t* out4);
int acme_dqn_set_applied_steps(acme_dqn* l, int64_t n);
int acme_dqn_skip_word(const acme_dqn* l, const uint32_t** out);
int acme_dqn_set_data_parallel_gate(acme_dqn* l, int32_t enable);
int acme_dqn_set_reissue(acme_dqn* l, int32_t enable);
int acme_dqn_verdict_timeouts(acme_dqn* l, int64_t* out);
int64_t acme_dqn_verdicts_issued(const acme_dqn* l);
int64_t acme_dqn_update_rider_launches(const acme_dqn* l);
int acme_dqn_step_verdict(const acme_dqn* l, int64_t seq, int32_t* state);
int acme_dqn_scale_state(const acme_dqn* l, float* out, int32_t capacity, int32_t* count);
int acme_dqn_set_scale_state(acme_dqn* l, const float* in, int32_t count);

typedef struct acme_transition_batch {
  const void* o_tm1;
  const int32_t* a_tm1;
  const float* r_t;
  const float* d_t;
  const void* o_t;
  const double* probabilities;
  int64_t batch;
  const double* global_min_probability;
  int64_t mean_over;
  const uint16_t* obs_f16;
  void* inputs_event;
} acme_transition_batch;

typedef struct acme_dqn_outputs {
  float* loss;
  float* td_error;
  double* priorities;
  float* q_tm1;
} acme_dqn_outputs;

int acme_dqn_forward_backward(acme_dqn* l, const acme_transition_batch* batch,
                              const acme_dqn_outputs* out, void* stream);
int acme_dqn_forward_backward_stage(acme_dqn* l, const acme_transition_batch* batch,
                                    const acme_dqn_outputs* out, int32_t stage, void* stream);
int acme_dqn_grad_split(const acme_dqn* l, int64_t* split);
int acme_dqn_dense_grads_ready(acme_dqn* l, void* stream);
int acme_dqn_dp_init(acme_dqn* l, void* nccl_comm, int32_t world_size);
int acme_dqn_dp_step(acme_dqn* l, const acme_transition_batch* batch,
                     const acme_dqn_outputs* out, void* stream);
int acme_nccl_get_unique_id(uint8_t* out128);
int acme_nccl_comm_init(const uint8_t* id128, int32_t world_size, int32_t rank, void** comm);
int acme_nccl_comm_destroy(void* comm);
int acme_dqn_apply(acme_dqn* l, void* stream);
int acme_dqn_step(acme_dqn* l, const acme_transition_batch* batch,
                  const acme_dqn_outputs* out, void* stream);
int acme_dqn_step_update(acme_dqn* l, const acme_transition_batch* batch,
                         const acme_dqn_outputs* out, acme_replay* replay,
                         const uint64_t* keys, void* after_event, void* stream);
int acme_dqn_q_values(acme_dqn* l, const void* obs, int64_t batch, int32_t use_target,
                      float* q_out, void* stream);
int64_t acme_dqn_num_steps(const acme_dqn* l);
int acme_dqn_debug_buffer(const acme_dqn* l, const char* name, const float** out,
                          int64_t* count);
int acme_dqn_set_num_steps(acme_dqn* l, int64_t n);
int acme_min_f64(const double* x, int64_t n, double* out_dev, void* stream);

#define ACME_D4PG_MAX_LAYERS 4
#define ACME_D4PG_MAX_ACT 16
#define ACME_D4PG_MAX_ATOMS 64

typedef struct acme_d4pg acme_d4pg;

typedef struct acme_d4pg_config {
  int32_t obs_dim;
  int32_t act_dim;
  int32_t max_batch;
  int32_t num_policy_layers;
  int32_t policy_sizes[ACME_D4PG_MAX_LAYERS];
  int32_t num_critic_layers;
  int32_t critic_sizes[ACME_D4PG_MAX_LAYERS];
  int32_t num_atoms;
  float vmin, vmax;
  float action_min[ACME_D4PG_MAX_ACT];
  float action_max[ACME_D4PG_MAX_ACT];
  float discount;
  int32_t target_update_period;
  float policy_learning_rate, critic_learning_rate;
  float adam_beta1, adam_beta2, adam_epsilon;
  int32_t clipping;
  float layer_norm_epsilon;
} acme_d4pg_config;

typedef struct acme_d4pg_batch {
  const float* o_tm1;
  const float* a_tm1;
  const float* r_t;
  const float* d_t;
  const float* o_t;
  int64_t batch;
} acme_d4pg_batch;

typedef struct acme_d4pg_outputs {
  float* critic_loss;
  float* policy_loss;
} acme_d4pg_outputs;

int acme_d4pg_create(const acme_d4pg_config* cfg, acme_d4pg** out);
int acme_d4pg_destroy(acme_d4pg* l);
int64_t acme_d4pg_flat_size(const acme_d4pg* l);
int64_t acme_d4pg_policy_size(const acme_d4pg* l);
int32_t acme_d4pg_num_tensors(const acme_d4pg* l);
int acme_d4pg_tensor_info(const acme_d4pg* l, int32_t i, int64_t* offset, int64_t* numel,
                          int32_t* ndim, int64_t* shape4, const char** name);
int acme_d4pg_bind(acme_d4pg* l, float* params, float* target, float* grads, float* adam_m,
                   float* adam_v);
int acme_d4pg_step(acme_d4pg* l, const acme_d4pg_batch* batch, const acme_d4pg_outputs* out,
                   void* stream);
int acme_d4pg_policy(acme_d4pg* l, const float* obs, int64_t rows, int32_t use_target,
                     float* actions, void* stream);
int64_t acme_d4pg_num_steps(const acme_d4pg* l);
int acme_d4pg_set_num_steps(acme_d4pg* l, int64_t n);
int acme_d4pg_debug_buffer(const acme_d4pg* l, const char* name, const float** out,
                           int64_t* count);

typedef struct acme_ddpg acme_ddpg;

typedef struct acme_ddpg_config {
  int32_t obs_dim;
  int32_t act_dim;
  int32_t max_batch;
  int32_t num_policy_layers;
  int32_t policy_sizes[ACME_D4PG_MAX_LAYERS];
  int32_t num_critic_layers;
  int32_t critic_sizes[ACME_D4PG_MAX_LAYERS];
  float action_min[ACME_D4PG_MAX_ACT];
  float action_max[ACME_D4PG_MAX_ACT];
  float discount;
  int32_t target_update_period;
  float policy_learning_rate, critic_learning_rate;
  float adam_beta1, adam_beta2, adam_epsilon;
  int32_t clipping;
  float layer_norm_epsilon;
} acme_ddpg_config;

typedef acme_d4pg_batch acme_ddpg_batch;
typedef acme_d4pg_outputs acme_ddpg_outputs;

int acme_ddpg_create(const acme_ddpg_config* cfg, acme_ddpg** out);
int acme_ddpg_destroy(acme_ddpg* l);
int64_t acme_ddpg_flat_size(const acme_ddpg* l);
int64_t acme_ddpg_policy_size(const acme_ddpg* l);
int32_t acme_ddpg_num_tensors(const acme_ddpg* l);
int acme_ddpg_tensor_info(const acme_ddpg* l, int32_t i, int64_t* offset, int64_t* numel,
                          int32_t* ndim, int64_t* shape4, const char** name);
int acme_ddpg_bind(acme_ddpg* l, float* params, float* target, float* grads, float* adam_m,
                   float* adam_v);
int acme_ddpg_step(acme_ddpg* l, const acme_ddpg_batch* batch, const acme_ddpg_outputs* out,
                   void* stream);
int acme_ddpg_policy(acme_ddpg* l, const float* obs, int64_t rows, int32_t use_target,
                     float* actions, void* stream);
int64_t acme_ddpg_num_steps(const acme_ddpg* l);
int acme_ddpg_set_num_steps(acme_ddpg* l, int64_t n);
int acme_ddpg_debug_buffer(const acme_ddpg* l, const char* name, const float** out,
                           int64_t* count);

#define ACME_MPO_MAX_SAMPLES 64
#define ACME_MPO_MAX_ROWS 131072

// ... 241 lines not shown
```

Baseline: 1.068 million transitions/s.

## Fuse conv3 forward into conv1-2 and conv2 kernels via LDS-resident x2

Adds a fused conv1->conv2->conv3 kernel for the target forward and a fused conv2->conv3 kernel for the online forward. The conv2 activation stays in LDS, and the HBM write of x2 is done only for the rows needed for backward (keep_x2). This removes a separate conv3 launch and the x2 round trip through HBM. In exchange, LDS placement gets tighter, which may lower occupancy, and the fused path requires an even frame count. It is enabled by default through the FUSE_X2 tune knob.

Result: faster. 1.099 million transitions/s, median of 6 (+2.9%).

```diff
diff --git a/acme_amd/_lib.py b/acme_amd/_lib.py
--- a/acme_amd/_lib.py
+++ b/acme_amd/_lib.py
@@ -244,6 +244,7 @@
     "acme_dqn_guard_state": (c_i32, [c_vp, ctypes.POINTER(c_i64)]),
     "acme_dqn_verdict_timeouts": (c_i32, [c_vp, ctypes.POINTER(c_i64)]),
     "acme_dqn_update_rider_launches": (c_i64, [c_vp]),
+    "acme_dqn_fused_x2_launches": (c_i64, [c_vp]),
     "acme_dqn_set_applied_steps": (c_i32, [c_vp, c_i64]),
     "acme_dqn_skip_word": (c_i32, [c_vp, ctypes.POINTER(c_vp)]),
     "acme_dqn_set_reissue": (c_i32, [c_vp, c_i32]),
diff --git a/acme_amd/csrc/dqn.hip b/acme_amd/csrc/dqn.hip
--- a/acme_amd/csrc/dqn.hip
+++ b/acme_amd/csrc/dqn.hip
@@ -115,6 +115,8 @@
   bool bk32 = false;
   bool update_rider = true;
   int64_t rider_launches = 0;
+  int fuse_x2 = torso::kFuseX2Default;
+  int64_t fused_x2_launches = 0;
   bool frames_u8 = true;
   int64_t seq = 0;
   uint32_t* host_verdicts = nullptr;
@@ -249,9 +251,10 @@
 int nature_forward_p3(acme_dqn* l, const float* prm, uint16_t* wpl, const torso::Frames& frames,
                       int rows, const torso::Plane& x1, const torso::Plane& x2,
                       const torso::Plane& x3, float* hid, float* q, hipStream_t st,
-                      float* slab = nullptr, int keep_x1 = -1, bool defer_head = false) {
+                      float* slab = nullptr, int keep_x1 = -1, bool defer_head = false,
+                      int keep_x2 = -1) {
   if (!slab) slab = l->slab;
-  int rc = torso::forward_p3(torso_pweights(l, prm, wpl), frames, rows, torso::PActs{x1, x2, x3}, st, keep_x1, l->bk32);
+  int rc = torso::forward_p3(torso_pweights(l, prm, wpl), frames, rows, torso::PActs{x1, x2, x3}, st, keep_x1, l->bk32, keep_x2);
   if (rc != ACME_OK) return rc;
   {
     P3DenseFwd p;
@@ -587,6 +590,7 @@
   l->single_role = tune_variant("WSN") == 1;
   l->bk32 = tune_variant("BK32") == 1;
   l->update_rider = tune_variant("UPDATE_RIDER", kUpdateRiderDefault) != 0;
+  l->fuse_x2 = tune_variant("FUSE_X2", torso::kFuseX2Default) & 3;
   l->stamps_on = tune_variant("STAMPS") == 1;
   const int A = cfg->num_actions;
   const int B = cfg->max_batch;
@@ -803,6 +807,7 @@
 }
 
 int64_t acme_dqn_update_rider_launches(const acme_dqn* l) { return l ? l->rider_launches : 0; }
+int64_t acme_dqn_fused_x2_launches(const acme_dqn* l) { return l ? l->fused_x2_launches : 0; }
 
 int acme_dqn_set_reissue(acme_dqn* l, int32_t enable) {
   ACME_CHECK_ARG(l, "null learner");
@@ -1082,13 +1087,15 @@
       l->target_dirty = true;
     }
     const bool online_first = side != nullptr;
+    const int keep_on = (l->fuse_x2 & 2) ? B : -1, keep_tg = (l->fuse_x2 & 1) ? 0 : -1;
+    l->fused_x2_launches += (keep_on >= 0) + (keep_tg >= 0);
     if (online_first &&
         (rc = nature_forward_p3(l, l->params, l->wpl, fwd_frames, 2 * B, l->x1p, l->x2p, l->x3p,
-                                l->hid, l->q_on, st, nullptr, B, true)) != ACME_OK)
+                                l->hid, l->q_on, st, nullptr, B, true, keep_on)) != ACME_OK)
       return rc;
     if ((rc = nature_forward_p3(l, l->target, l->tpl, fwd_frames.rows_from(B), B,
                                 l->t1p, l->t2p, l->t3p, l->thid, l->q_tg, tst,
-                                side ? l->tslab : l->slab, 0)) != ACME_OK)
+                                side ? l->tslab : l->slab, 0, false, keep_tg)) != ACME_OK)
       return rc;
     {
       RescaleGuard rg;
@@ -1102,7 +1109,7 @@
     if (side) ACME_HIP_TRY(hipEventRecord(l->ev[1], side));
     if (!online_first &&
         (rc = nature_forward_p3(l, l->params, l->wpl, fwd_frames, 2 * B, l->x1p, l->x2p, l->x3p,
-                                l->hid, l->q_on, st, nullptr, B, true)) != ACME_OK)
+                                l->hid, l->q_on, st, nullptr, B, true, keep_on)) != ACME_OK)
       return rc;
     if (side) ACME_HIP_TRY(hipStreamWaitEvent(st, l->ev[1], 0));
   } else if (nature) {
diff --git a/acme_amd/csrc/gemm_p3c12.h b/acme_amd/csrc/gemm_p3c12.h
--- a/acme_amd/csrc/gemm_p3c12.h
+++ b/acme_amd/csrc/gemm_p3c12.h
@@ -6,41 +6,147 @@
 namespace acme {
 namespace gemm {
 
-template <class G1, class G2, bool U8 = false>
-struct P3C1ToLds {
-  using Base = conv::P3ConvFwd<G1, 1, U8>;
-  using I2 = ImgGeom<G2, false>;
+template <class Gfrom, class Gto, int NPA, bool U8 = false, int FPB = 1>
+struct P3ConvToLds {
+  using Base = conv::P3ConvFwd<Gfrom, NPA, U8>;
   static constexpr int A_MODE = Base::A_MODE, B_MODE = Base::B_MODE;
-  static constexpr int A_PLANES = 1, B_PLANES = kPlanes;
+  static constexpr int A_PLANES = NPA, B_PLANES = kPlanes;
   static constexpr bool kStore8 = true;
   static constexpr bool kAmax = true;
   int M, N, K, k_chunk;
   Base base;
-  uint8_t* x1;
+  uint8_t* img;
   int plane;
   int m0;
-  bool hbm;
+  int hbm_rows;
   __device__ PScale* amax_sc() const { return base.y.sc; }
-  __device__ float store8(int m, int n, const conv::V8& acc, int) const {
+  using Pre = typename Base::Pre;
+  __device__ Pre pre(int n) const { return base.pre(n); }
+  __device__ float store8p(int m, int n, const conv::V8& acc, int, const Pre& q) const {
     conv::V8 v;
-    base.act8(n, acc, v);
+#pragma unroll
+    for (int j = 0; j < 8; ++j) {
+      float x = acc[j] * q.rs;
+      if constexpr (NPA == 1) x = x / 255.0f;
+      x += q.b[j];
+      v[j] = x > 0.f ? x : 0.f;
+    }
     uint32_t h[4], l[4];
-    const float mx = conv::split8(v, base.y.w(), h, l);
-    const int pp = m - m0, oh = pp / G1::OW, ow = pp - oh * G1::OW;
-    const int a = I2::at(0, oh, ow, n / 8);
-    *reinterpret_cast<u32x4*>(x1 + a) = u32x4{h[0], h[1], h[2], h[3]};
-    *reinterpret_cast<u32x4*>(x1 + plane + a) = u32x4{l[0], l[1], l[2], l[3]};
-    if (hbm) {
-      const int64_t e = (int64_t)m * G1::CO + n;
+    const float mx = conv::split8(v, q.w, h, l);
+    int pp = m - m0, f = 0;
+    if constexpr (FPB > 1) {
+      f = pp / Gfrom::OPIX;
+      pp -= f * Gfrom::OPIX;
+    }
+    const int a = sink_at<Gfrom, Gto>(f, pp, n);
+    *reinterpret_cast<u32x4*>(img + a) = u32x4{h[0], h[1], h[2], h[3]};
+    *reinterpret_cast<u32x4*>(img + plane + a) = u32x4{l[0], l[1], l[2], l[3]};
+    if (m < hbm_rows) {
+      const int64_t e = (int64_t)m * Gfrom::CO + n;
       *reinterpret_cast<uint4*>(base.y.p + e) = uint4{h[0], h[1], h[2], h[3]};
       *reinterpret_cast<uint4*>(base.y.p + base.y.stride + e) = uint4{l[0], l[1], l[2], l[3]};
     }
     return mx;
   }
 };
-
-template <class G1, class G2, bool U8 = false, int BK1_ = 32, int BK2_ = 32>
+template <class G1, class G2, bool U8 = false>
+using P3C1ToLds = P3ConvToLds<G1, G2, 1, U8, 1>;
+
+template <class GI, int NT_, int WM, int WN, int BK_, class P, class PQ>
+struct P3ImgPhase {
+  static constexpr int NT = NT_, GK = 32, KS = 2, BK = BK_, NG = BK / GK, NP = kPlanes;
+  static_assert(NT == 64 * WM * WN && BK % GK == 0 && NG >= 1, "whole waves, whole 32-k groups");
+  static_assert(P::A_PLANES == NP && P::B_PLANES == NP, "two-plane operands");
+  using C = P3Core<WM * 32, 64, WM, WN, GK, PQ>;
+  using PB = typename C::PB;
+  static_assert(NG * PB::UNITS <= NT, "one weight unit per thread per plane and stage");
+  static constexpr int RING = 2 * NG * PB::BYTES;
+  struct Ring {
+    bool own;
+    int g, u;
+    typename P::BRow br;
+    __amdgpu_buffer_rsrc_t sb[NP];
+    u32x4 r[2][NP];
+  };
+  __device__ static __forceinline__ void init(Ring& w, const P& p, int tid) {
+    w.own = tid < NG * PB::UNITS;
+    w.g = tid / PB::UNITS;
+    w.u = tid % PB::UNITS;
+    w.br = p.b_row(w.own ? PB::row_of(w.u) : 0);
+#pragma unroll
+    for (int pl = 0; pl < NP; ++pl) w.sb[pl] = plane_rsrc(p.b_src, pl);
+  }
+  template <int SET>
+  __device__ static __forceinline__ void fetch(Ring& w, const P& p, int k0) {
+    const int kg = k0 + w.g * GK;
+    const uint32_t off = w.own && kg < p.K ? p.b_off(w.br, kg, PB::kk_of(w.u)) : kOOB;
+#pragma unroll
+    for (int pl = 0; pl < NP; ++pl)
+      w.r[SET][pl] = __builtin_bit_cast(u32x4, __builtin_amdgcn_raw_buffer_load_b128(w.sb[pl], off, 0, 0));
+  }
+  template <int SET>
+  __device__ static __forceinline__ void stash(const Ring& w, uint8_t* ring, int buf) {
+    if (!w.own) return;
+    uint8_t* s = ring + (buf * NG + w.g) * PB::BYTES + PB::offset(w.u);
+#pragma unroll
+    for (int pl = 0; pl < NP; ++pl) *reinterpret_cast<u32x4*>(s + pl * PB::PLANE) = w.r[SET][pl];
+  }
+  __device__ static __forceinline__ void kloop(const P& p, Ring& w, uint8_t* ring,
+                                               const uint8_t* img, int plane, int zero, int rows,
+                                               int wm, int wn, int lane, typename C::Acc& acc) {
+    const int lr = wm * 32 + (lane & 31);
+    const int f = lr / GI::OPIX;
+    const typename GI::Lane ln = GI::lane(f, lr - f * GI::OPIX, lr < rows);
+    stash<0>(w, ring, 0);
+    __syncthreads();
+    auto group = [&](int k0, const uint8_t* sb) {
+      const typename GI::Stage sg = GI::stage(ln, k0, zero);
+      f16x8 fb[KS][NP], fa[KS][NP];
+#pragma unroll
+      for (int s = 0; s < KS; ++s) {
+#pragma unroll
+        for (int pl = 0; pl < NP; ++pl) fb[s][pl] = PB::frag(sb, pl, wn * 32, s, lane);
+        const int a = GI::unit(sg, ln, k0, s, lane >> 5);
+#pragma unroll
+        for (int pl = 0; pl < NP; ++pl)
+          fa[s][pl] = *reinterpret_cast<const f16x8*>(img + pl * plane + a);
+      }
+      __builtin_amdgcn_sched_barrier(0);
+#pragma unroll
+      for (int s = 0; s < KS; ++s) acc.terms(0, 0, fa[s], fb[s]);
+    };
+    auto iter = [&](auto S, int kt) {
+      constexpr int set = decltype(S)::value;
+      stash<set ^ 1>(w, ring, (kt + 1) & 1);
+      fetch<set>(w, p, (kt + 2) * BK);
+      __builtin_amdgcn_sched_barrier(0);
+      const uint8_t* sb = ring + (kt & 1) * NG * PB::BYTES;
+#pragma unroll
+      for (int g = 0; g < NG; ++g) {
+        if (g > 0) {
+          if (kt * BK + g * GK >= p.K) break;
+          __builtin_amdgcn_sched_barrier(0);
+        }
+        group(kt * BK + g * GK, sb + g * PB::BYTES);
+      }
+      __syncthreads();
+    };
+    const int nk = (p.K + BK - 1) / BK;
+    int kt = 0;
+    for (; kt + 1 < nk; kt += 2) {
+      iter(std::integral_constant<int, 0>{}, kt);
+      iter(std::integral_constant<int, 1>{}, kt + 1);
+    }
+    if (kt < nk) iter(std::integral_constant<int, 0>{}, kt);
+  }
+};
+
+template <class G1, class G2, bool U8 = false, int BK1_ = 32, int BK2_ = 32, class G3 = void,
+          int BK3_ = 32>
 struct P3C12Cfg {
+  static constexpr bool C3 = !std::is_void<G3>::value;
+  using G3g = std::conditional_t<C3, G3, G2>;
+  using Place = C123Place<G1, G2, G3g, BK1_ / 32, BK2_ / 32, BK3_ / 32>;
   using I1 = ImgGeomPairs<G1>;
   using I2 = ImgGeom<G2, false>;
   using P1 = conv::P3ConvFwd<G1, 1, U8>;
@@ -68,13 +174,30 @@
                     C2::EPI_BYTES <= I1::IMG,
                 "conv2's ring and the epilogue staging reuse the frame image region");
   static_assert(G1::OPIX <= 512 && I2::OPIX <= 128 && P2::A_PLANES == NP, "geometry");
+  using I3 = ImgGeom<G3g, false>;
+  using P3 = conv::P3ConvFwd<G3g, kPlanes>;
+  using P2L = P3ConvToLds<G2, G3g, kPlanes>;
+  using C2L = P3Core<128, 64, 4, 2, GK, P2L>;
+  using Ph3 = P3ImgPhase<I3, NT, 4, 2, BK3_, P3, P3>;
+  static constexpr int X2 = Place::X2, ZERO3 = Place::ZERO3, PLANE3 = Place::PLANE3;
+  static_assert(Place::FRAME == FRAME && Place::X1 == X1 && Place::PLANE2 == PLANE2 &&
+                    Place::LDS == LDS && Place::ring1.lo == RING1 &&
+                    Place::ring1.hi == RING1 + 2 * NG1 * PB1::BYTES &&
+                    Place::ring2.hi == 2 * NG2 * PB2::BYTES && Place::epi1.hi == C1::EPI_BYTES &&
+                    Place::epi23.hi == C2::EPI_BYTES,
+                "C123Place describes this kernel");
+  static_assert(!C3 || (Place::ring3.hi == Ph3::RING && Place::epi23.hi == C2L::EPI_BYTES &&
+                        Place::epi23.hi == Ph3::C::EPI_BYTES && I3::OPIX <= 128),
+                "C123Place describes conv3's regions");
+  static_assert(Place::ok(), "no two live LDS regions overlap in any phase; under 160 KiB");
 };
 
-template <class G1, class G2, bool U8, int BK1_, int BK2_>
-__global__ void __launch_bounds__(512) gemm_p3c12_kernel(const conv::P3ConvFwd<G1, 1, U8> p1,
-                                                         const conv::P3ConvFwd<G2, kPlanes> p2,
-                                                         int frames, int hbm_frames) {
-  using Cfg = P3C12Cfg<G1, G2, U8, BK1_, BK2_>;
+template <class G1, class G2, bool U8, int BK1_, int BK2_, class G3 = void, int BK3_ = 32>
+__global__ void __launch_bounds__(512) gemm_p3c12_kernel(
+    const conv::P3ConvFwd<G1, 1, U8> p1, const conv::P3ConvFwd<G2, kPlanes> p2, int frames,
+    int hbm_frames, const typename P3C12Cfg<G1, G2, U8, BK1_, BK2_, G3, BK3_>::P3 p3,
+    int hbm2_frames) {
+  using Cfg = P3C12Cfg<G1, G2, U8, BK1_, BK2_, G3, BK3_>;
   using I1 = typename Cfg::I1;
   using I2 = typename Cfg::I2;
   using PB1 = typename Cfg::PB1;
@@ -228,7 +351,8 @@
     typename Cfg::P1L q;
     q.M = (f + 1) * G1::OPIX < p1.M ? (f + 1) * G1::OPIX : p1.M;
     q.N = p1.N; q.K = p1.K; q.k_chunk = p1.k_chunk;
-    q.base = p1; q.x1 = x1; q.plane = Cfg::PLANE2; q.m0 = f * G1::OPIX; q.hbm = f < hbm_frames;
+    q.base = p1; q.img = x1; q.plane = Cfg::PLANE2; q.m0 = f * G1::OPIX;
+    q.hbm_rows = f < hbm_frames ? q.M : 0;
     Cfg::C1::epilogue(q, smem, q.m0, 0, wave, wave, 0, lane, 0, acc, false);
   }
 
@@ -272,9 +396,34 @@
       iter(S0{}, kt);
       iter(S1{}, kt + 1);
     }
-    P2 q = p2;
-    q.M = (f + 1) * I2::OPIX < p2.M ? (f + 1) * I2::OPIX : p2.M;
-    Cfg::C2::epilogue(q, smem, f * I2::OPIX, 0, wave, wm, wn, lane, 0, acc, false);
+    const int m2 = (f + 1) * I2::OPIX < p2.M ? (f + 1) * I2::OPIX : p2.M;
+    if constexpr (!Cfg::C3) {
+      P2 q = p2;
+      q.M = m2;
+      Cfg::C2::epilogue(q, smem, f * I2::OPIX, 0, wave, wm, wn, lane, 0, acc, false);
+    } else {
+      using Ph3 = typename Cfg::Ph3;
+      using I3 = typename Cfg::I3;
+      uint8_t* x2 = smem + Cfg::X2;
+      if (tid < 16 * NP)
+        *reinterpret_cast<u32x4*>(x2 + (tid >> 4) * Cfg::PLANE3 + Cfg::ZERO3 + 16 * (tid & 15)) = zero_u4();
+      typename Ph3::Ring w3;
+      Ph3::init(w3, p3, tid);
+      Ph3::template fetch<0>(w3, p3, 0);
+      Ph3::template fetch<1>(w3, p3, Ph3::BK);
+      typename Cfg::P2L q;
+      q.M = m2; q.N = p2.N; q.K = p2.K; q.k_chunk = p2.k_chunk;
+      q.base = p2; q.img = x2; q.plane = Cfg::PLANE3; q.m0 = f * I2::OPIX;
+      q.hbm_rows = f < hbm2_frames ? m2 : 0;
+      Cfg::C2L::epilogue(q, smem, q.m0, 0, wave, wm, wn, lane, 0, acc, false);
+      typename Ph3::C::Acc acc3;
+      acc3.zero();
+      const typename Cfg::P3::Pre pre3 = p3.pre(wn * 32 + Ph3::C::epi_col(lane));
+      Ph3::kloop(p3, w3, smem, x2, Cfg::PLANE3, Cfg::ZERO3, I3::OPIX, wm, wn, lane, acc3);
+      typename Cfg::P3 q3 = p3;
+      q3.M = (f + 1) * I3::OPIX < p3.M ? (f + 1) * I3::OPIX : p3.M;
+      Ph3::C::epilogue(q3, smem, f * I3::OPIX, 0, wave, wm, wn, lane, 0, acc3, false, &pre3);
+    }
   }
 }
 
@@ -290,9 +439,142 @@
       p2.N > 64 || p1.K % (2 * Cfg::BK1) != 0 || p2.K % (2 * Cfg::BK2) != 0)
     return hipErrorInvalidValue;
   hipLaunchKernelGGL((gemm_p3c12_kernel<G1, G2, U8, BK1_, BK2_>), dim3(frames), dim3(Cfg::NT), Cfg::LDS, st, p1, p2,
-                     frames, hbm_frames);
+                     frames, hbm_frames, typename Cfg::P3{}, 0);
   return hipGetLastError();
 }
 
-}
-}
+template <int BK1_, int BK2_, int BK3_, class G1, class G2, class G3, bool U8>
+inline hipError_t launch_gemm_p3c123(const conv::P3ConvFwd<G1, 1, U8>& p1,
+                                     const conv::P3ConvFwd<G2, kPlanes>& p2,
+                                     const conv::P3ConvFwd<G3, kPlanes>& p3, int frames,
+                                     int hbm_frames, int hbm2_frames, hipStream_t st) {
+  using Cfg = P3C12Cfg<G1, G2, U8, BK1_, BK2_, G3, BK3_>;
+  static_assert(Cfg::LDS <= 160 * 1024, "LDS");
+  static hipError_t attr =
+      p3_set_lds(&gemm_p3c12_kernel<G1, G2, U8, BK1_, BK2_, G3, BK3_>, Cfg::LDS);
+  if (attr != hipSuccess) return attr;
+  if (frames < 1 || p1.M != frames * G1::OPIX || p2.M != frames * G2::OPIX ||
+      p3.M != frames * G3::OPIX || p1.N > 32 || p2.N != 64 || p3.N > 64 ||
+      p1.K % (2 * Cfg::BK1) != 0 || p2.K % (2 * Cfg::BK2) != 0 || p3.K % 32 != 0)
+    return hipErrorInvalidValue;
+  hipLaunchKernelGGL((gemm_p3c12_kernel<G1, G2, U8, BK1_, BK2_, G3, BK3_>), dim3(frames),
+                     dim3(Cfg::NT), Cfg::LDS, st, p1, p2, frames, hbm_frames, p3, hbm2_frames);
+  return hipGetLastError();
+}
+
+template <class G2, class G3, int BK2_, int BK3_>
+struct P3C23Cfg {
+  using Place = C23Place<G2, G3, BK2_ / 32, BK3_ / 32>;
+  using I2 = ImgGeom<G2, false>;
+  using I3 = ImgGeom<G3, false>;
+  using P2 = conv::P3ConvFwd<G2, kPlanes>;
+  using P3 = conv::P3ConvFwd<G3, kPlanes>;
+  static constexpr int NT = 1024, FPB = Place::FPB, NP = kPlanes;
+  using P2L = P3ConvToLds<G2, G3, kPlanes, false, FPB>;
+  using Ph2 = P3ImgPhase<I2, NT, 8, 2, BK2_, P2, P2L>;
+  using Ph3 = P3ImgPhase<I3, NT, 8, 2, BK3_, P3, P3>;
+  static constexpr int LDS = Place::LDS;
+  static_assert(FPB * I2::OPIX <= 256 && FPB * I3::OPIX <= 256, "8 waves of 32 rows cover the frames");
+  static_assert(Place::ring2.hi - Place::ring2.lo == Ph2::RING && Place::ring3.hi == Ph3::RING &&
+                    Place::EPI == Ph2::C::EPI_BYTES && Place::EPI == Ph3::C::EPI_BYTES,
+                "C23Place describes this kernel");
+  static_assert(Place::ok(), "no two live LDS regions overlap in any phase; under 160 KiB");
+};
+
+template <class G2, class G3, int BK2_, int BK3_>
+__global__ void __launch_bounds__(1024) gemm_p3c23_kernel(const conv::P3ConvFwd<G2, kPlanes> p2,
+                                                          const conv::P3ConvFwd<G3, kPlanes> p3,
+                                                          int frames, int hbm_frames) {
+  using Cfg = P3C23Cfg<G2, G3, BK2_, BK3_>;
+  using Place = typename Cfg::Place;
+  using I2 = typename Cfg::I2;
+  using I3 = typename Cfg::I3;
+  using Ph2 = typename Cfg::Ph2;
+  using Ph3 = typename Cfg::Ph3;
+  constexpr int NT = Cfg::NT, NP = Cfg::NP, FPB = Cfg::FPB;
+  extern __shared__ __attribute__((aligned(16))) uint8_t smem[];
+  const int tid = threadIdx.x, lane = tid & 63, wave = tid >> 6;
+  const int wm = wave >> 1, wn = wave & 1;
+  const int f0 = blockIdx.x * FPB;
+  const int nf = frames - f0 < FPB ? frames - f0 : FPB;
+
+  typename Ph2::Ring w2;
+  Ph2::init(w2, p2, tid);
+  Ph2::template fetch<0>(w2, p2, 0);
+  Ph2::template fetch<1>(w2, p2, Ph2::BK);
+
+  {
+    constexpr int UNITS = FPB * I2::UNITS;
+    constexpr int PER = (UNITS + NT - 1) / NT;
+    __amdgpu_buffer_rsrc_t srcA[NP];
+#pragma unroll
+    for (int pl = 0; pl < NP; ++pl) srcA[pl] = plane_rsrc(p2.a_src, pl);
+    u32x4 v[PER][NP];
+#pragma unroll
+    for (int j = 0; j < PER; ++j) {
+      const int u = tid + j * NT;
+      const bool ok = u < UNITS && u / I2::UNITS < nf;
+      const uint32_t off = ok ? (uint32_t)(((int64_t)f0 * I2::UNITS + u) * 16) : kOOB;
+#pragma unroll
+      for (int pl = 0; pl < NP; ++pl)
+        v[j][pl] = __builtin_bit_cast(u32x4, __builtin_amdgcn_raw_buffer_load_b128(srcA[pl], off, 0, 0));
+    }
+#pragma unroll
+    for (int j = 0; j < PER; ++j) {
+      const int u = tid + j * NT;
+      if (UNITS % NT == 0 || u < UNITS) {
+        const int f = u / I2::UNITS;
+        const int a = I2::fill(f, u - f * I2::UNITS);
+#pragma unroll
+        for (int pl = 0; pl < NP; ++pl) *reinterpret_cast<u32x4*>(smem + pl * Place::PLANE2 + a) = v[j][pl];
+      }
+    }
+    if (tid < 16 * NP)
+      *reinterpret_cast<u32x4*>(smem + (tid >> 4) * Place::PLANE2 + Place::ZERO2 + 16 * (tid & 15)) = zero_u4();
+  }
+
+  typename Cfg::P2L q;
+  q.M = (f0 + nf) * I2::OPIX < p2.M ? (f0 + nf) * I2::OPIX : p2.M;
+  q.N = p2.N; q.K = p2.K; q.k_chunk = p2.k_chunk;
+  q.base = p2; q.img = smem + Place::X2; q.plane = Place::PLANE3; q.m0 = f0 * I2::OPIX;
+  q.hbm_rows = (hbm_frames < frames ? hbm_frames : frames) * I2::OPIX;
+  typename Ph2::C::Acc acc2;
+  acc2.zero();
+  const typename Cfg::P2L::Pre pre2 = q.pre(wn * 32 + Ph2::C::epi_col(lane));
+  Ph2::kloop(p2, w2, smem + Place::RING2, smem, Place::PLANE2, Place::ZERO2, nf * I2::OPIX, wm, wn,
+             lane, acc2);
+
+  uint8_t* x2 = smem + Place::X2;
+  if (tid < 16 * NP)
+    *reinterpret_cast<u32x4*>(x2 + (tid >> 4) * Place::PLANE3 + Place::ZERO3 + 16 * (tid & 15)) = zero_u4();
+  typename Ph3::Ring w3;
+  Ph3::init(w3, p3, tid);
+  Ph3::template fetch<0>(w3, p3, 0);
+  Ph3::template fetch<1>(w3, p3, Ph3::BK);
+  Ph2::C::epilogue(q, smem, q.m0, 0, wave, wm, wn, lane, 0, acc2, false, &pre2);
+  typename Ph3::C::Acc acc3;
+  acc3.zero();
+  const typename Cfg::P3::Pre pre3 = p3.pre(wn * 32 + Ph3::C::epi_col(lane));
+  Ph3::kloop(p3, w3, smem, x2, Place::PLANE3, Place::ZERO3, nf * I3::OPIX, wm, wn, lane, acc3);
+  typename Cfg::P3 q3 = p3;
+  q3.M = (f0 + nf) * I3::OPIX < p3.M ? (f0 + nf) * I3::OPIX : p3.M;
+  Ph3::C::epilogue(q3, smem, f0 * I3::OPIX, 0, wave, wm, wn, lane, 0, acc3, false, &pre3);
+}
+
+template <int BK2_, int BK3_, class G2, class G3>
+inline hipError_t launch_gemm_p3c23(const conv::P3ConvFwd<G2, kPlanes>& p2,
+                                    const conv::P3ConvFwd<G3, kPlanes>& p3, int frames,
+                                    int hbm_frames, hipStream_t st) {
+  using Cfg = P3C23Cfg<G2, G3, BK2_, BK3_>;
+  static hipError_t attr = p3_set_lds(&gemm_p3c23_kernel<G2, G3, BK2_, BK3_>, Cfg::LDS);
+  if (attr != hipSuccess) return attr;
+  if (frames < 2 || frames % Cfg::FPB != 0 || hbm_frames < 0 || p2.M != frames * G2::OPIX ||
+      p3.M != frames * G3::OPIX || p2.N != 64 || p3.N > 64 || p2.K % 32 != 0 || p3.K % 32 != 0)
+    return hipErrorInvalidValue;
+  hipLaunchKernelGGL((gemm_p3c23_kernel<G2, G3, BK2_, BK3_>), dim3(frames / Cfg::FPB),
+                     dim3(Cfg::NT), Cfg::LDS, st, p2, p3, frames, hbm_frames);
+  return hipGetLastError();
+}
+
+}
+}
diff --git a/acme_amd/csrc/gemm_p3i_geom.h b/acme_amd/csrc/gemm_p3i_geom.h
--- a/acme_amd/csrc/gemm_p3i_geom.h
+++ b/acme_amd/csrc/gemm_p3i_geom.h
@@ -177,5 +177,65 @@
   }
 };
 
+
+template <class Gfrom, class Gto>
+ACME_GEOM_FN int sink_at(int f, int pp, int n) {
+  static_assert(Gfrom::OH == Gto::IH && Gfrom::OW == Gto::IW && Gfrom::CO == Gto::CI,
+                "the output is the next layer's input");
+  const int oh = pp / Gfrom::OW, ow = pp - oh * Gfrom::OW;
+  return ImgGeom<Gto, false>::at(f, oh, ow, n / 8);
+}
+
+constexpr int p3_ring_bytes(int bn, int ng) { return 2 * ng * (2 * bn * 32 * 2); }
+constexpr int p3_epi_bytes(int waves, int tn) { return waves * 32 * (tn + 4) * 4; }
+
+struct LdsSpan {
+  int lo, hi;
+};
+constexpr bool lds_disjoint(LdsSpan a, LdsSpan b) { return a.hi <= b.lo || b.hi <= a.lo; }
+constexpr int lds_max(int a, int b) { return a > b ? a : b; }
+
+template <class G1, class G2, class G3, int NG1, int NG2, int NG3>
+struct C123Place {
+  using I1 = ImgGeomPairs<G1>;
+  using I2 = ImgGeom<G2, false>;
+  using I3 = ImgGeom<G3, false>;
+  static constexpr int NP = 2, WAVES = 8;
+  static constexpr int ZERO1 = img_zero_base(I1::IMG), FRAME = ZERO1 + kImgZeroBytes;
+  static constexpr int ZERO2 = img_zero_base(I2::IMG), PLANE2 = ZERO2 + kImgZeroBytes;
+  static constexpr int ZERO3 = img_zero_base(I3::IMG), PLANE3 = ZERO3 + kImgZeroBytes;
+  static constexpr int X1 = FRAME, X2 = FRAME;
+  static constexpr int LDS = X1 + NP * PLANE2;
+  static constexpr LdsSpan frame{0, FRAME}, x1{X1, X1 + NP * PLANE2}, x2{X2, X2 + NP * PLANE3};
+  static constexpr LdsSpan ring1{X1, X1 + p3_ring_bytes(32, NG1)};
+  static constexpr LdsSpan ring2{0, p3_ring_bytes(64, NG2)}, ring3{0, p3_ring_bytes(64, NG3)};
+  static constexpr LdsSpan epi1{0, p3_epi_bytes(WAVES, 32)}, epi23{0, p3_epi_bytes(WAVES, 32)};
+  static constexpr bool ok() {
+    return lds_disjoint(frame, ring1) && ring1.hi <= X1 + I2::IMG && lds_disjoint(epi1, x1) &&
+           lds_disjoint(ring2, x1) && lds_disjoint(epi23, x2) && lds_disjoint(ring3, x2) &&
+           x2.hi <= x1.hi && epi1.hi <= FRAME && epi23.hi <= FRAME && ring2.hi <= FRAME &&
+           ring3.hi <= FRAME && LDS <= 160 * 1024;
+  }
+};
+
+template <class G2, class G3, int NG2, int NG3>
+struct C23Place {
+  using I2 = ImgGeom<G2, false>;
+  using I3 = ImgGeom<G3, false>;
+  static constexpr int NP = 2, FPB = 2, WAVES = 16;
+  static constexpr int ZERO2 = img_zero_base(FPB * I2::IMG), PLANE2 = ZERO2 + kImgZeroBytes;
+  static constexpr int ZERO3 = img_zero_base(FPB * I3::IMG), PLANE3 = ZERO3 + kImgZeroBytes;
+  static constexpr int RING2 = NP * PLANE2;
+  static constexpr int EPI = p3_epi_bytes(WAVES, 32);
+  static constexpr int X2 = img_zero_base(lds_max(EPI, p3_ring_bytes(64, NG3)));
+  static constexpr LdsSpan x1{0, NP * PLANE2}, ring2{RING2, RING2 + p3_ring_bytes(64, NG2)};
+  static constexpr LdsSpan epi{0, EPI}, x2{X2, X2 + NP * PLANE3}, ring3{0, p3_ring_bytes(64, NG3)};
+  static constexpr int LDS = lds_max(ring2.hi, x2.hi);
+  static constexpr bool ok() {
+    return lds_disjoint(x1, ring2) && lds_disjoint(epi, x2) && lds_disjoint(ring3, x2) &&
+           LDS <= 160 * 1024;
+  }
+};
+
 }
 }
diff --git a/acme_amd/csrc/torso.h b/acme_amd/csrc/torso.h
--- a/acme_amd/csrc/torso.h
+++ b/acme_amd/csrc/torso.h
@@ -66,7 +66,8 @@
   }
 };
 int forward_p3(const PWeights& w, const Frames& frames, int rows, const PActs& a,
-               hipStream_t st, int keep_x1 = -1, bool bk32 = false);
+               hipStream_t st, int keep_x1 = -1, bool bk32 = false, int keep_x2 = -1);
+constexpr int kFuseX2Default = 3;
 struct WgradSlab {
   const float* slab = nullptr;
   int splits = 0;
diff --git a/acme_amd/csrc/torso.hip b/acme_amd/csrc/torso.hip
--- a/acme_amd/csrc/torso.hip
+++ b/acme_amd/csrc/torso.hip
@@ -154,7 +154,7 @@
 
 template <bool U8>
 int conv12_fwd_p3(const PWeights& w, const Frames& frames, int rows, int nsep, const PActs& a,
-                  hipStream_t st, bool bk32) {
+                  hipStream_t st, bool bk32, int keep_x2) {
   const int nf = rows - nsep;
   const Frames fr = frames.rows_from(nsep);
   if (U8 && fr.split < nf)
@@ -171,9 +171,23 @@
   p2.bias = w.b2;
   p2.y = Planes{a.x2.p + (int64_t)nsep * kFlat, a.x2.stride, a.x2.sc};
   const double fl = 2.0 * p1.M * p1.N * (double)p1.K + 2.0 * p2.M * p2.N * (double)p2.K;
-  ACME_PROF_PEAK("conv12_fwd", st, fl, 0.0, gemm::p3_peak_tflops<decltype(p2)>());
-  hipError_t e = bk32 ? gemm::launch_gemm_p3c12<32, 32>(p1, p2, nf, 0, st)
-                      : gemm::launch_gemm_p3c12<kBkFused1, kBkFused2>(p1, p2, nf, 0, st);
+  hipError_t e;
+  if (keep_x2 >= 0) {
+    P3ConvFwd<G3, gemm::kPlanes> p3;
+    p3.M = nf * G3::OPIX; p3.N = G3::CO; p3.K = G3::K; p3.k_chunk = G3::K;
+    p3.a_src = SRC(a.x2, (int64_t)rows * kFlat); p3.b_src = SRC(w.w3, G3::K * G3::CO);
+    p3.bias = w.b3;
+    p3.y = Planes{a.x3.p + (int64_t)nsep * kFlat, a.x3.stride, a.x3.sc};
+    const int keep = std::max(0, std::min(keep_x2, rows) - nsep);
+    ACME_PROF_PEAK("conv123_fwd", st, fl + 2.0 * p3.M * p3.N * (double)p3.K, 0.0,
+                   gemm::p3_peak_tflops<decltype(p2)>());
+    e = bk32 ? gemm::launch_gemm_p3c123<32, 32, 32>(p1, p2, p3, nf, 0, keep, st)
+             : gemm::launch_gemm_p3c123<kBkFused1, kBkFused2, kBkConv3>(p1, p2, p3, nf, 0, keep, st);
+  } else {
+    ACME_PROF_PEAK("conv12_fwd", st, fl, 0.0, gemm::p3_peak_tflops<decltype(p2)>());
+    e = bk32 ? gemm::launch_gemm_p3c12<32, 32>(p1, p2, nf, 0, st)
+             : gemm::launch_gemm_p3c12<kBkFused1, kBkFused2>(p1, p2, nf, 0, st);
+  }
   if (e != hipSuccess) return (set_error("gemm launch failed: %s", hipGetErrorString(e)), ACME_ERR_HIP);
   return ACME_OK;
 }
@@ -224,16 +238,35 @@
 }
 
 int forward_p3(const PWeights& w, const Frames& frames, int rows, const PActs& a,
-               hipStream_t st, int keep_x1, bool bk32) {
+               hipStream_t st, int keep_x1, bool bk32, int keep_x2) {
   const int nsep = keep_x1 == 0 ? 0 : rows;
+  const bool fuse3 = keep_x2 >= 0;
   int rc;
   if (nsep < rows &&
-      (rc = frames.u8 ? conv12_fwd_p3<true>(w, frames, rows, nsep, a, st, bk32)
-                      : conv12_fwd_p3<false>(w, frames, rows, nsep, a, st, bk32)) != ACME_OK)
+      (rc = frames.u8 ? conv12_fwd_p3<true>(w, frames, rows, nsep, a, st, bk32, keep_x2)
+                      : conv12_fwd_p3<false>(w, frames, rows, nsep, a, st, bk32, keep_x2)) != ACME_OK)
     return rc;
   if (nsep > 0 && (rc = frames.u8 ? conv1_fwd_p3<true>(w, frames, nsep, PP(a.x1), st, bk32, g_stamps_conv[0])
                                   : conv1_fwd_p3<false>(w, frames, nsep, PP(a.x1), st, bk32, g_stamps_conv[0])) != ACME_OK)
     return rc;
+  if (fuse3 && nsep > 0) {
+    if (rows % 2 != 0)
+      return (set_error("the fused conv2 -> conv3 forward takes an even number of frames"),
+              ACME_ERR_INVALID);
+    P3ConvFwd<G2, gemm::kPlanes> p2;
+    p2.M = rows * G2::OPIX; p2.N = G2::CO; p2.K = G2::K; p2.k_chunk = G2::K;
+    p2.a_src = SRC(a.x1, (int64_t)rows * kX1); p2.b_src = SRC(w.w2, G2::K * G2::CO);
+    p2.bias = w.b2; p2.y = PP(a.x2);
+    P3ConvFwd<G3, gemm::kPlanes> p3;
+    p3.M = rows * G3::OPIX; p3.N = G3::CO; p3.K = G3::K; p3.k_chunk = G3::K;
+    p3.a_src = SRC(a.x2, (int64_t)rows * kFlat); p3.b_src = SRC(w.w3, G3::K * G3::CO);
+    p3.bias = w.b3; p3.y = PP(a.x3);
+    const double fl = 2.0 * p2.M * p2.N * (double)p2.K + 2.0 * p3.M * p3.N * (double)p3.K;
+    ACME_LAUNCH_GEMM("conv23_fwd", fl, gemm::p3_peak_tflops<decltype(p2)>(),
+                     (bk32 ? gemm::launch_gemm_p3c23<32, 32>(p2, p3, rows, keep_x2, st)
+                           : gemm::launch_gemm_p3c23<kBkConv2, kBkConv3>(p2, p3, rows, keep_x2, st)));
+    return ACME_OK;
+  }
   if (nsep > 0) {
     P3ConvFwd<G2, gemm::kPlanes> p;
     p.M = nsep * G2::OPIX; p.N = G2::CO; p.K = G2::K; p.k_chunk = G2::K;
@@ -242,7 +275,7 @@
     p.stamps = g_stamps_conv[1];
     P3I_GEMM_BK("conv2_fwd", I2F, 2, 64, 8, 2, 1, kBkConv2, bk32, p, nsep);
   }
-  {
+  if (!fuse3) {
     P3ConvFwd<G3, gemm::kPlanes> p;
     p.M = rows * G3::OPIX; p.N = G3::CO; p.K = G3::K; p.k_chunk = G3::K;
     p.a_src = SRC(a.x2, (int64_t)rows * kFlat); p.b_src = SRC(w.w3, G3::K * G3::CO);
diff --git a/acme_amd/native.py b/acme_amd/native.py
--- a/acme_amd/native.py
+++ b/acme_amd/native.py
@@ -527,6 +527,9 @@
 
     def update_rider_launches(self) -> int:
         return int(lib().acme_dqn_update_rider_launches(self._h))
+
+    def fused_x2_launches(self) -> int:
+        return int(lib().acme_dqn_fused_x2_launches(self._h))
 
     @property
     def applied_steps(self) -> int:
diff --git a/include/acme_hip.h b/include/acme_hip.h
--- a/include/acme_hip.h
+++ b/include/acme_hip.h
@@ -196,6 +196,7 @@
 int acme_dqn_verdict_timeouts(acme_dqn* l, int64_t* out);
 int64_t acme_dqn_verdicts_issued(const acme_dqn* l);
 int64_t acme_dqn_update_rider_launches(const acme_dqn* l);
+int64_t acme_dqn_fused_x2_launches(const acme_dqn* l);
 int acme_dqn_step_verdict(const acme_dqn* l, int64_t seq, int32_t* state);
 int acme_dqn_scale_state(const acme_dqn* l, float* out, int32_t capacity, int32_t* count);
 int acme_dqn_set_scale_state(acme_dqn* l, const float* in, int32_t count);
```
